# PKU-MARL/HARL

Measured on AMD Instinct MI355X. Metric: transitions/sec through HAPPO update (MPE spread, 3 agents), higher is better.
Workload: dtype f32

## Files before the change

### harl_amd/_lib.py

```python
from __future__ import annotations

import ctypes as C
import os
from typing import Dict, Optional

import torch

from .traffic import algorithmic_bytes, algorithmic_flops

_HERE = os.path.dirname(os.path.abspath(__file__))
LIB_PATH = os.path.join(_HERE, "lib", "libharl_%s.so" % (os.environ.get("HARL_LIB") or "hip"))

PS_STRIDE = 48
DHEAD_LD = 32
SLAB = 32

_vp, _i, _l, _f, _d = C.c_void_p, C.c_int, C.c_long, C.c_float, C.c_double

SIGNATURES = {
    "harl_gae_returns": [_vp] * 8 + [_i, _i, _f, _f, _i, _i, _i, _vp],
    "harl_masked_moments": [_vp, _vp, _l, _vp, _vp, _vp],
    "harl_dist_rows": [_vp, _l, _i, _i, _vp, _f, _f, _vp, _vp, _vp, _i, _i, _vp, _vp, _vp, _vp, _vp, _vp],
    "harl_moments_mean": [_vp, _vp, _vp],
    "harl_clock_probe": [_vp, _l, _vp],
    "harl_build_seq": [_vp, _i, _i, _i, _l, _vp, _vp, _i, _vp, _vp, _vp, _vp, _vp],
    "harl_adv_normalize": [_vp, _vp, _vp, _l, _vp],
    "harl_factor_update": [_vp, _vp, _vp, _l, _i, _i, _vp],
    "harl_sum_sumsq": [_vp, _vp, _l, _vp, _vp],
    "harl_valuenorm_apply": [_vp, _vp, _d, _d, _vp],
    "harl_gradnorm_clip_adam": [_vp, _vp, _vp, _vp, _l, _vp, _i, _f, _d, _d, _d, _f, _f, _d, _d, _vp, _vp],
    "harl_fold_linear": [_vp] * 6 + [_i, _i, _vp],
    "harl_unfold_linear_grads": [_vp, _vp, _i, _vp, _vp, _vp, _vp, _vp, _vp, _vp, _i, _i, _i, _vp],
    "harl_mlp_fwd_input": [_vp, _l, _vp, _l, _i, _vp, _vp, _i, _i, _vp, _vp, _vp, _vp, _vp, _vp, _vp],
    "harl_mlp_x0n_wide": [_vp, _l, _vp, _l, _i, _i, _vp, _vp, _vp, _vp],
    "harl_mlp_fwd_wide": [_vp, _l, _i, _vp, _i, _vp, _i, _vp, _vp, _vp, _vp, _vp],
    "harl_mlp_linear_wide": [_vp, _l, _i, _vp, _i, _vp, _i, _vp, _vp, _vp],
    "harl_act_ln_fwd": [_vp, _l, _i, _i, _vp, _vp, _vp, _vp],
    "harl_act_bwd": [_vp, _vp, _vp, _vp, _l, _i, _i, _vp],
    "harl_act_ln_tangent": [_vp, _vp, _vp, _vp, _vp, _l, _i, _i, _vp, _vp],
    "harl_mlp_tangent_wide": [_vp, _l, _i, _vp, _i, _vp, _i, _vp, _vp, _vp, _vp, _vp, _vp],
    "harl_mlp_fwd_fused2x": [_vp, _l, _vp, _i, _vp, _vp, _vp, _i, _i, _vp, _vp, _vp, _vp, _vp, _vp, _vp],
    "harl_mlp_fwd_fused2": [_vp, _l, _vp, _l, _i, _vp, _vp, _i, _vp, _vp, _i, _i, _vp, _vp, _vp, _vp, _vp, _vp, _vp, _vp,
                            _vp, _vp],
    "harl_mlp_fwd_hidden": [_vp, _l, _i, _i, _vp, _vp, _vp, _vp, _vp, _vp],
    "harl_mlp_bwd_dx": [_vp, _vp, _vp, _vp, _l, _i, _i, _vp, _vp, _vp, _i, _vp, _i, _vp],
    "harl_mlp_bwd_dx_dw": [_vp, _vp, _vp, _vp, _l, _i, _i, _vp, _vp, _vp, _i, _vp, _vp, _i, _i, _vp],
    "harl_mlp_dw_partials": [_vp, _i, _i, _i, _vp, _i, _l, _vp, _vp, _vp, _i, _l, _vp, _i, _vp],
    "harl_mlp_dw_partials_multi": [_i, _vp, _vp, _vp, _i, _i, _l, _i, _vp],
    "harl_mlp_dw_partials_multi_v": [_i, _vp, _vp, _vp, _i, _vp, _vp, _vp, _l, _i, _vp],
    "harl_gru_dw6": [_vp, _vp, _vp, _vp, _vp, _vp, _vp, _l, _i, _vp],
    "harl_mlp_fwd_trunk": [_vp, _l, _i, _vp, _i, _vp, _i, _vp, _i, _vp, _vp, _vp, _vp, _vp, _vp, _vp, _vp, _vp, _vp],
    "harl_mlp_bwd_trunk": [_l, _i, _i, _vp, _vp, _vp, _vp, _vp, _vp, _vp, _vp, _vp, _vp, _vp],
    "harl_reduce_partials": [_vp, _i, _l, _vp, _vp],
    "harl_reduce_partials_multi": [_vp, _vp, _i, _i, _l, _vp, _vp],
    "harl_adam_fold": [_vp, _vp, _vp, _vp, _l, _vp, _vp, _i, _vp, _vp, _vp, _i, _vp, _i, _f, _i, _i, _vp, _i, _f, _d, _d,
                       _d, _f, _f, _d, _d, _vp, _vp],
    "harl_pack_scalars_hilo": [_vp, _vp, _vp],
    "harl_reduce_pack_scalars": [_vp, _i, _vp, _vp, _vp],
    "harl_randperm_replay": [_vp, _l, _l, _vp, _vp, _vp],
    "harl_rng_advance": [_vp, _l, _l, _vp],
    "harl_rng_jump": [_vp, _l, _l, _vp],
    "harl_actor_head_logp": [_vp, _l, _i, _vp, _vp, _vp, _f, _f, _i, _i, _vp, _vp, _vp, _vp, _vp, _i, _vp, _l, _l, _vp],
    "harl_actor_head_loss": [_vp, _vp, _vp, _l, _i, _vp, _vp, _vp, _f, _f, _i, _i, _vp, _vp, _vp, _vp, _vp, _vp,
                             _vp, _vp, _d, _f, _i, _i, _l, _l, _vp, _vp, _vp, _vp, _vp, _i, _vp],
    "harl_critic_head_values": [_vp, _l, _i, _vp, _vp, _vp, _vp],
    "harl_critic_head_loss": [_vp, _vp, _vp, _l, _i, _vp, _vp, _vp, _vp, _vp, _vp, _f, _i, _i, _f, _l, _l, _vp, _vp, _vp,
                              _vp, _i, _vp],
    "harl_gru_fwd": [_vp] * 7 + [_i, _i, _l] + [_vp] * 8 + [_i, _vp, _vp],
    "harl_gru_bwd": [_vp] * 9 + [_i, _i, _l] + [_vp] * 8 + [_vp],
    "harl_fold_linear_tangent": [_vp] * 9 + [_i, _i, _vp],
    "harl_fold_table": [_vp, _vp, _vp, _i, _i, _vp],
    "harl_unfold_table": [_vp, _vp, _vp, _vp, _i, _i, _vp],
    "harl_fold_tangent_table": [_vp, _vp, _vp, _vp, _i, _i, _vp],
    "harl_mlp_tangent_input": [_vp, _l, _vp, _l, _i, _vp, _vp, _i, _i, _vp, _vp, _vp, _vp, _vp],
    "harl_gru_gates": [_vp, _vp, _i, _l, _vp, _vp, _vp, _i, _vp],
    "harl_gru_tangent": [_vp] * 15 + [_i, _i, _l, _vp, _vp],
    "harl_mlp_tangent_hidden": [_vp, _vp, _l, _i, _i, _vp, _vp, _vp, _vp, _vp, _vp, _vp, _vp],
    "harl_mlp_tangent_hidden2": [_vp, _vp, _l, _i, _i, _vp, _vp, _vp, _vp, _vp, _vp, _vp, _vp, _vp],
    "harl_actor_head_fvp": [_vp, _vp, _vp, _vp, _l, _i, _vp, _vp, _vp, _vp, _vp, _f, _f, _i, _i, _vp, _l, _l, _vp, _vp, _vp],
    "harl_trpo_kl_sum": [_vp, _vp, _vp, _vp, _f, _f, _l, _i, _i, _vp, _vp],
    "harl_update_supported": [_i, _i, _i, _i],
    "harl_update_fwd_actor": [_vp, _l, _i, _i] + [_vp] * 7 + [_f, _f, _i, _i] + [_vp] * 7 + [_d, _f, _i, _i] + [_vp] * 4 + [_i] + [_vp] * 4,
    "harl_update_logp": [_vp, _l, _i, _i] + [_vp] * 7 + [_f, _f, _i, _i] + [_vp] * 5 + [_i, _vp, _vp],
    "harl_update_last_actor": [_vp, _l, _i] + [_vp] * 5 + [_f, _f, _i, _i] + [_vp] * 8 + [_d, _f, _i, _i] + [_vp] * 4 + [_i, _vp],
    "harl_update_last_critic": [_vp, _l, _i] + [_vp] * 8 + [_f, _i, _i, _f] + [_vp] * 3 + [_i, _vp],
    "harl_update_fwd_critic": [_vp, _l, _i, _i] + [_vp] * 9 + [_f, _i, _i, _f] + [_vp] * 3 + [_i] + [_vp] * 4,
    "harl_update_values": [_vp, _l, _i, _i] + [_vp] * 7 + [_vp],
    "harl_update_bwd": [_vp, _vp, _l, _i, _i] + [_vp] * 5 + [_i, _vp],
    "harl_head_blocks": [_l],
    "harl_trpo_fvp_finish": [_vp, _vp, _vp, _vp, _l, _f, _f, _l, _i, _f, _f, _vp],
    "harl_trpo_cg_step": [_vp, _vp, _vp, _vp, _l, _vp, _vp, _vp],
    "harl_mlp_panel_fwd": [_vp, _l, _i, _vp, _i, _vp, _i, _vp, _vp, _vp, _vp],
    "harl_mlp_panel_bwd": [_vp, _vp, _vp, _vp, _l, _i, _i, _vp, _vp, _vp],
    "harl_head_dw_rows256": [_vp, _l, _i, _vp, _vp, _i, _vp],
    "harl_mlp_panel_tangent": [_vp, _vp, _l, _i, _vp, _vp, _i, _vp, _vp, _vp, _vp, _vp, _vp],
    "harl_reduce_scalars": [_vp, _i, _vp, _vp],
    "harl_mlp_linear": [_vp, _l, _i, _i, _vp, _vp, _vp, _vp],
    "harl_mlp_linear3": [_vp, _vp, _vp, _l, _i, _i, _vp, _vp, _vp, _vp, _vp, _vp, _vp, _vp, _vp, _vp],
    "harl_gru_cell_init": [_vp, _vp, _i, _l, _vp, _vp],
    "harl_gru_cell_fwd": [_vp] * 8 + [_i, _l] + [_vp] * 7 + [_vp],
    "harl_gru_cell_bwd": [_vp] * 10 + [_i, _l] + [_vp] * 5 + [_vp],
    "harl_rownorm": [_vp, _l, _i, _vp, _vp, _vp],
    "harl_gru_cell_tangent": [_vp] * 19 + [_i, _l] + [_vp] * 3,
    "harl_md_head_logp": [_vp, _i, _vp, _i, _vp, _vp, _l, _vp, _vp, _vp, _i, _vp, _i, _vp, _l, _l, _vp],
    "harl_md_head_loss": [_vp, _vp, _i, _vp, _i, _vp, _vp, _l, _vp, _vp, _vp, _i, _vp, _vp, _vp, _vp, _vp, _d, _f, _i, _i,
                          _l, _l, _vp, _vp, _i, _vp],
    "harl_trpo_begin": [_vp, _vp, _l, _i, _vp, _vp, _vp, _vp, _l, _vp, _vp, _vp, _vp],
    "harl_trpo_step": [_vp, _vp, _vp, _vp, _vp, _vp, _l, _f, _vp, _vp, _vp],
    "harl_trpo_ls_candidate": [_vp, _vp, _vp, _vp, _l, _vp],
    "harl_trpo_ls_test": [_vp, _vp, _d, _d, _d, _d, _vp, _vp],
    "harl_reduce_scalars_set": [_vp, _i, _vp, _vp],
    "harl_zero_bytes": [_vp, _l, _vp],
    "harl_comm_create": [_i, _i, _l, _i, _vp, _vp],
    "harl_comm_connect": [_vp, _vp],
    "harl_comm_allreduce": [_vp, _vp, _l, _i, _vp],
    "harl_comm_set_timeout": [_vp, _d],
    "harl_comm_status": [_vp],
    "harl_comm_destroy": [_vp],
    "harl_version": [],
}


class HipLibraryMissing(RuntimeError):
    pass


_lib: Optional[C.CDLL] = None


def load() -> C.CDLL:
    global _lib
    if _lib is not None:
        return _lib
    if not os.path.exists(LIB_PATH):
        raise HipLibraryMissing(
# ... 109 lines not shown
```

### harl_amd/csrc/heads_common.h

```cpp
#pragma once
#include "common.h"

using namespace harl;

namespace {
constexpr float LOG_SQRT_2PI = 0.918938533204672741780329736406f;
constexpr float HALF_LOG_2PI_PLUS_HALF = 1.418938533204672741780329736406f;

struct ActorArgs {
  const float *xL;
  const uint32_t *relu_mask;
  const float *rstd;
  long M;
  const float *Whp, *bhp, *log_std;
  float std_x_coef, std_y_coef;
  int act_dim;
  const int64_t *idx;
  const float *actions, *avail, *old_logp, *adv;
  const double *adv_moments;
  const float *factor_in, *active;
  float clip_lo, clip_hi, entropy_coef;
  int agg_mean;
  float *dzL, *dhead, *part_scalars;
  float *dw_part;
  float *logp_out, *factor_out;
  float *head_out;
  long m_valid, m_pad;
  int trpo;
  long n_slabs;
};

template <int H, int DAP>
__device__ __forceinline__ void stage_head(float *whl, float *cst, const float *__restrict__ Whp,
                                           const float *__restrict__ bhp, int act_dim) {
  for (int e = threadIdx.x; e < 2 * (H / 2) * DAP; e += WG_THREADS) {
    const int d = e % DAP, R = (e / DAP) % (H / 2), hh = e / (DAP * (H / 2));
    const int f = feat_base(R) + 4 * hh;
    whl[e] = d < act_dim ? Whp[d * H + f] : 0.f;
  }
  for (int e = threadIdx.x; e < DAP; e += WG_THREADS) {
    cst[e] = e < act_dim ? bhp[e] : 0.f;
    float rs = 0.f;
    if (e < act_dim)
      for (int f = 0; f < H; ++f) rs += Whp[e * H + f];
    cst[4 * DAP + e] = rs;
  }
}

template <int H, int DAP>
__device__ __forceinline__ void head_fwd_stream(const float *__restrict__ xL, long slab, int lane,
                                                const float *whl_h, const float *cst, float (&z)[DAP]) {
#pragma unroll
  for (int d = 0; d < DAP; ++d) z[d] = 0.f;
  const f32x4 *xp = reinterpret_cast<const f32x4 *>(xL + slab * (long)(H * SLAB)) + lane;
// ... 78 lines not shown
      }
    }
    __builtin_amdgcn_sched_barrier(0);
  }
#pragma unroll
  for (int d = 0; d < DA; ++d) z[d] = wave_sum32(z[d]) + cst[d];
}

constexpr int HEAD_T_PAD = 16;
__host__ __device__ constexpr int head_t_rows(int da) { return 2 * ((da + 1) / 2); }
__host__ __device__ constexpr int head_t_block(int H, int da) { return head_t_rows(da) * (H / 2) + HEAD_T_PAD; }

template <int H, int DAP, int DA>
__device__ __forceinline__ void head_fwd_regs_t(const f32x4 (&xs)[H / 8], const float *whlT_h, const float *cst,
                                                float (&z)[DAP]) {
#pragma unroll
  for (int d = 0; d < DAP; ++d) z[d] = 0.f;
  f32x4 w[2][DA];
#pragma unroll
  for (int d = 0; d < DA; ++d) w[0][d] = *reinterpret_cast<const f32x4 *>(whlT_h + d * (H / 2));
#pragma unroll
  for (int q = 0; q < H / 8; ++q) {
    if (q + 1 < H / 8) {
#pragma unroll
      for (int d = 0; d < DA; ++d) w[(q + 1) & 1][d] = *reinterpret_cast<const f32x4 *>(whlT_h + d * (H / 2) + 4 * (q + 1));
    }
#pragma unroll
    for (int c = 0; c < 4; ++c)
#pragma unroll
      for (int d = 0; d < DA; ++d) z[d] += xs[q][c] * w[q & 1][d][c];
    __builtin_amdgcn_sched_barrier(0);
  }
#pragma unroll
  for (int d = 0; d < DA; ++d) z[d] = wave_sum32(z[d]) + cst[d];
}

template <int H, int DAP, int DA>
__device__ __forceinline__ void stage_head_t(float *whlT, float *cst, const float *__restrict__ Whp,
                                             const float *__restrict__ bhp, int n_threads) {
  constexpr int DAE = head_t_rows(DA), BLK = head_t_block(H, DA);
  for (int e = threadIdx.x; e < 2 * DAE * (H / 2); e += n_threads) {
    const int R = e % (H / 2), d = (e / (H / 2)) % DAE, hh = e / ((H / 2) * DAE);
    whlT[hh * BLK + d * (H / 2) + R] = d < DA ? Whp[d * H + feat_base(R) + 4 * hh] : 0.f;
  }
  for (int e = threadIdx.x; e < DAP; e += n_threads) {
    cst[e] = e < DA ? bhp[e] : 0.f;
    float rs = 0.f;
    if (e < DA)
      for (int f = 0; f < H; ++f) rs += Whp[e * H + f];
    cst[4 * DAP + e] = rs;
  }
}

template <int H, int DAP, int DA = DAP, bool PACKED = false, bool WT = false>
__device__ __forceinline__ void head_bwd_regs_bits(const f32x4 (&xs)[H / 8], uint32_t b0, const uint32_t b1, float rstd,
                                                   long slab, int lane, const float *whl ,
                                                   const float (&dzh)[DAP], float s1, float s2,
                                                   float *__restrict__ dz_out, const uint32_t bm1 = 0u,
                                                   const uint32_t bm2 = 0u) {
  s1 *= (1.0f / H);
  s2 *= (1.0f / H);
  const int i = lane & 31, h = lane >> 5;
  const float *wa = WT ? whl + ((i >> 2) & 1) * head_t_block(H, DA) + (i & 3) + 4 * (i >> 3) + h * (H / 2)
                       : whl + (((i >> 2) & 1) * (H / 2) + (i & 3) + 4 * (i >> 3)) * DAP + h;
  f32x16 acc[H / 32];
#pragma unroll
  for (int t = 0; t < H / 32; ++t)
#pragma unroll
    for (int r = 0; r < 16; ++r) acc[t][r] = 0.f;
#pragma unroll
  for (int st = 0; st < (DA + 1) / 2; ++st) {
    const unsigned hm = 0u - (unsigned)h;
    const float bsel = __uint_as_float((__float_as_uint(dzh[2 * st + 1]) & hm) | (__float_as_uint(dzh[2 * st]) & ~hm));
#pragma unroll
    for (int t = 0; t < H / 32; ++t)
      acc[t] = __builtin_amdgcn_mfma_f32_32x32x2f32(wa[WT ? 16 * t + 2 * st * (H / 2) : 16 * t * DAP + 2 * st], bsel, acc[t], 0, 0, 0);
  }
  f32x4 *op = reinterpret_cast<f32x4 *>(dz_out + slab * (long)(H * SLAB)) + lane;
  const float c1 = -s1 * rstd, c2 = -s2 * rstd;
  const f32x2 c1v = {c1, c1}, c2v = {c2, c2}, rv = {rstd, rstd};
#pragma unroll
  for (int q = 0; q < H / 8; ++q) {
    if (q == 8) b0 = H == 256 ? bm1 : b1;
    if (H == 256 && q == 16) b0 = bm2;
    if (H == 256 && q == 24) b0 = b1;
    f32x4 o;
    if constexpr (PACKED) {
#pragma unroll
      for (int P = 0; P < 2; ++P) {
        const int e = 4 * q + 2 * P;
        const f32x2 d = {acc[e >> 4][e & 15], acc[(e + 1) >> 4][(e + 1) & 15]}, x = {xs[q][2 * P], xs[q][2 * P + 1]};
        const f32x2 da = fma2(x, c2v, fma2(d, rv, c1v));
        o[2 * P] = mask_pop(da[0], b0);
        o[2 * P + 1] = mask_pop(da[1], b0);
      }
    } else {
#pragma unroll
      for (int c = 0; c < 4; ++c) {
        const float dx = acc[(4 * q + c) >> 4][(4 * q + c) & 15];
        const float da = rstd * (dx - s1 - xs[q][c] * s2);
        o[c] = (int)b0 < 0 ? da : 0.f;
        b0 <<= 1;
      }
    }
    op[q * WAVE] = o;
  }
}

template <int H, int DAP>
__device__ __forceinline__ void head_bwd_regs(const f32x4 (&xs)[H / 8], const uint32_t *__restrict__ mask_in,
                                              float rstd, long slab, int lane, const float *whl ,
                                              const float (&dzh)[DAP], float s1, float s2,
                                              float *__restrict__ dz_out) {
  constexpr int NW = (H / 2 + 31) / 32;
  const uint32_t b0 = mask_in[(slab * NW + 0) * WAVE + lane];
  const uint32_t b1 = NW > 1 ? mask_in[(slab * NW + (NW - 1)) * WAVE + lane] : 0u;
  const uint32_t bm1 = NW == 4 ? mask_in[(slab * NW + 1) * WAVE + lane] : 0u, bm2 = NW == 4 ? mask_in[(slab * NW + 2) * WAVE + lane] : 0u;
  head_bwd_regs_bits<H, DAP>(xs, b0, b1, rstd, slab, lane, whl, dzh, s1, s2, dz_out, bm1, bm2);
}

template <int H>
struct HeadDw {
  static constexpr int HX = 64 + 4;
  static constexpr int TD = 33;
  static constexpr int WAVE_FLOATS = SLAB * HX + SLAB * TD;
  static constexpr int OUT_FLOATS = 32 * H + 32;
};

template <int H, int DAP>
__device__ __forceinline__ void head_dw_step(const f32x4 (&xs)[H / 8], const float (&dzh)[DAP], float *tx, float *td,
                                             int lane, f32x16 (&acc)[H / 32]) {
  constexpr int HX = HeadDw<H>::HX, TD = HeadDw<H>::TD;
  const int i = lane & 31, h = lane >> 5;
  if (h == 0) {
#pragma unroll
    for (int d = 0; d < DAP; ++d) td[i * TD + d] = dzh[d];
  }
#pragma unroll
  for (int half = 0; half < H / 64; ++half) {
#pragma unroll
    for (int q = 0; q < 8; ++q)
      *reinterpret_cast<f32x4 *>(tx + i * HX + 32 * (q >> 2) + 8 * (q & 3) + 4 * h) = xs[8 * half + q];
    asm volatile("s_waitcnt lgkmcnt(0)" ::: "memory");
    __builtin_amdgcn_wave_barrier();
#pragma unroll
    for (int t = 0; t < SLAB / 2; ++t) {
      const float a = td[(2 * t + h) * TD + i];
#pragma unroll
      for (int n = 0; n < 2; ++n) {
        const float b = tx[(2 * t + h) * HX + 32 * n + i];
        acc[2 * half + n] = __builtin_amdgcn_mfma_f32_32x32x2f32(a, b, acc[2 * half + n], 0, 0, 0);
      }
    }
    asm volatile("s_waitcnt lgkmcnt(0)" ::: "memory");
    __builtin_amdgcn_wave_barrier();
  }
}

// ... 474 lines not shown
```

### harl_amd/csrc/mlp.hip

```cpp
#include "common.h"
#include "split_mfma.h"
#include "mfma_transpose.h"
#include "dw_common.h"
#include "fwd_epilogue.h"
#include "../../include/harl_hip.h"
#include <stdlib.h>
#include <type_traits>

using namespace harl;

#define MFMA(a, b, c) __builtin_amdgcn_mfma_f32_32x32x2f32((a), (b), (c), 0, 0, 0)

template <int HO>
__device__ __forceinline__ void ln_jac_store(f32x16 (&acc)[HO / 32], const float *__restrict__ xprimal,
                                             const uint32_t *__restrict__ mask_in, const float *__restrict__ rstd_in,
                                             int lane, long slab, float *__restrict__ xdot_out) {
  constexpr int NR = HO / 2, NW = (NR + 31) / 32;
  float xh[NR];
  atl_load<HO>(xprimal, slab, lane, xh);
  uint32_t bits[NW];
#pragma unroll
  for (int w = 0; w < NW; ++w) bits[w] = mask_in[(slab * NW + w) * WAVE + lane];
  const float rstd = rstd_in[slab * SLAB + (lane & 31)];
  float ad[NR];
// ... 1410 lines not shown
          constexpr int n = decltype(nc)::value, ks = n >> 2, b = n & 3;
          if constexpr (n + 1 < 8) read_frag(r & 1, (n + 1) >> 2, (n + 1) & 3, bv[(n + 1) & 1]);
          __builtin_amdgcn_sched_barrier(0);
          constexpr int AT[6] = {2, 0, 1, 1, 0, 0}, BT[6] = {0, 2, 1, 0, 1, 0};
          static_for<0, 6>([&](auto kc) {
            constexpr int k6 = decltype(kc)::value;
            acc2[b] = mfma_bf16(At[AT[k6]][ks], bv[n & 1][BT[k6]], acc2[b]);
            if constexpr (FILL) slot(std::integral_constant<int, 6 * n + k6>{});
            __builtin_amdgcn_sched_barrier(0);
          });
        });
        PHASE(6);
        b_store((r + 1) & 1);
#pragma unroll
        for (int t = 0; t < 3; ++t) {
          At[t][0] = AtN[t][0];
          At[t][1] = AtN[t][1];
        }
        PHASE(7);
      }
    });
  }

  {
    constexpr long ROW2 = (long)H * H + H;
    float *mypart = dw2_part + (long)blockIdx.x * ROW2;
#pragma unroll
    for (int b = 0; b < 4; ++b)
#pragma unroll
      for (int r = 0; r < 16; ++r) {
        const int o = 32 * wave + (r & 3) + 8 * (r >> 2) + 4 * h;
        mypart[(long)o * H + 32 * b + i] = acc2[b][r];
      }
    const float dbt = wave_sum32(db2);
    if (h == 0) mypart[(long)H * H + 32 * wave + i] = dbt;
    for (int row = blockIdx.x + gridDim.x; row < n_part_rows; row += gridDim.x) {
      float *z = dw2_part + (long)row * ROW2;
      for (int e = threadIdx.x; e < ROW2; e += WG_THREADS) z[e] = 0.f;
    }
  }
  if constexpr (KT > 0) {
    f32x16 a1x[4][1];
#pragma unroll
    for (int a = 0; a < 4; ++a) a1x[a][0] = acc1[a];
    finish_partials<4, 1>(a1x, dbs, reinterpret_cast<float *>(img), dw1_part, n_part_rows);
  }
  PHASE(11);
  PHASE_END(3);
}

#ifndef HARL_BWD_SPLIT_WAVES
#define HARL_BWD_SPLIT_WAVES 1
#endif
template <int KT, bool FILL>
__global__ __launch_bounds__(2 * WG_THREADS, 1) void k_bwd_dx_dw8(
    const float *__restrict__ dz, const float *__restrict__ xprev, const uint32_t *__restrict__ mask_prev,
    const float *__restrict__ rstd_prev, const float *__restrict__ Wp, float *__restrict__ dz_prev, long n_slabs,
    const float *__restrict__ x0n, float *__restrict__ dw1_part, float *__restrict__ dw2_part, int n_part_rows) {
  constexpr int H = 128, MT = 4, NJ = 8, NR = 64, KPF = 32, NTH = 2 * WG_THREADS;
  extern __shared__ __attribute__((aligned(16))) float lds[];
  PHASE_BEGIN();
  u32x4 *img = reinterpret_cast<u32x4 *>(lds);
  unsigned char *Bb = reinterpret_cast<unsigned char *>(img + 3 * MT * NJ * 64);
  stage_split_matrix<H, H, true, NTH>(img, Wp);
  __syncthreads();
  const int lane = threadIdx.x & 63, wave_ = wave_id();
  const int wave = wave_ & 3;
  const bool owner = wave_ < WAVES_PER_WG;
  const int i = lane & 31, h = lane >> 5;
  const u32x4 *wl = img + lane;
  const long sr_stride = (long)gridDim.x * WAVES_PER_WG;
  const long base0 = (long)blockIdx.x * WAVES_PER_WG;
  const Ident ident = make_ident(lane);

  f32x16 acc2[4];
  f32x16 acc1[KT > 0 ? 4 : 1];
  float dbs[KT > 0 ? 4 : 1];
  float db2 = 0.f;
  auto zero_acc2 = [&]() {
#pragma unroll
    for (int b = 0; b < 4; ++b)
#pragma unroll
      for (int r = 0; r < 16; ++r) acc2[b][r] = 0.f;
  };
  auto zero_acc1 = [&]() {
#pragma unroll
    for (int a = 0; a < (KT > 0 ? 4 : 1); ++a) {
      dbs[a] = 0.f;
#pragma unroll
      for (int r = 0; r < 16; ++r) acc1[a][r] = 0.f;
    }
  };

  f32x4 prA[4], prB[4];
  u32x2_t spB[4][3];
  u32x4 ya[3][2];
  f32x16 tc[3];
  u32x4 At[3][2], AtN[3][2];
  float rr0 = 0.f, rr1 = 0.f;
  auto d_load = [&](long ds) {
#pragma unroll
    for (int u = 0; u < 4; ++u) {
      prA[u] = (reinterpret_cast<const f32x4 *>(dz + ds * (long)(H * SLAB)) + lane)[(4 * wave + u) * WAVE];
      prB[u] = (reinterpret_cast<const f32x4 *>(xprev + ds * (long)(H * SLAB)) + lane)[(4 * wave + u) * WAVE];
    }
  };
  float vnext = 1.f;
  auto d_load_next = [&](long ds, long fallback) { d_load(ds < n_slabs ? ds : fallback); };
  auto a_chunk = [&](int k) {
    const int pi = k >> 1, j = pi >> 2, c = pi & 3, u = pi >> 1, e = 2 * (pi & 1);
    if ((k & 1) == 0) {
      unsigned p1;
      split_stage1(prA[u][e], prA[u][e + 1], p1, rr0, rr1);
      ya[0][j][c] = p1;
    } else {
      unsigned p2, p3;
      split_stage2(rr0, rr1, p2, p3);
      ya[1][j][c] = p2;
      ya[2][j][c] = p3;
    }
  };
  auto b_chunk = [&](int k) {
    const int u = k >> 2, c2 = (k >> 1) & 1;
    if ((k & 1) == 0) {
      unsigned p1;
      split_stage1(prB[u][2 * c2], prB[u][2 * c2 + 1], p1, rr0, rr1);
      spB[u][0][c2] = p1;
    } else {
      unsigned p2, p3;
      split_stage2(rr0, rr1, p2, p3);
      spB[u][1][c2] = p2;
      spB[u][2][c2] = p3;
    }
  };
  auto t_mfma = [&](int k) {
    const f32x16 zero = {0.f, 0.f, 0.f, 0.f, 0.f, 0.f, 0.f, 0.f, 0.f, 0.f, 0.f, 0.f, 0.f, 0.f, 0.f, 0.f};
    const int t = k % 3;
    if (k < 3) tc[t] = mfma_bf16(ya[t][0], ident.j0, zero);
    else tc[t] = mfma_bf16(ya[t][1], ident.j1, tc[t]);
  };
  auto p_chunk = [&](int k) {
    if (k < 3) {
      pack_transposed(tc[k], AtN[k][0], AtN[k][1]);
    } else {
      f32x2 a = {0.f, 0.f};
#pragma unroll
      for (int r = 0; r < 8; ++r) a += f32x2{tc[k - 3][2 * r], tc[k - 3][2 * r + 1]};
      db2 += vnext * (a[0] + a[1]);
    }
  };
  auto b_store = [&](int buf) {
#pragma unroll
    for (int u = 0; u < 4; ++u) {
      const int q = 4 * wave + u;
      unsigned char *d = Bb + buf * BDW_BUF + (i >> 2) * BDW_SQ + (2 * (q >> 2) + ((q & 3) >> 1)) * 128 + (i & 3) * 32 +
                         (8 * (q & 1) + 4 * h) * 2;
#pragma unroll
      for (int term = 0; term < 3; ++term) *reinterpret_cast<u32x2_t *>(d + term * BDW_IMG) = spB[u][term];
    }
  };
  const int p16 = lane & 15, g1b = (lane >> 4) & 1;
  const int frag_lane = g1b * 128 + (p16 >> 2) * 32 + (p16 & 3) * 8;
  auto read_frag = [&](int buf, int ks, int tile, u32x4 (&f)[3]) {
#pragma unroll
    for (int term = 0; term < 3; ++term) {
      const unsigned char *fp = Bb + buf * BDW_BUF + term * BDW_IMG + (4 * ks + h) * BDW_SQ + 2 * tile * 128 + frag_lane;
      const u32x2_t lo = tr_read(fp), hi = tr_read(fp + 2 * BDW_SQ);
      f[term] = u32x4{lo[0], lo[1], hi[0], hi[1]};
    }
  };

  float raw[NR];
  u32x4 g1[NJ], g2[NJ], g3[NJ];
  auto o_chunk = [&](int k) {
    const int pi = k >> 1, j = pi >> 2, c = pi & 3;
    if ((k & 1) == 0) {
      unsigned p1;
      split_stage1(raw[2 * pi], raw[2 * pi + 1], p1, rr0, rr1);
      g1[j][c] = p1;
    } else {
      unsigned p2, p3;
      split_stage2(rr0, rr1, p2, p3);
      g2[j][c] = p2;
      g3[j][c] = p3;
    }
  };
  if (!owner && base0 < n_slabs) {
    d_load(base0);
#pragma unroll
    for (int k = 0; k < 16; ++k) a_chunk(k);
#pragma unroll
    for (int k = 0; k < 6; ++k) t_mfma(k);
#pragma unroll
    for (int k = 0; k < 16; ++k) b_chunk(k);
#pragma unroll
    for (int k = 0; k < 6; ++k) p_chunk(k);
#pragma unroll
    for (int t = 0; t < 3; ++t) {
      At[t][0] = AtN[t][0];
      At[t][1] = AtN[t][1];
    }
    b_store(0);
  }
  PHASE(10);

  auto o_part = [&](long base) {
    const long slab = base + wave;
    const bool own = slab < n_slabs;
    constexpr int OB1 = KT > 0 ? 4 : 3, OB2 = KT > 0 ? NJ : 6, OB3 = KT > 0 ? NJ + 1 : NJ;
    auto obar = [&](int k) {
      if (base + k < n_slabs) __builtin_amdgcn_s_barrier();
    };
    if (own) {
      constexpr int RAW_LEAD = 3;
      auto raw_ks = [&](int j) {
        const f32x4 *p = reinterpret_cast<const f32x4 *>(dz + slab * (long)(H * SLAB)) + lane;
#pragma unroll
        for (int c = 0; c < 2; ++c) {
          const f32x4 v = p[(2 * j + c) * WAVE];
#pragma unroll
          for (int e = 0; e < 4; ++e) raw[8 * j + 4 * c + e] = v[e];
        }
      };
#pragma unroll
      for (int j = 0; j < RAW_LEAD; ++j) raw_ks(j);
      obar(0);
#pragma unroll
      for (int k = 0; k < 8; ++k) o_chunk(k);
      float xh[NR];
      float rstd;
      uint32_t mbits[2];
      f32x4 x0r[KT > 0 ? KPF / 8 : 1];
      auto x0_operands = [&]() {
        if constexpr (KT > 0) {
          const f32x4 *bp = reinterpret_cast<const f32x4 *>(x0n + slab * (long)(KPF * SLAB)) + lane;
#pragma unroll
          for (int q = 0; q < KPF / 8; ++q) x0r[q] = bp[q * WAVE];
        }
      };
      auto ln_operands = [&]() {
        atl_load<H>(xprev, slab, lane, xh);
        rstd = rstd_prev[slab * SLAB + i];
#pragma unroll
        for (int w = 0; w < 2; ++w) mbits[w] = mask_prev[(slab * 2 + w) * WAVE + lane];
      };
      constexpr int LN_STEP = NJ;
      f32x16 acc[MT];
#pragma unroll
      for (int t = 0; t < MT; ++t)
#pragma unroll
        for (int r = 0; r < 16; ++r) acc[t][r] = 0.f;
      PHASE(0);
      split_gemm_fill<MT, NJ>(wl, g1, g2, g3, acc, [&](int s_, int k6) {
        const int j1 = s_ / MT + 1, q = (s_ % MT) * 6 + k6;
        if (j1 < NJ && q % 3 == 0) o_chunk(8 * j1 + q / 3);
        if (s_ % MT == 0 && k6 == 0 && j1 - 1 + RAW_LEAD < NJ) raw_ks(j1 - 1 + RAW_LEAD);
        if (s_ % MT == MT - 1 && k6 == 5) {
          if (j1 == LN_STEP) ln_operands();
          if (j1 == OB1) obar(1);
          if (j1 == OB2) obar(2);
          if (j1 == OB3) obar(3);
        }
      });
      PHASE(1);
      float dx[NR];
#pragma unroll
      for (int R = 0; R < NR; ++R) dx[R] = acc[R >> 4][R & 15];
      float out[NR];
      ln_bwd_relu_mbits<H>(dx, xh, mbits, rstd, out);
      if (dz_prev) atl_store<H>(dz_prev, slab, lane, out);
      x0_operands();
      if constexpr (OB3 == NJ + 1) obar(3);
      PHASE(2);
      if constexpr (KT > 0) {
        float xr0[KPF / 2];
#pragma unroll
        for (int q = 0; q < KPF / 8; ++q) {
          xr0[4 * q + 0] = x0r[q][0];
          xr0[4 * q + 1] = x0r[q][1];
          xr0[4 * q + 2] = x0r[q][2];
          xr0[4 * q + 3] = x0r[q][3];
        }
        u32x4 a1[KPF / 16], a2[KPF / 16], a3[KPF / 16];
        split_acts<KPF / 2>(xr0, a1, a2, a3);
        u32x4 Bt[3][2];
        transpose_block<false>(a1[0], a1[1], a2[0], a2[1], a3[0], a3[1], ident, Bt);
#pragma unroll
        for (int a = 0; a < 4; ++a) {
          u32x4 A1[3][2];
          dbs[a] += split_transpose_block<true>(&out[16 * a], ident, A1);
          dw_tile(acc1[a], A1, Bt);
        }
        PHASE(3);
      }
    }
    else {
#pragma unroll
      for (int k = 0; k < 4; ++k) obar(k);
    }
  };
  auto d_part = [&](long base) {
    d_load_next(base + 1, base);
    PHASE(4);
    static_for<0, 4>([&](auto rc) {
      constexpr int r = decltype(rc)::value;
      if (base + r < n_slabs) {
        __syncthreads();
        PHASE(5);
        const long ds1 = r < 3 ? base + r + 1 : base + sr_stride;
        const long ds2 = r < 2 ? base + r + 2 : base + sr_stride;
        vnext = uniform_f(ds1 < n_slabs ? 1.f : 0.f);
        constexpr int TSLOT = r == 0 ? 31 : 15;
        auto slot = [&](auto sc) {
          constexpr int s_ = decltype(sc)::value;
          if constexpr (r == 0) {
            if constexpr (s_ >= 16 && s_ < 32) a_chunk(s_ - 16);
            else if constexpr (s_ >= 32 && s_ < 42) b_chunk(s_ - 32 + 6);
            else if constexpr (s_ >= 42) p_chunk(s_ - 42);
            if constexpr (s_ == 47) d_load_next(ds2, base);
          } else {
            if constexpr (s_ < 16) a_chunk(s_);
            else if constexpr (s_ < 26) b_chunk(s_ - 16 + 6);
            else if constexpr (s_ < 32) p_chunk(s_ - 26);
            if constexpr (s_ == 31 && r < 3) d_load_next(ds2, base);
          }
          if constexpr (s_ == TSLOT) {
            static_for<0, 6>([&](auto kc) {
              constexpr int k = decltype(kc)::value;
              __builtin_amdgcn_sched_barrier(0);
              t_mfma(k);
              b_chunk(k);
            });
          }
        };
        u32x4 bv[2][3];
        read_frag(r & 1, 0, 0, bv[0]);
        if constexpr (!FILL) static_for<0, 48>(slot);
        static_for<0, 8>([&](auto nc) {
          constexpr int n = decltype(nc)::value, ks = n >> 2, b = n & 3;
          if constexpr (n + 1 < 8) read_frag(r & 1, (n + 1) >> 2, (n + 1) & 3, bv[(n + 1) & 1]);
          __builtin_amdgcn_sched_barrier(0);
          constexpr int AT[6] = {2, 0, 1, 1, 0, 0}, BT[6] = {0, 2, 1, 0, 1, 0};
          static_for<0, 6>([&](auto kc) {
            constexpr int k6 = decltype(kc)::value;
            acc2[b] = mfma_bf16(At[AT[k6]][ks], bv[n & 1][BT[k6]], acc2[b]);
            if constexpr (FILL) slot(std::integral_constant<int, 6 * n + k6>{});
            __builtin_amdgcn_sched_barrier(0);
          });
        });
        PHASE(6);
        b_store((r + 1) & 1);
#pragma unroll
        for (int t = 0; t < 3; ++t) {
          At[t][0] = AtN[t][0];
          At[t][1] = AtN[t][1];
        }
        PHASE(7);
      }
    });
  };
  if (owner) {
    zero_acc1();
    for (long base = base0; base < n_slabs; base += sr_stride) o_part(base);
    zero_acc2();
  } else {
    zero_acc2();
    for (long base = base0; base < n_slabs; base += sr_stride) d_part(base);
    zero_acc1();
  }

  {
    constexpr long ROW2 = (long)H * H + H;
    float *mypart = dw2_part + (long)blockIdx.x * ROW2;
    if (!owner) {
#pragma unroll
      for (int b = 0; b < 4; ++b)
#pragma unroll
        for (int r = 0; r < 16; ++r) {
          const int o = 32 * wave + (r & 3) + 8 * (r >> 2) + 4 * h;
          mypart[(long)o * H + 32 * b + i] = acc2[b][r];
        }
      const float dbt = wave_sum32(db2);
      if (h == 0) mypart[(long)H * H + 32 * wave + i] = dbt;
    }
    for (int row = blockIdx.x + gridDim.x; row < n_part_rows; row += gridDim.x) {
      float *z = dw2_part + (long)row * ROW2;
      for (int e = threadIdx.x; e < ROW2; e += NTH) z[e] = 0.f;
    }
  }
  if constexpr (KT > 0) {
    f32x16 a1x[4][1];
#pragma unroll
    for (int a = 0; a < 4; ++a) a1x[a][0] = acc1[a];
    finish_partials<4, 1, NTH>(a1x, dbs, reinterpret_cast<float *>(img), dw1_part, n_part_rows);
  }
  PHASE(11);
  PHASE_END_BY(4, 0);
  PHASE_END_BY(5, 64 * WAVES_PER_WG);
}

HARL_PHASE_ACCESSOR(mlp)

static int bad(const char *m) {
  set_error(m);
  return -2;
}

extern "C" int harl_mlp_fwd_input(const float *X, long ldx, const int64_t *idx, long M, int D, const float *Wp,
                                  const float *bp, int use_ln0, int H, float *xout, uint32_t *relu_mask, float *rstd,
                                  float *mu0, float *rstd0, float *x0n, void *stream) {
  if (M <= 0) return 0;
  const long n_slabs = n_slabs_of(M);
  const int nch = (D + 31) / 32;
  const int grid = persistent_grid(n_slabs, 2);
  hipStream_t s = (hipStream_t)stream;
  if (H != 128 && H != 64) return bad("harl_mlp_fwd_input: hidden width must be 64 or 128");
  if (D <= 64) {
    const int kr = D <= 32 ? 32 : 64;
    const size_t shm = ((size_t)kr * H + H + (size_t)WAVES_PER_WG * SLAB * (kr + 1)) * sizeof(float);
#define LS(Hv, R)                                                                                                 \
  {                                                                                                               \
    allow_big_lds(k_fwd_input_staged<Hv, R>, shm);                                                                \
    hipLaunchKernelGGL((k_fwd_input_staged<Hv, R>), dim3(grid), dim3(WG_THREADS), shm, s, X, ldx, idx, M, D, Wp, bp, \
                       use_ln0, xout, relu_mask, rstd, mu0, rstd0, x0n, n_slabs);                                  \
  }
    if (H == 128) {
      if (D <= 32) LS(128, 2) else LS(128, 1)
    } else {
      if (D <= 32) LS(64, 2) else LS(64, 1)
    }
#undef LS
    return check_launch("harl_mlp_fwd_input");
  }
  const int resident = (long)nch * 32 * H * 4 <= 64 * 1024;
  const size_t shm = ((size_t)(resident ? nch * 32 : 32) * H + H) * sizeof(float);
  if (H == 128) {
    allow_big_lds(k_fwd_input<128, false>, shm);
    hipLaunchKernelGGL((k_fwd_input<128, false>), dim3(grid), dim3(WG_THREADS), shm, s, X, ldx, idx, M, D, Wp, bp,
                       use_ln0, xout, relu_mask, rstd, mu0, rstd0, n_slabs, nch, resident, nullptr, nullptr, nullptr);
  } else {
    allow_big_lds(k_fwd_input<64, false>, shm);
    hipLaunchKernelGGL((k_fwd_input<64, false>), dim3(grid), dim3(WG_THREADS), shm, s, X, ldx, idx, M, D, Wp, bp,
                       use_ln0, xout, relu_mask, rstd, mu0, rstd0, n_slabs, nch, resident, nullptr, nullptr, nullptr);
  }
  return check_launch("harl_mlp_fwd_input");
}

extern "C" int harl_mlp_tangent_input(const float *X, long ldx, const int64_t *idx, long M, int D, const float *Wdp,
                                      const float *bdp, int use_ln0, int H, const float *x1, const uint32_t *mask1,
                                      const float *rstd1, float *x1dot, void *stream) {
  if (M <= 0) return 0;
  const long n_slabs = n_slabs_of(M);
// ... 176 lines not shown
static bool lean_bwd() {
  static const bool v = [] {
    const char *e = getenv("HARL_BWD_STREAMS");
    return e && e[0] == '1';
  }();
  return v;
}

extern "C" int harl_mlp_bwd_dx(const float *dz, const float *xprev, const uint32_t *relu_mask_prev,
                               const float *rstd_prev, long M, int HO, int HI, const float *Wp, float *dz_prev,
                               const float *x0n, int kp0, float *dw_part, int n_wg, void *stream) {
  if (M <= 0) return 0;
  const long n_slabs = n_slabs_of(M);
  hipStream_t s = (hipStream_t)stream;
  if (dw_part) {
    if (!x0n || (kp0 != 32 && kp0 != 64) || n_wg <= 0)
      return bad("harl_mlp_bwd_dx: fused first-layer gradient needs x0n, kp0 in {32, 64} and n_wg > 0");
#define LFX(a, b, kt, lean)                                                                                       \
  {                                                                                                               \
    size_t shm = split_image_bytes(b, a);                                                                         \
    const size_t rowb = ((size_t)b * 32 * kt + b) * sizeof(float);                                                \
    if (shm < rowb) shm = rowb;                                                                                   \
    allow_big_lds(k_bwd_dx<a, b, kt, lean>, shm);                                                                 \
    hipLaunchKernelGGL((k_bwd_dx<a, b, kt, lean>), dim3(n_wg < 256 ? n_wg : 256), dim3(WG_THREADS), shm, s, dz,   \
                       xprev, relu_mask_prev, rstd_prev, Wp, dz_prev, n_slabs, x0n, dw_part, n_wg);               \
  }
#define LF(a, b, kt) LFX(a, b, kt, false)
    const int kt = kp0 / 32;
    if (HO == 128 && HI == 128 && kt == 1 && lean_bwd()) LFX(128, 128, 1, true)
    else if (HO == 128 && HI == 128) { if (kt == 1) LF(128, 128, 1) else LF(128, 128, 2) }
    else if (HO == 64 && HI == 64) { if (kt == 1) LF(64, 64, 1) else LF(64, 64, 2) }
    else if (HO == 128 && HI == 64) { if (kt == 1) LF(128, 64, 1) else LF(128, 64, 2) }
    else if (HO == 64 && HI == 128) { if (kt == 1) LF(64, 128, 1) else LF(64, 128, 2) }
    else return bad("harl_mlp_bwd_dx: widths must be 64 or 128");
#undef LF
#undef LFX
    return check_launch("harl_mlp_bwd_dx");
  }
  const size_t shm = split_image_bytes(HI, HO);
  const int grid = persistent_grid(n_slabs, split_one_wg(HI, HO) ? 1 : 2);
#define L(a, b)                                                                                                    \
  allow_big_lds(k_bwd_dx<a, b>, shm);                                                                              \
  hipLaunchKernelGGL((k_bwd_dx<a, b>), dim3(grid), dim3(WG_THREADS), shm, s, dz, xprev, relu_mask_prev, rstd_prev, Wp, \
                     dz_prev, n_slabs, nullptr, nullptr, 0)
  if (HO == 128 && HI == 128) { L(128, 128); }
  else if (HO == 64 && HI == 64) { L(64, 64); }
  else if (HO == 128 && HI == 64) { L(128, 64); }
  else if (HO == 64 && HI == 128) { L(64, 128); }
  else return bad("harl_mlp_bwd_dx: widths must be 64 or 128");
#undef L
  return check_launch("harl_mlp_bwd_dx");
}

extern "C" int harl_mlp_bwd_dx_dw(const float *dz, const float *xprev, const uint32_t *relu_mask_prev,
                                  const float *rstd_prev, long M, int HO, int HI, const float *Wp, float *dz_prev,
                                  const float *x0n, int kp0, float *dw1_part, float *dw2_part, int n_wg, int fill,
                                  void *stream) {
  if (M <= 0) return 0;
  if (HO != 128 || HI != 128) return bad("harl_mlp_bwd_dx_dw: 128 x 128 layers only (the layer kernels take the other widths)");
  if (!dw2_part || n_wg <= 0) return bad("harl_mlp_bwd_dx_dw: needs the partial arena of dW' and n_wg > 0");
  const bool first = dw1_part != nullptr;
  if (first && (!x0n || kp0 != 32)) return bad("harl_mlp_bwd_dx_dw: the fused first-layer gradient needs x0n with kp0 = 32");
  if (!first && !dz_prev) return bad("harl_mlp_bwd_dx_dw: dz_prev is required when no first-layer gradient is fused");
  const long n_slabs = n_slabs_of(M);
  const long wgs = (n_slabs + WAVES_PER_WG - 1) / WAVES_PER_WG;
  int grid = n_wg < 256 ? n_wg : 256;
  if (wgs < grid) grid = (int)wgs;
  const size_t shm = bdw_lds_bytes();
  hipStream_t s = (hipStream_t)stream;
#if HARL_BWD_SPLIT_WAVES
#define LB(kt, fl)                                                                                                    \
  {                                                                                                                   \
    allow_big_lds(k_bwd_dx_dw8<kt, fl>, shm);                                                                         \
    hipLaunchKernelGGL((k_bwd_dx_dw8<kt, fl>), dim3(grid), dim3(2 * WG_THREADS), shm, s, dz, xprev, relu_mask_prev,  \
                       rstd_prev, Wp, dz_prev, n_slabs, x0n, dw1_part, dw2_part, n_wg);                              \
  }
#else
#define LB(kt, fl)                                                                                                    \
  {                                                                                                                   \
    allow_big_lds(k_bwd_dx_dw<kt, fl>, shm);                                                                          \
    hipLaunchKernelGGL((k_bwd_dx_dw<kt, fl>), dim3(grid), dim3(WG_THREADS), shm, s, dz, xprev, relu_mask_prev,       \
                       rstd_prev, Wp, dz_prev, n_slabs, x0n, dw1_part, dw2_part, n_wg);                              \
  }
#endif
  if (first) { if (fill) LB(1, true) else LB(1, false) }
  else { if (fill) LB(0, true) else LB(0, false) }
#undef LB
  return check_launch("harl_mlp_bwd_dx_dw");
}

template <int MT, int NT>
static void launch_dw_tr(const float *a, const float *b, long n_slabs, float *part, int K, int tile0, int n_wg, hipStream_t s) {
  const size_t shm = (size_t)3 * 8 * ((2 * MT * 128 + 8) + (2 * NT * 128 + 8));
  allow_big_lds(k_dw_tr<MT, NT>, shm);
  hipLaunchKernelGGL((k_dw_tr<MT, NT>), dim3(n_wg), dim3(WG_THREADS), shm, s, a, b, n_slabs, part, (long)K * SLAB, tile0, K);
}

template <int A_KIND, int B_KIND, int MT, int NT>
static void launch_dw(const float *a, const float *b, long ldx, const int64_t *idx, const float *mu0,
                      const float *rstd0, int K, long M, long n_slabs, float *part, int KP, int n_wg, int ny,
                      hipStream_t s) {
  const size_t shm = ((size_t)DW_S * ((32 * MT + 4) + (32 * NT + 4)) + 2 * DW_S) * sizeof(float);
  hipLaunchKernelGGL((k_dw<A_KIND, B_KIND, MT, NT>), dim3(n_wg, ny), dim3(WG_THREADS), shm, s, a, b, ldx, idx, mu0,
                     rstd0, K, M, n_slabs, part, KP);
}

extern "C" int harl_mlp_dw_partials(const float *a, int a_kind, int lda, int HO, const float *b, int b_kind, long ldx,
                                    const int64_t *idx, const float *mu0, const float *rstd0, int K, long M,
                                    float *part, int n_wg, void *stream) {
  if (M <= 0 || n_wg <= 0) return 0;
  const long n_slabs = n_slabs_of(M);
  const int KP = ((K + 31) / 32) * 32;
  hipStream_t s = (hipStream_t)stream;
  if (a_kind == 1 && lda != DHEAD_LD) return bad("harl_mlp_dw_partials: head gradient matrix must have row stride 32");
  const int MT = a_kind == 1 ? 1 : HO / 32;
  if (a_kind == 0 && HO != 64 && HO != 128 && HO != 256) return bad("harl_mlp_dw_partials: HO must be 64, 128 or 256");
  if (a_kind == 1 && HO > 32) return bad("harl_mlp_dw_partials: head width must be <= 32");
#define DW(AK, BK, MTv, NTv, ny) launch_dw<AK, BK, MTv, NTv>(a, b, ldx, idx, mu0, rstd0, K, M, n_slabs, part, KP, n_wg, ny, s)
  if (b_kind == 0) {
    const int NT = K / 32;
    if (K % 32 != 0 || K < 32) return bad("harl_mlp_dw_partials: ATL input width must be a multiple of 32");
#define DWS(MTv, NTv) launch_dw_tr<MTv, NTv>(a, b, n_slabs, part, K, tile0, n_wg, s);
    if (K > 128 || K == 96 || MT == 8) {
      if (K % 32 != 0 || K > 512 || (MT != 8 && MT != 4 && MT != 2)) return bad("harl_mlp_dw_partials: wide ATL input must be a multiple of 32, <= 512");
      const int ntiles = K / 32;
      const int gstep = MT == 8 ? 2 : (MT == 4 && ntiles > 4 ? (ntiles + (ntiles + 5) / 6 - 1) / ((ntiles + 5) / 6) : 4);
      for (int tile0 = 0; tile0 < ntiles; tile0 += gstep) {
        const int nt = ntiles - tile0 < gstep ? ntiles - tile0 : gstep;
        if (MT == 8) {
          if (nt == 2) DWS(8, 2) else DWS(8, 1)
        } else if (MT == 4) {
          if (nt == 6) DWS(4, 6) else if (nt == 5) DWS(4, 5) else
          if (nt == 4) DWS(4, 4) else if (nt == 3) DWS(4, 3) else if (nt == 2) DWS(4, 2) else DWS(4, 1)
        } else {
          if (nt == 4) DWS(2, 4) else if (nt == 3) DWS(2, 3) else if (nt == 2) DWS(2, 2) else DWS(2, 1)
        }
      }
      return check_launch("harl_mlp_dw_partials");
    }
    const int tile0 = 0;
    if (MT == 4 && NT == 1) DW(0, 0, 4, 1, 1);
    else if (MT == 2 && NT == 1) DW(0, 0, 2, 1, 1);
// ... 92 lines not shown
```

### harl_amd/csrc/update.hip

```cpp
#include <type_traits>
#include "common.h"
#include "split_mfma.h"
#include "heads_common.h"
#include "mfma_transpose.h"
#include "../../include/harl_hip.h"

using namespace harl;

namespace {

int bad(const char *m) {
  set_error(m);
  return -2;
}

template <int H, bool MASK>
__device__ __forceinline__ void relu_ln(const f32x16 (&acc)[H / 32], float (&v)[H / 2], uint32_t (&bits)[(H / 2 + 31) / 32],
                                        float &rstd_out) {
  constexpr int NR = H / 2;
#pragma unroll
  for (int w = 0; w < (NR + 31) / 32; ++w) bits[w] = 0u;
#pragma unroll
  for (int R = 0; R < NR; ++R) {
    if constexpr (MASK) v[R] = relu_push(acc[R >> 4][R & 15], bits[R >> 5]);
// ... 208 lines not shown
#pragma unroll
        for (int r = 0; r < 16; ++r) acc[t][r] = b1l[32 * t + (r & 3) + 8 * (r >> 2) + 4 * h];
      split_gemm<MT, NJ1>(wl1, a1, a2, a3, acc, [](int) {});
      relu_ln<H, true>(acc, x1, bits1, r1);
      ln_bwd_relu_bits<H>(dx, x1, bits1, r1, dz1);
    }
    u32x4 B[KT][3][2];
#pragma unroll
    for (int n = 0; n < KT; ++n)
      transpose_block<false>(a1[2 * n], a1[2 * n + 1], a2[2 * n], a2[2 * n + 1], a3[2 * n], a3[2 * n + 1], I, B[n]);
#pragma unroll
    for (int a = 0; a < MT; ++a) {
      u32x4 A[3][2];
      dbs[a] += split_transpose_block<true>(&dz1[16 * a], I, A);
#pragma unroll
      for (int n = 0; n < KT; ++n) dw_tile(acc1[a][n], A, B[n]);
    }
  }
  finish_partials<MT, KT>(acc1, dbs, reinterpret_cast<float *>(img2), part, n_part_rows);
}

struct UpdFwdArgs {
  const float *x0n, *W1p, *b1p, *W2p, *b2p;
  int D;
  long n_slabs;
  float *dz2;
  int n_part_rows;
  float *xh1;
  uint32_t *mask1;
  float *rstd1;
};

constexpr int UF_WAVES = 8, UF_THREADS = 64 * UF_WAVES;

template <int NV>
__device__ __forceinline__ void block_reduce_store8(float (&v)[NV], float *red , float *out_row) {
  const int lane = threadIdx.x & 63, wave = wave_id();
#pragma unroll
  for (int k = 0; k < NV; ++k) {
    float t = wave_reduce_sum(v[k]);
    if (lane == 0) red[wave * PS_STRIDE + k] = t;
  }
  __syncthreads();
  if (threadIdx.x < PS_STRIDE) {
    float t = 0.f;
    if (threadIdx.x < NV) {
#pragma unroll
      for (int w = 0; w < UF_WAVES; ++w) t += red[w * PS_STRIDE + threadIdx.x];
    }
    out_row[threadIdx.x] = t;
  }
}

template <int H, int KP0, int DA, bool DISCRETE, bool TRAIN, typename ARGS>
__global__ __launch_bounds__(UF_THREADS, 2) void k_upd_fwd(UpdFwdArgs U, ARGS A) {
  constexpr bool CRITIC = std::is_same<ARGS, CriticArgs>::value;
  static_assert(DA >= 1 && DA <= 8 && (!CRITIC || DA == 1), "the LDS head-gradient tile covers 8 head outputs");
  constexpr int DAP = DA <= 4 ? 4 : 8;
  constexpr int HROWS = DA;
  constexpr bool HID = KP0 == 0;
  constexpr bool EARLY_X0N = H == 128 && KP0 == 32 && DA <= 5 && !DISCRETE;
  constexpr bool EARLY_X0N_LP = !TRAIN && !HID && (H == 64 || (DA != 4 && !(KP0 == 64 && DA >= 7 && !DISCRETE)));
  static_assert(!HID || TRAIN, "the last-layer variant exists for optimiser steps only");
  extern __shared__ __attribute__((aligned(16))) float lds[];
  PHASE_BEGIN();
  constexpr int MT = H / 32, NJ1 = KP0 / 16, NJ2 = H / 16, NR = H / 2, NW = (NR + 31) / 32;
  u32x4 *w2img = reinterpret_cast<u32x4 *>(lds);
  u32x4 *w1img = w2img + 3 * MT * NJ2 * 64;
  float *b1l = reinterpret_cast<float *>(w1img + 3 * MT * NJ1 * 64);
  float *b2l = b1l + H;
  float *whlT = b2l + H;
  float *cst = whlT + 2 * head_t_block(H, DA);
  float *red = cst + 7 * DAP;
  float *hacc = red + UF_WAVES * PS_STRIDE;
  const int lane = threadIdx.x & 63, wave = wave_id(), i = lane & 31, h = lane >> 5;
  const long slab0 = (long)wave * gridDim.x + blockIdx.x, slab_stride = (long)gridDim.x * UF_WAVES;
  constexpr int NXR = HID ? NR : KP0 / 2;
  float xr[NXR];
  atl_load<2 * NXR>(U.x0n, slab0 < U.n_slabs ? slab0 : 0, lane, xr);
  constexpr bool ROWS = !CRITIC || TRAIN;
  long rawn = 0;
  if constexpr (ROWS) rawn = row_index_request(A.idx, A.Whp, slab0, lane, A.M);
  stage_split_matrix<H, H, false, UF_THREADS>(w2img, U.W2p);
  if constexpr (!HID) stage_w1_images<H, KP0, UF_THREADS>(w1img, U.W1p, U.D);
  for (int e = threadIdx.x; e < H; e += UF_THREADS) {
    if constexpr (!HID) b1l[e] = U.b1p[e];
    b2l[e] = U.b2p[e];
  }
  if (TRAIN)
    for (int e = threadIdx.x; e < UF_WAVES * HROWS * H; e += UF_THREADS) hacc[e] = 0.f;
  if (threadIdx.x < WG_THREADS) {
    stage_head_t<H, DAP, DA>(whlT, cst, A.Whp, A.bhp, WG_THREADS);
    if constexpr (!CRITIC) {
      if (!DISCRETE) {
        for (int e = threadIdx.x; e < DAP; e += WG_THREADS) {
          float sg = 0.5f, sig = 1.f, lsig = 0.f, dsd = 0.f;
          if (e < A.act_dim) {
            sg = 1.0f / (1.0f + expf(-A.log_std[e] / A.std_x_coef));
            sig = sg * A.std_y_coef;
            lsig = logf(sig);
            dsd = A.std_y_coef * sg * (1.f - sg) / A.std_x_coef;
          }
          cst[DAP + e] = sig;
          cst[2 * DAP + e] = lsig;
          cst[3 * DAP + e] = dsd;
          cst[5 * DAP + e] = 1.0f / sig;
          cst[6 * DAP + e] = 1.0f / (sig * sig);
        }
// ... 113 lines not shown
      s2 = dv * (z[0] - cst[0]);
    } else {
      if (!actor_sample<DAP, DISCRETE, TRAIN, DA>(A, cst, z, slab, lane, adv_mean, adv_den, sc, dzh, s1, s2, rcur)) continue;
    }
    PHASE(6);
    if constexpr (TRAIN) {
      if constexpr (EARLY_X0N) atl_load<2 * NXR>(U.x0n, sn, lane, xr);
      int lane_o = lane;
      asm volatile("" : "+v"(lane_o));
      const Ident I = make_ident(lane_o);
      const u32x4 I16 = make_ident16(lane_o);
      u32x4 Ah[3][2];
      {
        float e8[8];
#pragma unroll
        for (int c = 0; c < 8; ++c) e8[c] = (c < DAP && h == 0) ? dzh[c < DAP ? c : 0] : 0.f;
        u32x4 t1, t2, t3;
#pragma unroll
        for (int c = 0; c < 4; ++c) {
          unsigned a, b, d;
          split3(e8[2 * c], e8[2 * c + 1], a, b, d);
          t1[c] = a;
          t2[c] = b;
          t3[c] = d;
        }
        const f32x16 zero = {0.f, 0.f, 0.f, 0.f, 0.f, 0.f, 0.f, 0.f, 0.f, 0.f, 0.f, 0.f, 0.f, 0.f, 0.f, 0.f};
        const f32x16 c1 = mfma_bf16(t1, I16, zero), c2 = mfma_bf16(t2, I16, zero), c3 = mfma_bf16(t3, I16, zero);
        pack_transposed(c1, Ah[0][0], Ah[0][1]);
        pack_transposed(c2, Ah[1][0], Ah[1][1]);
        pack_transposed(c3, Ah[2][0], Ah[2][1]);
      }
#pragma unroll
      for (int n = 0; n < MT; ++n) {
        u32x4 B[3][2];
        split_transpose_block<false>(&v[16 * n], I, B);
        f32x16 tile = {0.f, 0.f, 0.f, 0.f, 0.f, 0.f, 0.f, 0.f, 0.f, 0.f, 0.f, 0.f, 0.f, 0.f, 0.f, 0.f};
        dw_tile(tile, Ah, B);
#pragma unroll
        for (int r = 0; r < 4; ++r) {
          if (r < HROWS && h == 0) hw[r * H + 32 * n + i] += tile[r];
          if (4 + r < HROWS && h == 1) hw[(4 + r) * H + 32 * n + i] += tile[r];
        }
      }
      if constexpr (CRITIC) {
        if (h == 0) dbacc[0] += dzh[0];
      } else {
        if (h == 1) {
#pragma unroll
          for (int d = 0; d < DAP; ++d) sc[8 + d] += dzh[d];
        }
      }
      PHASE(7);
      if constexpr (!EARLY_X0N) atl_load<2 * NXR>(U.x0n, sn, lane, xr);
      head_bwd_regs_bits<H, DAP, DA, true, true>(xs, bits2[0], bits2[NW - 1], r2, slab, lane, whlT, dzh, s1, s2, U.dz2);
      PHASE(8);
    }
  }
  if constexpr (TRAIN) {
    float dbv[DAP];
#pragma unroll
    for (int d = 0; d < DAP; ++d) {
      if constexpr (CRITIC) {
        dbv[d] = dbacc[d];
      } else {
        dbv[d] = h == 1 ? sc[8 + d] : 0.f;
        sc[8 + d] = h == 0 ? sc[8 + d] : 0.f;
      }
    }
    block_reduce_store8<NSC>(sc, red, A.part_scalars + (long)blockIdx.x * PS_STRIDE);
    for (int row = blockIdx.x + gridDim.x; row < U.n_part_rows; row += gridDim.x)
      if (threadIdx.x < PS_STRIDE) A.part_scalars[(long)row * PS_STRIDE + threadIdx.x] = 0.f;
    float dbs[DAP];
#pragma unroll
    for (int d = 0; d < DAP; ++d) dbs[d] = wave_reduce_sum(dbv[d]);
    float *dbl = red;
    __syncthreads();
    if (lane == 0) {
#pragma unroll
      for (int d = 0; d < DAP; ++d) dbl[wave * PS_STRIDE + d] = dbs[d];
    }
    __syncthreads();
    float *out = A.dw_part + (long)blockIdx.x * HeadDw<H>::OUT_FLOATS;
    for (int e = threadIdx.x; e < HeadDw<H>::OUT_FLOATS; e += UF_THREADS) {
      float t = 0.f;
      if (e < 32 * H) {
        const int row = e / H;
        if (row < HROWS) {
#pragma unroll
          for (int w = 0; w < UF_WAVES; ++w) t += hacc[(w * HROWS + row) * H + (e - row * H)];
        }
      } else {
        const int d = e - 32 * H;
        if (d < DAP) {
#pragma unroll
          for (int w = 0; w < UF_WAVES; ++w) t += dbl[w * PS_STRIDE + d];
        }
      }
      out[e] = t;
    }
    for (int row = blockIdx.x + gridDim.x; row < U.n_part_rows; row += gridDim.x) {
      float *zr = A.dw_part + (long)row * HeadDw<H>::OUT_FLOATS;
      for (int e = threadIdx.x; e < HeadDw<H>::OUT_FLOATS; e += UF_THREADS) zr[e] = 0.f;
    }
  }
  PHASE(11);
  PHASE_END((TRAIN ? 0 : 2) + (CRITIC ? 1 : 0));
}

int fwd_grid(long n_slabs) {
  const long wgs = (n_slabs + UF_WAVES - 1) / UF_WAVES;
  return (int)(wgs < 256 ? (wgs < 1 ? 1 : wgs) : 256);
}

int upd_grid(long n_slabs) {
  const long wgs = (n_slabs + WAVES_PER_WG - 1) / WAVES_PER_WG;
  return (int)(wgs < 256 ? (wgs < 1 ? 1 : wgs) : 256);
}

size_t fwd_lds_bytes(int H, int kp0, int dap, int hrows, int da) {
  return split_image_bytes(H, H) + split_image_bytes(H, kp0) +
         ((size_t)2 * H + (size_t)2 * head_t_block(H, da) + 7 * dap + UF_WAVES * PS_STRIDE + (size_t)UF_WAVES * hrows * H) *
             sizeof(float);
}

constexpr size_t LDS_PER_WG_MAX = 160 * 1024;

template <int H, int KP0, int DA, bool DISC, bool TRAIN, typename ARGS>
int launch_fwd(const UpdFwdArgs &U, const ARGS &A, hipStream_t s) {
  const size_t shm = fwd_lds_bytes(H, KP0, DA <= 4 ? 4 : 8, TRAIN ? DA : 0, DA);
  if (shm > LDS_PER_WG_MAX) {
    return bad("harl_update_*: this (D, H, act_dim) does not fit the LDS of one workgroup");
  }
  allow_big_lds(k_upd_fwd<H, KP0, DA, DISC, TRAIN, ARGS>, shm);
  hipLaunchKernelGGL((k_upd_fwd<H, KP0, DA, DISC, TRAIN, ARGS>), dim3(fwd_grid(U.n_slabs)), dim3(UF_THREADS), shm, s, U, A);
  return 0;
}

template <int H, int KP0, bool TRAIN, int DA = 8>
int launch_actor_width(const UpdFwdArgs &U, const ActorArgs &A, int discrete, hipStream_t s) {
  if (A.act_dim == DA)
    return discrete ? launch_fwd<H, KP0, DA, true, TRAIN, ActorArgs>(U, A, s) : launch_fwd<H, KP0, DA, false, TRAIN, ActorArgs>(U, A, s);
  if constexpr (DA > 1) return launch_actor_width<H, KP0, TRAIN, DA - 1>(U, A, discrete, s);
  return bad("harl_update_*: act_dim must be in [1, 8]");
}

template <bool TRAIN>
int dispatch_fwd_actor(const UpdFwdArgs &U, const ActorArgs &A, int H, int discrete, hipStream_t s) {
  const int D = A.act_dim;
  if (D < 1 || D > 8) return bad("harl_update_fwd: act_dim must be in [1, 8]");
  const int kp0 = U.D <= 32 ? 32 : 64;
#define CASE(Hv, Kv)                                                                \
  if (H == Hv && kp0 == Kv) {                                                       \
    const int rc = launch_actor_width<Hv, Kv, TRAIN>(U, A, discrete, s);             \
    return rc ? rc : check_launch("harl_update_fwd");                               \
  }
  CASE(128, 32) CASE(128, 64) CASE(64, 32) CASE(64, 64)
#undef CASE
  return bad("harl_update_fwd: hidden width must be 64 or 128");
}

int dispatch_last_actor(const UpdFwdArgs &U, const ActorArgs &A, int H, int discrete, hipStream_t s) {
  const int D = A.act_dim;
  if (D < 1 || D > 8) return bad("harl_update_last_actor: act_dim must be in [1, 8]");
  int rc;
  if (H == 128) rc = launch_actor_width<128, 0, true>(U, A, discrete, s);
  else if (H == 64) rc = launch_actor_width<64, 0, true>(U, A, discrete, s);
  else return bad("harl_update_last_actor: hidden width must be 64 or 128");
  return rc ? rc : check_launch("harl_update_last_actor");
}

int dispatch_last_critic(const UpdFwdArgs &U, const CriticArgs &A, int H, hipStream_t s) {
  int rc;
  if (H == 128) rc = launch_fwd<128, 0, 1, false, true, CriticArgs>(U, A, s);
  else if (H == 64) rc = launch_fwd<64, 0, 1, false, true, CriticArgs>(U, A, s);
  else return bad("harl_update_last_critic: hidden width must be 64 or 128");
  return rc ? rc : check_launch("harl_update_last_critic");
}

template <bool TRAIN>
int dispatch_fwd_critic(const UpdFwdArgs &U, const CriticArgs &A, int H, hipStream_t s) {
  const int kp0 = U.D <= 32 ? 32 : 64;
#define CASE(Hv, Kv)                                                     \
  if (H == Hv && kp0 == Kv) {                                            \
    const int rc = launch_fwd<Hv, Kv, 1, false, TRAIN, CriticArgs>(U, A, s); \
    return rc ? rc : check_launch("harl_update_fwd");                        \
  }
  CASE(128, 32) CASE(128, 64) CASE(64, 32) CASE(64, 64)
#undef CASE
  return bad("harl_update_fwd: hidden width must be 64 or 128");
}

}

HARL_PHASE_ACCESSOR(update)

extern "C" int harl_update_supported(int D, int H, int act_dim, int kind) {
  if (!(D >= 0 && D <= 64 && (H == 64 || H == 128) && act_dim >= 1 && act_dim <= 8)) return 0;
  const int dap = act_dim <= 4 ? 4 : 8;
  const int hrows = kind == 0 ? 0 : (kind == 2 ? 1 : act_dim);
  return fwd_lds_bytes(H, D == 0 ? 0 : (D <= 32 ? 32 : 64), dap, hrows, kind == 2 ? 1 : act_dim) <= LDS_PER_WG_MAX ? 1 : 0;
}

extern "C" int harl_update_fwd_actor(const float *x0n, long M, int D, int H, const float *W1p, const float *b1p,
                                     const float *W2p, const float *b2p, const float *Whp, const float *bhp,
                                     const float *log_std, float std_x_coef, float std_y_coef, int discrete, int act_dim,
                                     const float *actions, const float *avail, const float *old_logp, const float *adv,
                                     const double *adv_moments, const float *factor, const float *active,
                                     double clip_param, float entropy_coef, int agg_mean, int trpo, float *logp_out,
                                     float *dz2, float *part_scalars, float *dw_part_head, int n_part_rows, float *xh1,
                                     uint32_t *rmask1, float *rstd1, void *stream) {
  if (M <= 0) return 0;
  if (D < 1 || D > 64) return bad("harl_update_fwd_actor: input width must be <= 64");
  if (!dz2 || !part_scalars || !dw_part_head || n_part_rows <= 0) return bad("harl_update_fwd_actor: missing outputs");
  if (xh1 && (!rmask1 || !rstd1)) return bad("harl_update_fwd_actor: xh1 needs rmask1 and rstd1");
  UpdFwdArgs U{x0n, W1p, b1p, W2p, b2p, D, n_slabs_of(M), dz2, n_part_rows, xh1, rmask1, rstd1};
  if (fwd_grid(U.n_slabs) > n_part_rows) return bad("harl_update_fwd_actor: n_part_rows smaller than the launch grid");
  ActorArgs A{};
  A.trpo = trpo;
  A.logp_out = logp_out;
  A.dw_part = dw_part_head;
  A.M = M; A.Whp = Whp; A.bhp = bhp; A.log_std = log_std;
  A.std_x_coef = std_x_coef; A.std_y_coef = std_y_coef; A.act_dim = act_dim;
  A.actions = actions; A.avail = avail; A.old_logp = old_logp; A.adv = adv; A.adv_moments = adv_moments;
  A.factor_in = factor; A.active = active; A.entropy_coef = entropy_coef;
  A.clip_lo = (float)(1.0 - clip_param); A.clip_hi = (float)(1.0 + clip_param);
  A.agg_mean = agg_mean; A.part_scalars = part_scalars; A.n_slabs = U.n_slabs;
  return dispatch_fwd_actor<true>(U, A, H, discrete, (hipStream_t)stream);
}

extern "C" int harl_update_logp(const float *x0n, long M, int D, int H, const float *W1p, const float *b1p,
                                const float *W2p, const float *b2p, const float *Whp, const float *bhp,
                                const float *log_std, float std_x_coef, float std_y_coef, int discrete, int act_dim,
                                const float *actions, const float *avail, float *logp_out, const float *old_logp,
                                float *factor, int agg_mean, float *head_out, void *stream) {
  if (M <= 0) return 0;
  if (D < 1 || D > 64) return bad("harl_update_logp: input width must be <= 64");
  if (factor && !old_logp) return bad("harl_update_logp: factor update needs old_logp");
  UpdFwdArgs U{x0n, W1p, b1p, W2p, b2p, D, n_slabs_of(M), nullptr, 0, nullptr, nullptr, nullptr};
  ActorArgs A{};
  A.head_out = head_out;
  A.M = M; A.Whp = Whp; A.bhp = bhp; A.log_std = log_std;
  A.std_x_coef = std_x_coef; A.std_y_coef = std_y_coef; A.act_dim = act_dim;
  A.actions = actions; A.avail = avail; A.old_logp = old_logp; A.agg_mean = agg_mean;
  A.logp_out = logp_out; A.factor_out = factor; A.n_slabs = U.n_slabs;
  return dispatch_fwd_actor<false>(U, A, H, discrete, (hipStream_t)stream);
}

extern "C" int harl_update_fwd_critic(const float *x0n, long M, int D, int H, const float *W1p, const float *b1p,
                                      const float *W2p, const float *b2p, const float *Whp, const float *bhp,
                                      const float *value_preds, const float *returns, const float *vn_stats,
                                      float clip_param, int use_clipped, int use_huber, float huber_delta, float *dz2,
                                      float *part_scalars, float *dw_part_head, int n_part_rows, float *xh1,
                                      uint32_t *rmask1, float *rstd1, void *stream) {
  if (M <= 0) return 0;
  if (D < 1 || D > 64) return bad("harl_update_fwd_critic: input width must be <= 64");
  if (!dz2 || !part_scalars || !dw_part_head || n_part_rows <= 0) return bad("harl_update_fwd_critic: missing outputs");
  if (xh1 && (!rmask1 || !rstd1)) return bad("harl_update_fwd_critic: xh1 needs rmask1 and rstd1");
  UpdFwdArgs U{x0n, W1p, b1p, W2p, b2p, D, n_slabs_of(M), dz2, n_part_rows, xh1, rmask1, rstd1};
  if (fwd_grid(U.n_slabs) > n_part_rows) return bad("harl_update_fwd_critic: n_part_rows smaller than the launch grid");
  CriticArgs A{};
  A.M = M; A.Whp = Whp; A.bhp = bhp;
  A.value_preds = value_preds; A.returns = returns; A.vn_stats = vn_stats; A.clip_param = clip_param;
  A.huber_delta = huber_delta; A.use_clipped = use_clipped; A.use_huber = use_huber;
  A.part_scalars = part_scalars; A.n_slabs = U.n_slabs;
  A.dw_part = dw_part_head;
  return dispatch_fwd_critic<true>(U, A, H, (hipStream_t)stream);
}

extern "C" int harl_update_last_actor(const float *xin, long M, int H, const float *Wp, const float *bp, const float *Whp,
                                      const float *bhp, const float *log_std, float std_x_coef, float std_y_coef,
                                      int discrete, int act_dim, const int64_t *idx, const float *actions,
                                      const float *avail, const float *old_logp, const float *adv,
                                      const double *adv_moments, const float *factor, const float *active,
                                      double clip_param, float entropy_coef, int agg_mean, int trpo, float *logp_out,
                                      float *dz, float *part_scalars, float *dw_part_head, int n_part_rows, void *stream) {
  if (M <= 0) return 0;
  if (!xin || !dz || !part_scalars || !dw_part_head || n_part_rows <= 0) return bad("harl_update_last_actor: missing arguments");
  UpdFwdArgs U{xin, nullptr, nullptr, Wp, bp, 0, n_slabs_of(M), dz, n_part_rows, nullptr, nullptr, nullptr};
  if (fwd_grid(U.n_slabs) > n_part_rows) return bad("harl_update_last_actor: n_part_rows smaller than the launch grid");
  ActorArgs A{};
  A.trpo = trpo;
  A.logp_out = logp_out;
  A.dw_part = dw_part_head;
  A.M = M; A.Whp = Whp; A.bhp = bhp; A.log_std = log_std;
  A.std_x_coef = std_x_coef; A.std_y_coef = std_y_coef; A.act_dim = act_dim; A.idx = idx;
  A.actions = actions; A.avail = avail; A.old_logp = old_logp; A.adv = adv; A.adv_moments = adv_moments;
  A.factor_in = factor; A.active = active; A.entropy_coef = entropy_coef;
  A.clip_lo = (float)(1.0 - clip_param); A.clip_hi = (float)(1.0 + clip_param);
  A.agg_mean = agg_mean; A.part_scalars = part_scalars; A.n_slabs = U.n_slabs;
  return dispatch_last_actor(U, A, H, discrete, (hipStream_t)stream);
}

extern "C" int harl_update_last_critic(const float *xin, long M, int H, const float *Wp, const float *bp, const float *Whp,
                                       const float *bhp, const int64_t *idx, const float *value_preds, const float *returns,
                                       const float *vn_stats, float clip_param, int use_clipped, int use_huber,
                                       float huber_delta, float *dz, float *part_scalars, float *dw_part_head,
                                       int n_part_rows, void *stream) {
  if (M <= 0) return 0;
  if (!xin || !dz || !part_scalars || !dw_part_head || n_part_rows <= 0) return bad("harl_update_last_critic: missing arguments");
  UpdFwdArgs U{xin, nullptr, nullptr, Wp, bp, 0, n_slabs_of(M), dz, n_part_rows, nullptr, nullptr, nullptr};
  if (fwd_grid(U.n_slabs) > n_part_rows) return bad("harl_update_last_critic: n_part_rows smaller than the launch grid");
  CriticArgs A{};
  A.M = M; A.Whp = Whp; A.bhp = bhp; A.idx = idx;
  A.value_preds = value_preds; A.returns = returns; A.vn_stats = vn_stats; A.clip_param = clip_param;
  A.huber_delta = huber_delta; A.use_clipped = use_clipped; A.use_huber = use_huber;
  A.part_scalars = part_scalars; A.n_slabs = U.n_slabs;
  A.dw_part = dw_part_head;
  return dispatch_last_critic(U, A, H, (hipStream_t)stream);
}

extern "C" int harl_update_values(const float *x0n, long M, int D, int H, const float *W1p, const float *b1p,
                                  const float *W2p, const float *b2p, const float *Whp, const float *bhp, float *values,
                                  void *stream) {
  if (M <= 0) return 0;
  if (D < 1 || D > 64) return bad("harl_update_values: input width must be <= 64");
  UpdFwdArgs U{x0n, W1p, b1p, W2p, b2p, D, n_slabs_of(M), nullptr, 0, nullptr, nullptr, nullptr};
  CriticArgs A{};
  A.M = M; A.Whp = Whp; A.bhp = bhp; A.values_out = values; A.n_slabs = U.n_slabs;
  return dispatch_fwd_critic<false>(U, A, H, (hipStream_t)stream);
// ... 33 lines not shown
```

### harl_amd/happo.py

```python
from __future__ import annotations

import os
from typing import Optional

import numpy as np
import torch

from . import _lib
from ._lib import PS_STRIDE, call, ptr, stream
from .buffers import OnPolicyActorBuffer, consume_randperm, minibatch_indices, rng_sync
from .dist import Comm, local_minibatch_rows
from .nets import FusedAdam, StochasticPolicy, build_seq, seq_compact
from .valuenorm import _as_dev


class OnPolicyBase:

    def __init__(self, args, obs_space, act_space, device=torch.device("cuda:0")):
        self.args = args
        self.device = torch.device(device)
        _lib.require_gpu(self.device)
        self.tpdv = dict(dtype=torch.float32, device=self.device)
        self.data_chunk_length = args["data_chunk_length"]
        self.use_recurrent_policy = args["use_recurrent_policy"]
# ... 142 lines not shown
                else:
                    actions.copy_(torch.multinomial(probs, 1))
                self._dist_rows(head, M, actions=actions, logp=logp)
        else:
            noise = None if deterministic else torch.randn_like(head)
            actions = torch.empty_like(head)
            logp = torch.empty_like(head)
            self._dist_rows(head, M, noise=noise, actions=actions, logp=logp)
        return actions, logp, rnn_out

    @torch.no_grad()
    def act(self, obs, rnn_states_actor, masks, available_actions=None, deterministic=False):
        actions, _, rnn = self.get_actions(obs, rnn_states_actor, masks, available_actions, deterministic)
        return actions, rnn

    def prep_training(self):
        self.actor.train()
        self.actor.invalidate_caches()

    def prep_rollout(self):
        self.actor.eval()
        self.actor.invalidate_caches()


class HAPPO(OnPolicyBase):
    def __init__(self, args, obs_space, act_space, device=torch.device("cuda:0")):
        super().__init__(args, obs_space, act_space, device)
        self.clip_param = args["clip_param"]
        self.ppo_epoch = args["ppo_epoch"]
        self.actor_num_mini_batch = args["actor_num_mini_batch"]
        self.entropy_coef = args["entropy_coef"]
        self.use_max_grad_norm = args["use_max_grad_norm"]
        self.max_grad_norm = args["max_grad_norm"]
        self._surrogate_mode = 0
        self._info = torch.zeros(4, dtype=torch.float64, device=self.device)
        self._grad_tap = None
        self._trace = None
        self._state_tap = None
        self._factor_ready = None

    def _await_factor(self) -> None:
        ev = self._factor_ready
        if ev is not None:
            self._factor_ready = None
            torch.cuda.current_stream(self.device).wait_event(ev)

    def _forward_backward(self, obs, idx, m, actions, avail, old_logp, adv, adv_moments, factor, active, seq=None,
                          logp_out=None):
        net = self.actor
        s = stream()
        if net.fused_update_ok(idx, seq):
            fa = net.fused_args(obs, m)
            self._await_factor()
            call("harl_update_fwd_actor", *fa, ptr(net.log_std()), net.std_x_coef, net.std_y_coef, int(net.discrete),
                 net.act_dim, ptr(actions), ptr(avail), ptr(old_logp), ptr(adv), ptr(adv_moments), ptr(factor),
                 ptr(active), float(self.clip_param), float(self.entropy_coef), int(self.action_aggregation == "mean"),
                 self._surrogate_mode, ptr(logp_out), ptr(net.dz[0]), ptr(net.part_scalars),
                 ptr(net.part[net._part_offs[-1]:]), net.n_wg, *net.hybrid_outputs(), s, tag="update_fwd")
            net.backward_after_fused(obs, m)
            return net.n_wg
        if net.fused_last_ok(idx, seq):
            L = len(net.hidden_sizes)
            net.forward_trunk(obs, idx, m, upto=L - 1)
            (Wl, bl), (Wh, bh) = net._packs[L - 1], net._packs[-1]
            self._await_factor()
            call("harl_update_last_actor", ptr(net.xh[L - 2]), m, net.hidden_sizes[-1], ptr(Wl), ptr(bl), ptr(Wh), ptr(bh),
                 ptr(net.log_std()), net.std_x_coef, net.std_y_coef, int(net.discrete), net.act_dim, ptr(idx), ptr(actions),
                 ptr(avail), ptr(old_logp), ptr(adv), ptr(adv_moments), ptr(factor), ptr(active), float(self.clip_param),
                 float(self.entropy_coef), int(self.action_aggregation == "mean"), self._surrogate_mode, ptr(logp_out),
                 ptr(net.dz[0]), ptr(net.part_scalars), ptr(net.part[net._part_offs[-1]:]), net.n_wg, s, tag="update_last")
            net.backward_trunk(obs, idx, m, head_dw_done=True)
            return net.n_wg
        net.forward_trunk(obs, idx, m, seq=seq)
        Wp, bp = net._packs[-1]
        fx, fmask, frstd, fh = net.feat()
        mv, mp = (seq["m"], seq["m_pad"]) if seq is not None else (0, 0)
        self._await_factor()
        if net.md:
            net.md_logits(m)
            nblk = _lib.load().harl_head_blocks(m)
            lay = net.md_layout()
            call("harl_md_head_loss", lay[0], *lay, m, ptr(idx), ptr(actions), ptr(old_logp), old_logp.shape[1], ptr(adv),
                 ptr(adv_moments), ptr(factor), ptr(active), ptr(self._md_ent_scale(idx, m, active, seq)),
                 float(self.clip_param), float(self.entropy_coef), int(self.action_aggregation == "mean"),
                 self._surrogate_mode, mv, mp, ptr(logp_out), ptr(net.part_scalars), nblk, s, tag="md_head_loss")
            net.backward_trunk(obs, idx, m, seq=seq)
            return nblk
        call("harl_actor_head_loss", ptr(fx), ptr(fmask), ptr(frstd), m, fh,
             ptr(Wp), ptr(bp), ptr(net.log_std()), net.std_x_coef, net.std_y_coef, int(net.discrete), net.act_dim,
             ptr(idx), ptr(actions), ptr(avail), ptr(old_logp), ptr(adv), ptr(adv_moments), ptr(factor), ptr(active),
             float(self.clip_param), float(self.entropy_coef), int(self.action_aggregation == "mean"), self._surrogate_mode,
             mv, mp, ptr(logp_out), ptr(net.dz[0]), ptr(net.dhead), ptr(net.part_scalars),
             None if net.wide_head else ptr(net.part[net._part_offs[-1]:]), net.n_wg, s,
             tag="actor_head_loss")
        net.backward_trunk(obs, idx, m, seq=seq, head_dw_done=not net.wide_head)
        return net.n_wg if not net.wide_head else _lib.load().harl_head_blocks(m)

    def _md_ent_scale(self, idx, m, active, seq) -> Optional[torch.Tensor]:
        if active is None:
            return None
        if getattr(self, "_md_ent_override", None) is not None:
            return self._md_ent_override
        if seq is not None:
            j = torch.arange(m, device=self.device)
            live = (j % seq["m_pad"]) < seq["m"]
            rows = idx[live] if idx is not None else j[live]
            st = torch.stack([active[rows].sum(), torch.tensor(float(rows.numel()), device=self.device)])
        else:
            a = active if idx is None else active[idx]
            st = torch.stack([a.sum(), torch.tensor(float(m), device=self.device)])
        self.comm.all_reduce_sum(st)
        return (st[0] / st[1]).reshape(1).contiguous()
# ... 160 lines not shown
```

### harl_amd/nets.py

```python
from __future__ import annotations

import math
import os
from typing import Dict, List, Optional, Sequence, Tuple

import torch
import torch.nn as nn

from . import _lib
from ._lib import DHEAD_LD, PS_STRIDE, SLAB, call, ptr, stream

SUPPORTED_WIDTHS = (64, 128, 256)
ACT_IDS = {"relu": 0, "leaky_relu": 1, "tanh": 2, "sigmoid": 3, "selu": 4}


_FUSED_UPDATE_MODES = ("hybrid", "logp", "1", "actor", "0")


def _fused_update_mode() -> str:
    mode = os.environ.get("HARL_FUSED_UPDATE", "hybrid")
    if mode not in _FUSED_UPDATE_MODES:
        raise ValueError(f"HARL_FUSED_UPDATE={mode!r}: expected one of {_FUSED_UPDATE_MODES}")
    return mode


BWD_FUSED_MIN_ROWS = 400_000


def _bwd_fused_mode(M: int = 0) -> str:
    m = os.environ.get("HARL_BWD_FUSED", "auto")
    if m not in ("0", "1", "nofill", "auto"):
        raise ValueError(f"HARL_BWD_FUSED={m!r}: expected auto, 0, 1 or nofill")
    if m == "auto":
        return "1" if M >= BWD_FUSED_MIN_ROWS else "0"
    return m


def _bwd_streams() -> bool:
    return os.environ.get("HARL_BWD_STREAMS", "0") == "1"


def _space_shape(space) -> Tuple[int, ...]:
    name = space.__class__.__name__
    if name == "Box":
        return tuple(space.shape)
    if name == "list":
        return tuple(space)
    raise NotImplementedError(f"observation space {name}")


class _Node(nn.Module):
    """Empty container used to reproduce the reference's dotted parameter names."""


def _register(root: nn.Module, dotted: str, p: nn.Parameter) -> None:
    parts = dotted.split(".")
    mod = root
    for name in parts[:-1]:
        if name not in mod._modules:
            mod.add_module(name, _Node())
        mod = mod._modules[name]
    mod.register_parameter(parts[-1], p)


class _FlatNet(nn.Module):

    def __init__(self, args: dict, in_dim: int, device: torch.device):
        super().__init__()
        _lib.require_gpu(device)
        self.device_ = device
        self.hidden_sizes = list(args["hidden_sizes"])
        self.use_feature_normalization = bool(args["use_feature_normalization"])
        self.activation_func = args.get("activation_func", "relu")
        if self.activation_func not in ACT_IDS:
            raise NotImplementedError(f"activation_func {self.activation_func!r}: supported are {sorted(ACT_IDS)} (the functions "
                                      "torch.nn.init.calculate_gain knows, as in the reference's MLPLayer)")
        self.act_id = ACT_IDS[self.activation_func]
        self.recurrent = bool(args.get("use_recurrent_policy", False) or args.get("use_naive_recurrent_policy", False))
        self.recurrent_n = int(args.get("recurrent_n", 1))
        hl = self.hidden_sizes[-1]
        self.gru_wide = self.recurrent and ((hl == 128 and os.environ.get("HARL_GRU128", "1") != "0")
                                            or (hl in (64, 128) and self.recurrent_n > 1))
        if self.recurrent and hl == 64 and os.environ.get("HARL_GRU_COMPOSED") == "1":
            self.gru_wide = True
        if self.recurrent and self.recurrent_n < 1:
# ... 175 lines not shown
                b0 = self._gru_pack_base + 2 * l * (n + 3 * H)
                self.gru_packs.append(dict(Wih=self.pack_arena[b0:b0 + n], bih=self.pack_arena[b0 + n:b0 + n + 3 * H],
                                           Whh=self.pack_arena[b0 + n + 3 * H:b0 + 2 * n + 3 * H],
                                           bhh=self.pack_arena[b0 + 2 * n + 3 * H:b0 + 2 * n + 6 * H]))
            self.gru_pack = self.gru_packs[0]
        covered = sum(o * k + o for (_, _, _, _, o, k) in ents)
        covered += sum(k for go, k in {(go, k) for (_, _, go, _, _, k) in ents if go >= 0}) * 2
        if isinstance(self, StochasticPolicy) and not self.discrete:
            covered += self.act_dim
        assert covered == self.n_params, f"layer table covers {covered} of {self.n_params} parameters"
        self.table = None

    def fold(self) -> None:
        if not self._packs:
            self._build_tables()
        ver = self.flat_param._version
        if getattr(self, "_fold_version", None) == ver and os.environ.get("HARL_ALWAYS_FOLD", "0") != "1":
            return
        s = stream()
        fp, pa = self.flat_param, self.pack_arena
        if self.table is not None and os.environ.get("HARL_FOLD_TABLE", "1") != "0":
            call("harl_fold_table", ptr(fp), ptr(pa), ptr(self.table), self.n_entries, sum(r[4] for r in self._table_rows), s)
            self._fold_version = ver
            return
        for (wo, bo, go, beo, o, k), (pw, pb, _, _) in zip(self._entries(), self._pack_slots):
            call("harl_fold_linear", ptr(fp[wo:]), ptr(fp[bo:]), ptr(fp[go:]) if go >= 0 else None,
                 ptr(fp[beo:]) if beo >= 0 else None, ptr(pa[pw:]), ptr(pa[pb:]), o, k, s)
        self._fold_version = ver

    def _ensure_ws(self, M: int) -> None:
        if M <= self._max_rows:
            return
        dev = self.device_
        n_slabs = (M + SLAB - 1) // SLAB
        mp = n_slabs * SLAB
        f32, u32 = torch.float32, torch.int32
        self.xh = [torch.empty(mp * h, dtype=f32, device=dev) for h in self.hidden_sizes]
        self.rmask = [torch.empty(n_slabs * max(h // 64, 1) * 64, dtype=u32, device=dev) for h in self.hidden_sizes]
        self.rstd = [torch.empty(mp, dtype=f32, device=dev) for _ in self.hidden_sizes]
        self.mu0 = torch.empty(mp, dtype=f32, device=dev)
        self.rstd0 = torch.empty(mp, dtype=f32, device=dev)
        self.kp0 = ((self.in_dim + 31) // 32) * 32
        self.wide = 32 < self.in_dim <= 512
        self._x0n_key = None
        self.x0n = torch.empty(mp * self.kp0, dtype=f32, device=dev) if (self.in_dim <= 64 or self.wide) else None
        self.w1img = (torch.empty(3 * self.hidden_sizes[0] * self.kp0 // 2, dtype=f32, device=dev)
                      if (self.wide or self.act_id) else None)
        hmax = max(self.hidden_sizes)
        if self.act_id:
            self.zraw = torch.empty(mp * hmax, dtype=f32, device=dev)
            self.amean = [torch.empty(mp, dtype=f32, device=dev) for _ in self.hidden_sizes]
            self.ones_mask = torch.full((n_slabs * 64 * 2,), -1, dtype=u32, device=dev)
        self.dz = [torch.empty(mp * hmax, dtype=f32, device=dev) for _ in range(3 if len(self.hidden_sizes) == 3 and self.trunk_fused() else 2)]
        self._trunk_cache = {}
        self.wide_head = (not self.md) and self._layers()[-1][4] > 32
        self.dhead = torch.zeros(mp * (64 if self.wide_head else DHEAD_LD), dtype=f32, device=dev)
        self.md_z = [torch.zeros(mp * sp, dtype=f32, device=dev) for sp in self._md_sp]
        n_iter = (n_slabs + 1) // 2
        nwg_env = os.environ.get("HARL_NWG")
        nwg_cap = int(nwg_env) if nwg_env else max(256, min(512, n_slabs // 10))
        if (not nwg_env and _bwd_fused_mode(M) == "1" and len(self.hidden_sizes) >= 2 and all(h == 128 for h in self.hidden_sizes)
                and ((self.in_dim + 31) // 32) * 32 == 32 and not (self.recurrent or self.md or self.act_id or self.panel)):
            nwg_cap = 256
        self.n_wg = max(1, min(nwg_cap, n_iter))
        part_off, rows = 0, [list(r) for r in self._table_rows]
        self._part_offs = []
        for r, elems in zip(rows, self._elems):
            r[11] = part_off
            self._part_offs.append(part_off)
            part_off += self.n_wg * elems
        self.part = torch.empty(part_off, dtype=f32, device=dev)
        self.table = torch.tensor(rows, dtype=torch.int32, device=dev).reshape(-1).contiguous()
        if self.recurrent:
            H = self.hidden_sizes[-1]
            a = lambda: torch.empty(mp * H, dtype=f32, device=dev)
            self.rnn_y, self.rnn_rstd = a(), torch.empty(mp, dtype=f32, device=dev)
            self.rnn_saved_l = [[a() for _ in range(5)] for _ in range(self.recurrent_n)]
            self.rnn_dgate_l = [[a() for _ in range(4)] for _ in range(self.recurrent_n)]
            self.rnn_saved, self.rnn_dgate = self.rnn_saved_l[0], self.rnn_dgate_l[0]
            self.rnn_ones = torch.full((n_slabs * 64 * ((H // 2 + 31) // 32),), -1, dtype=u32, device=dev)
            self.rnn_gi = torch.empty(3 * mp * H, dtype=f32, device=dev)
            if self.gru_wide:
                from . import gru_wide
                gru_wide.ensure_ws(self, mp)
        self.n_head_blocks = max(_lib.load().harl_head_blocks(M), self.n_wg)
        self.part_scalars = torch.zeros(self.n_head_blocks * PS_STRIDE, dtype=f32, device=dev)
        self.scalars = torch.zeros(PS_STRIDE, dtype=torch.float64, device=dev)
        self._max_rows = M

    def feat(self):
        if self.recurrent:
            return self.rnn_y, self.rnn_ones, self.rnn_rstd, self.hidden_sizes[-1]
        if self.act_id:
            return self.xh[-1], self.ones_mask, self.rstd[-1], self.hidden_sizes[-1]
        return self.xh[-1], self.rmask[-1], self.rstd[-1], self.hidden_sizes[-1]

    def forward_rnn(self, seq: dict, save: bool, gates_done: bool = False) -> None:
        if self.gru_wide:
            from . import gru_wide
            return gru_wide.forward(self, seq, save)
        gp = self.gru_pack
        sv = self.rnn_saved
        call("harl_gru_fwd", ptr(self.xh[-1]), ptr(seq["mask_rows"]), ptr(seq["h0"]), ptr(gp["Wih"]), ptr(gp["bih"]),
             ptr(gp["Whh"]), ptr(gp["bhh"]), self.hidden_sizes[-1], seq["L"], seq["m_pad"], ptr(self.rnn_y),
             ptr(self.rnn_rstd), ptr(sv[0]), ptr(sv[1]), ptr(sv[2]), ptr(sv[3]), ptr(sv[4]), ptr(seq.get("h_last")),
             int(save) | (2 if gates_done else 0), ptr(self.rnn_gi), stream(), tag="gru_fwd")
# ... 82 lines not shown
            first_hidden = 2
        elif len(hs) >= 2 and hs[0] == hs[1] and self.in_dim <= 32:
            (W1, b1), (W2, b2) = self._packs[0], self._packs[1]
            self._x0n_key = None
            call("harl_mlp_fwd_fused2", ptr(X), X.shape[1], ptr(idx), M, self.in_dim, ptr(W1), ptr(b1),
                 int(self.use_feature_normalization), ptr(W2), ptr(b2), hs[0], int(for_backward), ptr(self.xh[0]),
                 ptr(self.rmask[0]), ptr(self.rstd[0]), ptr(self.mu0), ptr(self.rstd0), ptr(self.xh[1]),
                 ptr(self.rmask[1]), ptr(self.rstd[1]), ptr(self.x0n) if for_backward else None, s, tag="fwd_fused2")
            first_hidden = 2
        elif self.wide:
            Wp, bp = self._packs[0]
            self._x0n_image(X, M, s, idx)
            call("harl_mlp_fwd_wide", ptr(self.x0n), M, self.kp0, ptr(Wp), self.in_dim, ptr(bp), hs[0], ptr(self.w1img),
                 ptr(self.xh[0]), ptr(self.rmask[0]), ptr(self.rstd[0]), s, tag="fwd_wide")
        else:
            Wp, bp = self._packs[0]
            self._x0n_key = None
            call("harl_mlp_fwd_input", ptr(X), X.shape[1], ptr(idx), M, self.in_dim, ptr(Wp), ptr(bp),
                 int(self.use_feature_normalization), hs[0], ptr(self.xh[0]), ptr(self.rmask[0]), ptr(self.rstd[0]),
                 ptr(self.mu0), ptr(self.rstd0), ptr(self.x0n) if for_backward else None, s, tag="fwd_input")
        assert upto is None or upto >= first_hidden
        for l in range(first_hidden, len(hs) if upto is None else upto):
            Wp, bp = self._packs[l]
            call("harl_mlp_fwd_hidden", ptr(self.xh[l - 1]), M, hs[l - 1], hs[l],
                 ptr(Wp), ptr(bp), ptr(self.xh[l]), ptr(self.rmask[l]), ptr(self.rstd[l]), s, tag="fwd_hidden")
        if self.recurrent:
            self.forward_rnn(seq, save=rnn_save)

    def fused_update_ok(self, idx: Optional[torch.Tensor], seq: Optional[dict] = None, train: bool = True) -> bool:
        hs = self.hidden_sizes
        mode = _fused_update_mode()
        if self.act_id:
            return False
        if mode == "0" or (train and mode == "logp") or (train and mode == "actor" and isinstance(self, VNet)):
            return False
        if not (not self.recurrent and not self.md and idx is None and seq is None
                and len(hs) == 2 and hs[0] == hs[1] and hs[0] in (64, 128) and self.in_dim <= 64 and self._layers()[-1][4] <= 8):
            return False
        kind = 0 if not train else (2 if isinstance(self, VNet) else 1)
        return bool(_lib.load().harl_update_supported(self.in_dim, hs[0], self._layers()[-1][4], kind))

    def fused_last_ok(self, idx: Optional[torch.Tensor], seq: Optional[dict] = None) -> bool:
        hs = self.hidden_sizes
        if _fused_update_mode() != "hybrid" or self.act_id or self.recurrent or self.md or self.panel:
            return False
        if seq is not None or len(hs) < 2 or hs[-1] != hs[-2] or hs[-1] not in (64, 128) or self._layers()[-1][4] > 8:
            return False
        two_fused = hs[0] == hs[1] and ((self.in_dim <= 64 and idx is None) or self.in_dim <= 32)
        return len(hs) >= (3 if two_fused else 2) and bool(_lib.load().harl_update_supported(0, hs[-1], self._layers()[-1][4], 2 if isinstance(self, VNet) else 1))

    def fused_hybrid(self) -> bool:
        return _fused_update_mode() == "hybrid"

    def hybrid_outputs(self):
        if not self.fused_hybrid():
            return (None, None, None)
        return (ptr(self.xh[0]), ptr(self.rmask[0]), ptr(self.rstd[0]))

    def backward_after_fused(self, X: torch.Tensor, M: int) -> None:
        if self.fused_hybrid():
            self.backward_trunk(X, None, M, head_dw_done=True)
        else:
            self.backward_fused(M)

    def fused_args(self, X: torch.Tensor, M: int):
        self._ensure_ws(M)
        self._x0n_image(X, M, stream())
        (W1, b1), (W2, b2), (Wh, bh) = self._packs[0], self._packs[1], self._packs[-1]
        return (ptr(self.x0n), M, self.in_dim, self.hidden_sizes[0], ptr(W1), ptr(b1), ptr(W2), ptr(b2), ptr(Wh), ptr(bh))

    def _bwd_side(self):
        if getattr(self, "_bwd_side_stream", None) is None:
            self._bwd_side_stream = torch.cuda.Stream(device=self.device_)
            self._bwd_ev = [torch.cuda.Event(), torch.cuda.Event()]
        return self._bwd_side_stream

    def _combine_partials(self, s) -> None:
        call("harl_reduce_partials_multi", ptr(self.part), ptr(self.table), self.n_entries, self.n_wg, self.total_dwp,
             ptr(self.dwp), s, tag="reduce_partials")

    def backward_fused(self, M: int) -> None:
        s = stream()
        (W1, b1), (W2, _) = self._packs[0], self._packs[1]
        po = self._part_offs
        call("harl_update_bwd", ptr(self.x0n), ptr(self.dz[0]), M, self.in_dim, self.hidden_sizes[0], ptr(W1), ptr(b1),
             ptr(W2), ptr(self.part[po[0]:]), ptr(self.part[po[1]:]), self.n_wg, s, tag="update_bwd")
        self._combine_partials(s)

    def backward_trunk(self, X: torch.Tensor, idx: Optional[torch.Tensor], M: int, seq: Optional[dict] = None,
                       head_dw_done: bool = False) -> None:
        s = stream()
        L = len(self.hidden_sizes)
        nwg = self.n_wg
        po = self._part_offs
        hdim = self._layers()[-1][4]
        fx, _, _, fh = self.feat()
        if self.md:
            self.md_backward(M)
        elif not head_dw_done:
            if self.wide_head:
                call("harl_mlp_dw_partials", ptr(self.dhead), 0, 0, 64, ptr(fx), 0, 0, None, None, None, fh, M,
                     ptr(self.part[po[-1]:]), nwg, s, tag="dw_head")
            elif self.panel:
                call("harl_head_dw_rows256", ptr(self.dhead), M, hdim, ptr(fx), ptr(self.part[po[-1]:]), nwg, s, tag="dw_head")
            else:
                call("harl_mlp_dw_partials", ptr(self.dhead), 1, DHEAD_LD, hdim, ptr(fx), 0, 0, None, None, None, fh, M,
                     ptr(self.part[po[-1]:]), nwg, s, tag="dw_head")
        if self.trunk_fused() and not self.gru_wide:
            return self._backward_trunk_fused(M, seq, s)
        cur = 0
        if self.recurrent:
            gp, sv, dg = self.gru_pack, self.rnn_saved, self.rnn_dgate
            H = self.hidden_sizes[-1]
            if self.gru_wide:
                from . import gru_wide
                gru_wide.backward(self, seq)
            else:
                call("harl_gru_bwd", ptr(self.dz[0]), ptr(seq["mask_rows"]), ptr(gp["Wih"]), ptr(gp["Whh"]), ptr(sv[0]),
                     ptr(sv[1]), ptr(sv[2]), ptr(sv[3]), ptr(sv[4]), H, seq["L"], seq["m_pad"], ptr(self.xh[-1]),
                     ptr(self.rmask[-1]), ptr(self.rstd[-1]), ptr(dg[0]), ptr(dg[1]), ptr(dg[2]), ptr(dg[3]), ptr(self.dz[1]), s,
                     tag="gru_bwd")
            import ctypes as C
            for gl in range(self.recurrent_n):
                dg_, sv_ = self.rnn_dgate_l[gl], self.rnn_saved_l[gl]
                xin = self.xh[-1] if gl == 0 else self.rnn_hraw_l[gl - 1]
                a6 = (C.c_void_p * 6)(*[ptr(t) for t in (dg_[0], dg_[1], dg_[2], dg_[0], dg_[1], dg_[3])])
                b6 = (C.c_void_p * 6)(*([ptr(xin)] * 3 + [ptr(sv_[0])] * 3))
                p6 = (C.c_void_p * 6)(*[ptr(self.part[po[L + 6 * gl + k]:]) for k in range(6)])
                call("harl_mlp_dw_partials_multi", 6, a6, b6, p6, H, H, M, nwg, s, tag="dw_gru")
            cur = 1
        if self.panel:
            for l in range(L - 1, -1, -1):
                b_in, k_in = (self.x0n, self.kp0) if l == 0 else (self.xh[l - 1], 256)
                call("harl_mlp_dw_partials", ptr(self.dz[cur]), 0, 0, 256, ptr(b_in), 0, 0, None, None, None, k_in, M,
                     ptr(self.part[po[l]:]), nwg, s, tag="dw_hidden" if l else "dw_input")
                if l > 0:
                    Wp, _ = self._packs[l]
                    call("harl_mlp_panel_bwd", ptr(self.dz[cur]), ptr(self.xh[l - 1]), ptr(self.rmask[l - 1]),
                         ptr(self.rstd[l - 1]), M, 256, 256, ptr(Wp), ptr(self.dz[1 - cur]), s, tag="bwd_panel")
                    cur = 1 - cur
            self._combine_partials(s)
            return
        if self.act_id:
            hs = self.hidden_sizes
            call("harl_act_bwd", ptr(self.dz[cur]), ptr(self.xh[L - 1]), ptr(self.amean[L - 1]), ptr(self.rstd[L - 1]), M, hs[L - 1],
                 self.act_id, s, tag="act_bwd")
            for l in range(L - 1, 0, -1):
                ho, hi = hs[l], hs[l - 1]
                call("harl_mlp_dw_partials", ptr(self.dz[cur]), 0, 0, ho, ptr(self.xh[l - 1]), 0, 0, None, None, None, hi, M,
                     ptr(self.part[po[l]:]), nwg, s, tag="dw_hidden")
                Wp, _ = self._packs[l]
                call("harl_mlp_bwd_dx", ptr(self.dz[cur]), ptr(self.xh[l - 1]), ptr(self.ones_mask), ptr(self.rstd[l - 1]), M, ho,
                     hi, ptr(Wp), ptr(self.dz[1 - cur]), None, 0, None, 0, s, tag="bwd_dx")
                cur = 1 - cur
                call("harl_act_bwd", ptr(self.dz[cur]), ptr(self.xh[l - 1]), ptr(self.amean[l - 1]), ptr(self.rstd[l - 1]), M, hi,
                     self.act_id, s, tag="act_bwd")
            call("harl_mlp_dw_partials", ptr(self.dz[cur]), 0, 0, hs[0], ptr(self.x0n), 0, 0, None, None, None, self.kp0, M,
                 ptr(self.part[po[0]:]), nwg, s, tag="dw_input")
            self._combine_partials(s)
            return
        fuse_dw1 = L >= 2 and self.x0n is not None and self.in_dim < self.kp0 and self.kp0 <= 64
        bwd_mode = _bwd_fused_mode(M)
        side_pending = False
        if (bwd_mode != "0" and fuse_dw1 and self.kp0 == 64 and L >= 2 and self.hidden_sizes[0] == 128 and self.hidden_sizes[1] == 128
                and os.environ.get("HARL_BWD_K64", "0") == "1"):
            fuse_dw1 = False
        for l in range(L - 1, 0, -1):
            ho, hi = self.hidden_sizes[l], self.hidden_sizes[l - 1]
            Wp, _ = self._packs[l]
            dw1_here = l == 1 and fuse_dw1
            if bwd_mode != "0" and ho == 128 and hi == 128 and (not dw1_here or self.kp0 == 32):
                call("harl_mlp_bwd_dx_dw", ptr(self.dz[cur]), ptr(self.xh[l - 1]), ptr(self.rmask[l - 1]), ptr(self.rstd[l - 1]), M,
                     ho, hi, ptr(Wp), None if dw1_here else ptr(self.dz[1 - cur]), ptr(self.x0n) if dw1_here else None,
                     self.kp0 if dw1_here else 0, ptr(self.part[po[0]:]) if dw1_here else None, ptr(self.part[po[l]:]), nwg,
                     int(bwd_mode != "nofill"), s, tag="bwd_full_dw1" if dw1_here else "bwd_full")
                cur = 1 - cur
                continue
            two = (_bwd_streams() and ho == 128 and hi == 128 and self.device_.type == "cuda"
                   and (not (l == 1 and fuse_dw1) or self.kp0 == 32))
            if side_pending and not (l == 1 and fuse_dw1):
                torch.cuda.current_stream(self.device_).wait_event(self._bwd_ev[1])
            if two:
                main_s, side_s, e0 = torch.cuda.current_stream(self.device_), self._bwd_side(), self._bwd_ev[0]
                e0.record(main_s)
            else:
                call("harl_mlp_dw_partials", ptr(self.dz[cur]), 0, 0, ho, ptr(self.xh[l - 1]), 0, 0, None, None, None, hi, M,
                     ptr(self.part[po[l]:]), nwg, s, tag="dw_hidden")
            if l == 1 and fuse_dw1:
                call("harl_mlp_bwd_dx", ptr(self.dz[cur]), ptr(self.xh[0]), ptr(self.rmask[0]), ptr(self.rstd[0]), M, ho, hi,
                     ptr(Wp), None, ptr(self.x0n), self.kp0, ptr(self.part[po[0]:]), nwg, s, tag="bwd_dx_dw1")
            else:
                call("harl_mlp_bwd_dx", ptr(self.dz[cur]), ptr(self.xh[l - 1]), ptr(self.rmask[l - 1]),
                     ptr(self.rstd[l - 1]), M, ho, hi, ptr(Wp), ptr(self.dz[1 - cur]), None, 0, None, 0, s, tag="bwd_dx")
            if two:
                side_s.wait_event(e0)
                with torch.cuda.stream(side_s):
                    call("harl_mlp_dw_partials", ptr(self.dz[cur]), 0, 0, ho, ptr(self.xh[l - 1]), 0, 0, None, None, None, hi, M,
                         ptr(self.part[po[l]:]), nwg, side_s.cuda_stream, tag="dw_hidden")
                self._bwd_ev[1].record(side_s)
                side_pending = True
            cur = 1 - cur
        h0 = self.hidden_sizes[0]
        use_ln = self.use_feature_normalization
        if fuse_dw1:
            pass
        elif self.x0n is not None:
            call("harl_mlp_dw_partials", ptr(self.dz[cur]), 0, 0, h0, ptr(self.x0n), 0, 0, None, None, None, self.kp0, M,
                 ptr(self.part[po[0]:]), nwg, s, tag="dw_input")
        else:
            call("harl_mlp_dw_partials", ptr(self.dz[cur]), 0, 0, h0, ptr(X), 1, X.shape[1], ptr(idx),
                 ptr(self.mu0) if use_ln else None, ptr(self.rstd0) if use_ln else None, self.in_dim, M,
                 ptr(self.part[po[0]:]), nwg, s, tag="dw_input")
        if side_pending:
            e1 = self._bwd_ev[1]
            e1.record(self._bwd_side())
            torch.cuda.current_stream(self.device_).wait_event(e1)
        self._combine_partials(s)

    def _backward_trunk_fused(self, M: int, seq: Optional[dict], s) -> None:
        import ctypes as C
        L, po, nwg = len(self.hidden_sizes), self._part_offs, self.n_wg
        spare = [self.dz[2]] if L == 3 else []
        if self.recurrent:
            gp, sv, dg = self.gru_pack, self.rnn_saved, self.rnn_dgate
            call("harl_gru_bwd", ptr(self.dz[0]), ptr(seq["mask_rows"]), ptr(gp["Wih"]), ptr(gp["Whh"]), ptr(sv[0]),
                 ptr(sv[1]), ptr(sv[2]), ptr(sv[3]), ptr(sv[4]), 64, seq["L"], seq["m_pad"], ptr(self.xh[-1]),
                 ptr(self.rmask[-1]), ptr(self.rstd[-1]), ptr(dg[0]), ptr(dg[1]), ptr(dg[2]), ptr(dg[3]), None, s, tag="gru_bwd")
            dzs = [self.dz[1], self.dz[0]] + spare
        else:
            dzs = [self.dz[0], self.dz[1]] + spare
        args = self._trunk_cache.get("bwd")
        if args is None:
            vp = lambda ts: (C.c_void_p * len(ts))(*[ptr(t) for t in ts])
            top_down = range(L - 1, -1, -1)
            a, b, part, K, t0, nt = [], [], [], [], [], []

            def add(aa, bb, l, k, t, n):
                a.append(aa), b.append(bb), part.append(self.part[po[l]:]), K.append(k), t0.append(t), nt.append(n)
            if self.recurrent:
                for k, (aa, bb) in enumerate(zip((dg[0], dg[1], dg[2], dg[0], dg[1], dg[3]), [self.xh[-1]] * 3 + [sv[0]] * 3)):
# ... 347 lines not shown
```

### harl_amd/traffic.py

```python
from __future__ import annotations

from typing import Callable, Dict, Optional, Sequence


def _act(H: int) -> float:
    return 4.0 * H + H / 8.0 + 4.0


def _kp(D: int) -> int:
    return 32 * ((int(D) + 31) // 32)


def _fwd_fused2x(a: Sequence) -> float:
    M, D, H, store1 = a[1], a[3], a[7], a[8]
    return M * (4.0 * _kp(D) + (_act(H) if store1 else 0.0) + _act(H))


def _fwd_fused2(a: Sequence) -> float:
    M, D, H, store1, x0n = a[3], a[4], a[10], a[11], a[20]
    return M * (4.0 * D + (8.0 if a[2] else 0.0) + (_act(H) if store1 else 0.0) + _act(H) + 8.0 + (4.0 * _kp(D) if x0n else 0.0))


def _fwd_hidden(a: Sequence) -> float:
    return a[1] * (4.0 * a[2] + _act(a[3]))


def _fwd_wide(a: Sequence) -> float:
    return a[1] * (4.0 * a[2] + _act(a[6]))


def _fwd_input(a: Sequence) -> float:
    return a[3] * (4.0 * a[4] + (8.0 if a[2] else 0.0) + _act(a[8]) + 8.0 + (4.0 * _kp(a[4]) if a[14] else 0.0))


def _x0n_wide(a: Sequence) -> float:
    return a[3] * (4.0 * a[4] + (8.0 if a[2] else 0.0) + 4.0 * _kp(a[4]) + 8.0)


def _tangent_wide(a: Sequence) -> float:
    return a[1] * (4.0 * a[2] + _act(a[6]) + 4.0 * a[6])


def _bwd_dx(a: Sequence) -> float:
    M, HO, HI = a[4], a[5], a[6]
    return M * (4.0 * HO + _act(HI) + (4.0 * HI if a[8] else 0.0) + (4.0 * a[10] if a[9] else 0.0))


def _bwd_dx_dw(a: Sequence) -> float:
    M, HO, HI = a[4], a[5], a[6]
    return M * (4.0 * HO + _act(HI) + (4.0 * HI if a[8] else 0.0) + (4.0 * a[10] if a[9] else 0.0))


def _dw_partials(a: Sequence) -> float:
    lda, HO, K, M = a[2], a[3], a[10], a[11]
    return M * (4.0 * (lda if a[1] else HO) + 4.0 * K)


def _dw_partials_multi(a: Sequence) -> float:
    n, HO, K, M = a[0], a[4], a[5], a[6]
    return n * M * (4.0 * HO + 4.0 * K)


def _gru_fwd(a: Sequence) -> float:
    H, L, m_pad, save = a[7], a[8], a[9], a[18]
    xin = 3 * 4.0 * H if (save & 2) else 4.0 * H
    return L * m_pad * (xin + 4.0 + 4.0 * H + 4.0 + (5 * 4.0 * H if (save & 1) else 0.0))


def _gru_bwd(a: Sequence) -> float:
    H, L, m_pad = a[9], a[10], a[11]
    if not a[19]:
        return L * m_pad * (6 * 4.0 * H + 4.0 + 4 * 4.0 * H)
    return L * m_pad * (6 * 4.0 * H + 4.0 + _act(H) + 4 * 4.0 * H + 4.0 * H)


def _nonnull(arr) -> int:
    return sum(1 for p in arr if p)


def _fwd_trunk(a: Sequence) -> float:
    M, KP, H = a[1], a[2], a[6]
    return M * (4.0 * KP + _nonnull(a[11]) * _act(H) + (3 * 4.0 * H if a[17] else 0.0))


def _bwd_trunk(a: Sequence) -> float:
    M, H, nh = a[0], a[1], a[2]
    top = (3 * 4.0 * H + _act(H) + 4.0 * H) if a[3] else 4.0 * H
    return M * (top + nh * (_act(H) + 4.0 * H))


def _dw_partials_multi_v(a: Sequence) -> float:
    n, HO, M = a[0], a[4], a[8]
    return M * sum(4.0 * HO + 4.0 * 32 * a[7][k] for k in range(n))


def _head_rows(discrete: int, act_dim: int, avail) -> float:
    w = 1 if discrete else act_dim
    return 4.0 * w + 4.0 * w + (4.0 * act_dim if avail else 0.0)


def _actor_head_loss(a: Sequence) -> float:
    M, H, disc, ad = a[3], a[4], a[10], a[11]
    w = 1 if disc else ad
    return M * (_act(H) + _head_rows(disc, ad, a[14]) + 4.0 + (4.0 if a[18] else 0.0) + (4.0 if a[19] else 0.0)
                + (4.0 * w if a[26] else 0.0) + 4.0 * H + (4.0 * 32 if (a[28] and not a[30]) else 0.0))


def _actor_head_logp(a: Sequence) -> float:
    M, H, disc, ad = a[1], a[2], a[8], a[9]
    w = 1 if disc else ad
    return M * (4.0 * H + 4.0 * w + (4.0 * ad if a[11] else 0.0) + (4.0 * w if a[12] else 0.0) + (4.0 * w if a[13] else 0.0)
                + (8.0 if a[14] else 0.0) + (4.0 * ad if a[16] else 0.0))


def _critic_head_loss(a: Sequence) -> float:
    return a[3] * (_act(a[4]) + 8.0 + 4.0 * a[4])


def _update_fwd_actor(a: Sequence) -> float:
    M, D, H, disc, ad = a[1], a[2], a[3], a[13], a[14]
    w = 1 if disc else ad
    return M * (4.0 * _kp(D) + _head_rows(disc, ad, a[16]) + 4.0 + (4.0 if a[20] else 0.0) + (4.0 if a[21] else 0.0)
                + (4.0 * w if a[26] else 0.0) + 4.0 * H + (_act(H) if a[31] else 0.0))


def _update_logp(a: Sequence) -> float:
    M, D, disc, ad = a[1], a[2], a[13], a[14]
    w = 1 if disc else ad
    return M * (4.0 * _kp(D) + 4.0 * w + (4.0 * ad if a[16] else 0.0) + (4.0 * w if a[17] else 0.0) + (4.0 * w if a[18] else 0.0)
                + (8.0 if a[19] else 0.0) + (4.0 * ad if a[21] else 0.0))


def _update_fwd_critic(a: Sequence) -> float:
    return a[1] * (4.0 * _kp(a[2]) + 8.0 + 4.0 * a[3] + (_act(a[3]) if a[21] else 0.0))


def _update_last_actor(a: Sequence) -> float:
    M, H, disc, ad = a[1], a[2], a[10], a[11]
    w = 1 if disc else ad
    return M * (4.0 * H + _head_rows(disc, ad, a[14]) + 4.0 + (4.0 if a[18] else 0.0) + (4.0 if a[19] else 0.0)
                + (4.0 * w if a[24] else 0.0) + 4.0 * H)


def _update_last_critic(a: Sequence) -> float:
    return a[1] * (4.0 * a[2] + 8.0 + 4.0 * a[2])


def _update_values(a: Sequence) -> float:
    return a[1] * (4.0 * _kp(a[2]) + 4.0)


def _update_bwd(a: Sequence) -> float:
    return a[2] * (4.0 * _kp(a[3]) + 4.0 * a[4])


def _panel_fwd(a: Sequence) -> float:
    return a[1] * (4.0 * a[2] + _act(a[6]))


def _panel_bwd(a: Sequence) -> float:
    return a[4] * (4.0 * a[5] + _act(a[6]) + 4.0 * a[6])


def _tangent_hidden(a: Sequence) -> float:
    return a[2] * (2 * 4.0 * a[3] + _act(a[4]) + 4.0 * a[4])


def _gae(a: Sequence) -> float:
    T, n = a[8], a[9]
    return 4.0 * n * (T + 3 * (T + 1) + (T + 1) + T)


ALGORITHMIC_BYTES: Dict[str, Callable[[Sequence], float]] = {
    "harl_mlp_fwd_fused2x": _fwd_fused2x,
    "harl_mlp_fwd_fused2": _fwd_fused2,
    "harl_mlp_fwd_hidden": _fwd_hidden,
    "harl_mlp_fwd_wide": _fwd_wide,
    "harl_mlp_fwd_input": _fwd_input,
    "harl_mlp_x0n_wide": _x0n_wide,
    "harl_mlp_tangent_wide": _tangent_wide,
    "harl_mlp_bwd_dx": _bwd_dx,
    "harl_mlp_bwd_dx_dw": _bwd_dx_dw,
    "harl_mlp_dw_partials": _dw_partials,
    "harl_mlp_dw_partials_multi": _dw_partials_multi,
    "harl_mlp_dw_partials_multi_v": _dw_partials_multi_v,
    "harl_gru_dw6": lambda a: a[7] * 6 * 4.0 * 64,
    "harl_mlp_fwd_trunk": _fwd_trunk,
    "harl_mlp_bwd_trunk": _bwd_trunk,
    "harl_gru_fwd": _gru_fwd,
    "harl_gru_bwd": _gru_bwd,
    "harl_actor_head_loss": _actor_head_loss,
    "harl_actor_head_logp": _actor_head_logp,
    "harl_critic_head_loss": _critic_head_loss,
    "harl_update_fwd_actor": _update_fwd_actor,
    "harl_update_logp": _update_logp,
    "harl_update_fwd_critic": _update_fwd_critic,
    "harl_update_values": _update_values,
    "harl_update_last_actor": _update_last_actor,
    "harl_update_last_critic": _update_last_critic,
    "harl_update_bwd": _update_bwd,
    "harl_gae_returns": _gae,
    "harl_mlp_panel_fwd": _panel_fwd,
    "harl_mlp_panel_bwd": _panel_bwd,
    "harl_mlp_tangent_hidden": _tangent_hidden,
    "harl_mlp_tangent_hidden2": _tangent_hidden,
}


def algorithmic_bytes(name: str, args: Sequence) -> Optional[float]:
    f = ALGORITHMIC_BYTES.get(name)
    return None if f is None else float(f(args))


def _f_fused2x(a):
    return 2.0 * a[1] * (a[3] * a[7] + a[7] * a[7])


def _f_fused2(a):
    return 2.0 * a[3] * (a[4] * a[10] + a[10] * a[10])


def _f_update_fwd_actor(a):
    M, D, H, ad = a[1], a[2], a[3], a[14]
    return 2.0 * M * (D * H + H * H + 3 * ad * H)


def _f_update_logp(a):
    M, D, H, ad = a[1], a[2], a[3], a[14]
    return 2.0 * M * (D * H + H * H + ad * H)


def _f_update_fwd_critic(a):
    M, D, H = a[1], a[2], a[3]
    return 2.0 * M * (D * H + H * H + 3 * H)


def _f_update_values(a):
    M, D, H = a[1], a[2], a[3]
    return 2.0 * M * (D * H + H * H + H)


def _f_update_last_actor(a):
    return 2.0 * a[1] * (a[2] * a[2] + 3 * a[11] * a[2])


def _f_update_last_critic(a):
    return 2.0 * a[1] * (a[2] * a[2] + 3 * a[2])


# ... 8 lines not shown


def _f_bwd_dx_dw(a):
    M, HO, HI = a[4], a[5], a[6]
    return 2.0 * M * (2 * HO * HI + (HI * a[10] if a[9] else 0))


def _f_dw(a):
    return 2.0 * a[11] * a[3] * a[10]


def _f_dw_multi(a):
    return 2.0 * a[0] * a[6] * a[4] * a[5]


def _f_gru_fwd(a):
    H, L, m_pad = a[7], a[8], a[9]
    return 2.0 * L * m_pad * (3 if (a[18] & 2) else 6) * H * H


def _f_gru_bwd(a):
    H, L, m_pad = a[9], a[10], a[11]
    return 2.0 * L * m_pad * (6 if a[19] else 3) * H * H


def _f_fwd_trunk(a):
    M, D, H, nh = a[1], a[4], a[6], a[8]
    return 2.0 * M * (D * H + nh * H * H + (3 * H * H if a[17] else 0))


def _f_bwd_trunk(a):
    M, H, nh = a[0], a[1], a[2]
    return 2.0 * M * ((3 * H * H if a[3] else 0) + nh * H * H)


def _f_head(a_M, a_H, ad, train):
    return 2.0 * a_M * ad * a_H * (3 if train else 1)


ALGORITHMIC_FLOPS: Dict[str, Callable[[Sequence], float]] = {
    "harl_mlp_fwd_fused2x": _f_fused2x,
    "harl_mlp_fwd_fused2": _f_fused2,
    "harl_mlp_fwd_hidden": lambda a: 2.0 * a[1] * a[2] * a[3],
    "harl_mlp_linear": lambda a: 2.0 * a[1] * a[2] * a[3],
    "harl_mlp_linear3": lambda a: 3 * 2.0 * a[3] * a[4] * a[5],
    "harl_mlp_fwd_wide": lambda a: 2.0 * a[1] * a[4] * a[6],
    "harl_mlp_linear_wide": lambda a: 2.0 * a[1] * a[4] * a[6],
    "harl_mlp_fwd_input": lambda a: 2.0 * a[3] * a[4] * a[8],
    "harl_mlp_tangent_wide": lambda a: 2.0 * a[1] * a[4] * a[6],
    "harl_mlp_tangent_hidden": lambda a: 2.0 * 2 * a[2] * a[3] * a[4],
    "harl_mlp_tangent_hidden2": lambda a: 2.0 * 2 * a[2] * a[3] * a[4],
    "harl_mlp_bwd_dx": _f_bwd_dx,
    "harl_mlp_bwd_dx_dw": _f_bwd_dx_dw,
    "harl_mlp_dw_partials": _f_dw,
    "harl_mlp_dw_partials_multi": _f_dw_multi,
    "harl_mlp_dw_partials_multi_v": lambda a: 2.0 * a[8] * a[4] * 32 * sum(a[7][k] for k in range(a[0])),
    "harl_gru_dw6": lambda a: 2.0 * a[7] * 6 * 64 * 64,
    "harl_mlp_fwd_trunk": _f_fwd_trunk,
    "harl_mlp_bwd_trunk": _f_bwd_trunk,
    "harl_mlp_panel_fwd": lambda a: 2.0 * a[1] * a[4] * a[6],
    "harl_mlp_panel_bwd": lambda a: 2.0 * a[4] * a[5] * a[6],
    "harl_gru_fwd": _f_gru_fwd,
    "harl_gru_bwd": _f_gru_bwd,
    "harl_actor_head_loss": lambda a: _f_head(a[3], a[4], a[11], True) - (2.0 * a[3] * a[11] * a[4] if not a[30] else 0.0),
    "harl_actor_head_logp": lambda a: _f_head(a[1], a[2], a[9], False),
    "harl_actor_head_fvp": lambda a: 0.0,
    "harl_critic_head_loss": lambda a: _f_head(a[3], a[4], 1, True),
    "harl_update_fwd_actor": _f_update_fwd_actor,
    "harl_update_logp": _f_update_logp,
    "harl_update_fwd_critic": _f_update_fwd_critic,
    "harl_update_values": _f_update_values,
    "harl_update_last_actor": _f_update_last_actor,
    "harl_update_last_critic": _f_update_last_critic,
    "harl_update_bwd": _f_update_bwd,
}


def algorithmic_flops(name: str, args: Sequence) -> Optional[float]:
    f = ALGORITHMIC_FLOPS.get(name)
    if f is None:
        return None
    try:
        return float(f(args))
    except (TypeError, IndexError):
        return None
```

### harl_amd/v_critic.py

```python
from __future__ import annotations

import os
from typing import Optional

import torch

from . import _lib
from ._lib import PS_STRIDE, call, ptr, stream
from .buffers import OnPolicyCriticBufferEP, consume_randperm, minibatch_indices, rng_sync
from .dist import Comm, local_minibatch_rows
from .nets import FusedAdam, VNet, build_seq
from .valuenorm import ValueNorm, _as_dev


class VCritic:
    def __init__(self, args, cent_obs_space, device=torch.device("cuda:0")):
        self.args = args
        self.device = torch.device(device)
        _lib.require_gpu(self.device)
        self.tpdv = dict(dtype=torch.float32, device=self.device)
        self.clip_param = args["clip_param"]
        self.critic_epoch = args["critic_epoch"]
        self.critic_num_mini_batch = args["critic_num_mini_batch"]
        self.data_chunk_length = args["data_chunk_length"]
# ... 35 lines not shown
        if net.fused_update_ok(None, train=False):
            call("harl_update_values", *net.fused_args(x, M), ptr(out), stream(), tag="update_values")
            return out, (None if rnn_states_critic is None else _as_dev(rnn_states_critic, self.device))
        if not net.recurrent:
            net.forward_trunk(x, None, M, for_backward=False)
            call("harl_critic_head_values", ptr(net.xh[-1]), M, net.hidden_sizes[-1], ptr(Wp), ptr(bp), ptr(out), stream())
            return out, (None if rnn_states_critic is None else _as_dev(rnn_states_critic, self.device))
        H = net.hidden_sizes[-1]
        h0 = _as_dev(rnn_states_critic, self.device)
        m = h0.shape[0]
        HS = H * net.recurrent_n
        seq = build_seq(self.device, M // m, m, HS, h0=h0.reshape(m, HS), masks_src=_as_dev(masks, self.device),
                        want_h_last=True)
        Mp = seq["L"] * seq["m_pad"]
        net.forward_trunk(x, seq["idx"], Mp, for_backward=False, seq=seq)
        fx, _, _, fh = net.feat()
        outp = out if seq["idx"] is None else torch.empty(Mp, 1, **self.tpdv)
        call("harl_critic_head_values", ptr(fx), Mp, fh, ptr(Wp), ptr(bp), ptr(outp), stream())
        if seq["idx"] is not None:
            out.copy_(outp.reshape(seq["L"], seq["m_pad"], 1)[:, :m].reshape(M, 1))
        return out, seq["h_last"][:m].reshape(m, net.recurrent_n, H).clone()

    def _update_core(self, share_obs, idx, m, m_global, value_preds, returns, vn: Optional[ValueNorm], seq=None):
        net = self.critic
        s = stream()
        if vn is not None:
            vidx = seq["valid_idx"] if seq is not None else idx
            vn.update(returns, vidx, count=m_global, reduce_fn=self.comm.all_reduce_sum if self.comm.enabled else None,
                      local_count=(seq["L"] * seq["m"] if seq is not None else m))
        net._ensure_ws(max(m, 1))
        sc = net.scalars
        self._forward_backward(net, share_obs, idx, m, value_preds, returns, vn, seq, s)
        nblk = net.n_wg if m > 0 else 0
        ps_kw = dict(part_scalars=net.part_scalars, n_scalar_blocks=nblk)
        if self.comm.enabled:
            if m <= 0:
                net.dwp.zero_()
            hilo = net.dwp_msg[net.total_dwp:]
            call("harl_reduce_pack_scalars", ptr(net.part_scalars), nblk, ptr(sc), ptr(hilo), s)
            self.comm.all_reduce_message(net.dwp_msg)
            ps_kw = dict(scalars_hilo=hilo)
        scale = float(self.value_loss_coef) / float(m_global)
        if self._state_tap is not None:
            o = self.critic_optimizer
            self._state_tap.append((net.flat_param.clone(), o.exp_avg.clone(), o.exp_avg_sq.clone(), o.step_count))
        self.critic_optimizer.step(1, scale, self.use_max_grad_norm, self.max_grad_norm, self._info, **ps_kw)
        if self._trace is not None:
            self._trace.append(self._info.clone())
        if self._grad_tap is not None:
            self._grad_tap(net.flat_grad * scale, sc.clone())

    def _forward_backward(self, net, share_obs, idx, m, value_preds, returns, vn, seq, s) -> None:
        if m > 0 and net.fused_update_ok(idx, seq):
            call("harl_update_fwd_critic", *net.fused_args(share_obs, m), ptr(value_preds), ptr(returns),
                 ptr(vn.stats) if vn is not None else None, float(self.clip_param), int(self.use_clipped_value_loss),
                 int(self.use_huber_loss), float(self.huber_delta), ptr(net.dz[0]), ptr(net.part_scalars),
                 ptr(net.part[net._part_offs[-1]:]), net.n_wg, *net.hybrid_outputs(), s, tag="update_fwd_critic")
            net.backward_after_fused(share_obs, m)
        elif m > 0 and net.fused_last_ok(idx, seq):
            L = len(net.hidden_sizes)
            net.forward_trunk(share_obs, idx, m, upto=L - 1)
            (Wl, bl), (Wh, bh) = net._packs[L - 1], net._packs[-1]
            call("harl_update_last_critic", ptr(net.xh[L - 2]), m, net.hidden_sizes[-1], ptr(Wl), ptr(bl), ptr(Wh), ptr(bh),
                 ptr(idx), ptr(value_preds), ptr(returns), ptr(vn.stats) if vn is not None else None, float(self.clip_param),
                 int(self.use_clipped_value_loss), int(self.use_huber_loss), float(self.huber_delta), ptr(net.dz[0]),
                 ptr(net.part_scalars), ptr(net.part[net._part_offs[-1]:]), net.n_wg, s, tag="update_last_critic")
            net.backward_trunk(share_obs, idx, m, head_dw_done=True)
        elif m > 0:
            net.forward_trunk(share_obs, idx, m, seq=seq)
            Wp, bp = net._packs[-1]
            fx, fmask, frstd, fh = net.feat()
            mv, mp = (seq["m"], seq["m_pad"]) if seq is not None else (0, 0)
            call("harl_critic_head_loss", ptr(fx), ptr(fmask), ptr(frstd), m, fh,
                 ptr(Wp), ptr(bp), ptr(idx), ptr(value_preds), ptr(returns), ptr(vn.stats) if vn is not None else None,
                 float(self.clip_param), int(self.use_clipped_value_loss), int(self.use_huber_loss), float(self.huber_delta),
                 mv, mp, ptr(net.dz[0]), ptr(net.dhead), ptr(net.part_scalars), ptr(net.part[net._part_offs[-1]:]),
                 net.n_wg, s, tag="critic_head_loss")
            net.backward_trunk(share_obs, idx, m, seq=seq, head_dw_done=True)

    def update(self, sample, value_normalizer=None):
        share_obs, _rnn, value_preds, returns, _masks = sample
        dev = self.device
        x = _as_dev(share_obs, dev)
        m = x.shape[0]
        before = self._info.clone()
        self.critic.fold()
        if self.critic.recurrent:
            HS = self.critic.hidden_sizes[-1] * self.critic.recurrent_n
            h0 = _as_dev(_rnn, dev)
            seq = build_seq(dev, m // h0.shape[0], h0.shape[0], HS, h0=h0.reshape(-1, HS), masks_src=_as_dev(_masks, dev))
            self._update_core(x.reshape(m, -1), seq["idx"], seq["L"] * seq["m_pad"], m, _as_dev(value_preds, dev).reshape(m),
                              _as_dev(returns, dev).reshape(m), value_normalizer, seq=seq)
            d = self._info - before
            return d[0], d[1]
        self._update_core(x.reshape(m, -1), None, m, m, _as_dev(value_preds, dev).reshape(m),
                          _as_dev(returns, dev).reshape(m), value_normalizer)
        d = self._info - before
        return d[0], d[1]

    def train(self, critic_buffer: OnPolicyCriticBufferEP, value_normalizer: Optional[ValueNorm] = None, _defer=False):
        for _ in self._train_epochs(critic_buffer, value_normalizer):
            pass
        return self._train_result(_defer)

    def _train_result(self, _defer: bool):
        n_upd = self.critic_epoch * self.critic_num_mini_batch
        if _defer:
            return self._info / n_upd
        rng_sync()
        vals = (self._info / n_upd).cpu().tolist()
        return {"value_loss": vals[0], "critic_grad_norm": vals[1]}
# ... 48 lines not shown
```

### include/harl_hip.h

```cpp
#ifndef HARL_HIP_H
#define HARL_HIP_H

#include <stdint.h>

#ifdef __cplusplus
extern "C" {
#endif

#define HARL_PS_STRIDE 48
#define HARL_DHEAD_LD 32
#define HARL_MD_MAX_HEADS 8
#define HARL_MD_MAX_GROUPS 4
#define HARL_MM_SCRATCH_BYTES 24640
#define HARL_CG_SCRATCH_BYTES 1088

int harl_version(void);
const char *harl_last_error(void);

int harl_gae_returns(const float *rewards, float *value_preds, const float *masks, const float *bad_masks,
                     const float *next_value, const float *vn_stats, float *returns, float *advantages,
                     int T, int ncols, float gamma, float gamma_lambda, int use_gae,
                     int use_proper_time_limits, int fp_order, void *stream);

int harl_masked_moments(const float *x, const float *active, long n, double *out3, void *scratch, void *stream);
// ... 4 lines not shown
int harl_moments_mean(const double *moments3, float *mean_out, void *stream);
int harl_build_seq(const int64_t *first, int m, int m_pad, int L, long stride, const float *masks_src, const float *h0_src,
                   int H, int64_t *idx, int64_t *valid_idx, float *mask_rows, float *h0, void *stream);
int harl_clock_probe(long long *cycles_ticks, long ticks, void *stream);
int harl_adv_normalize(const float *adv, const double *moments3, float *adv_out, long n, void *stream);

int harl_factor_update(float *factor, const float *new_logp, const float *old_logp, long n, int act_dim,
                       int agg_mean, void *stream);

int harl_sum_sumsq(const float *x, const int64_t *idx, long m, double *sums2, void *stream);
int harl_valuenorm_apply(float *vn_stats, const double *sums2, double count, double beta, void *stream);

int harl_gradnorm_clip_adam(float *param, float *grad, float *exp_avg, float *exp_avg_sq, long n,
                            const float *grad_scale, int use_clip, float max_norm, double lr, double beta1,
                            double beta2, float eps, float weight_decay, double bias_correction1,
                            double bias_correction2, double *info_out, void *stream);

int harl_fold_linear(const float *W, const float *b, const float *gamma, const float *beta, float *Wp,
                     float *bp, int out_dim, int in_dim, void *stream);
int harl_unfold_linear_grads(const float *dWp, const float *dbp, int ldp, const float *W, const float *gamma,
                             const float *beta, float *dW, float *db, float *dgamma, float *dbeta,
                             int out_dim, int in_dim, int accumulate, void *stream);

int harl_mlp_fwd_input(const float *X, long ldx, const int64_t *idx, long M, int D, const float *Wp,
                       const float *bp, int use_ln0, int H, float *xout, uint32_t *relu_mask, float *rstd,
                       float *mu0, float *rstd0, float *x0n, void *stream);
int harl_mlp_x0n_wide(const float *X, long ldx, const int64_t *idx, long M, int D, int use_ln0, float *x0n, float *mu0,
                      float *rstd0, void *stream);
int harl_mlp_fwd_wide(const float *x0n, long M, int KP, const float *Wp, int D, const float *bp, int H, void *w_img,
                      float *xout, uint32_t *relu_mask, float *rstd, void *stream);
int harl_mlp_panel_fwd(const float *xin, long M, int KP, const float *Wp, int D, const float *bp, int HO, float *xout,
                       uint32_t *relu_mask, float *rstd, void *stream);
int harl_head_dw_rows256(const float *dhead, long M, int act_dim, const float *xhat, float *part, int n_wg, void *stream);
int harl_mlp_panel_tangent(const float *xin_dot, const float *xin, long M, int KP, const float *Wp, const float *Wdp, int D,
                           const float *bdp, const float *xprimal, const uint32_t *mask_in, const float *rstd_in,
                           float *xout_dot, void *stream);
int harl_mlp_panel_bwd(const float *dz, const float *xprev, const uint32_t *relu_mask_prev, const float *rstd_prev, long M,
                       int HO, int HI, const float *Wp, float *dz_prev, void *stream);
int harl_mlp_fwd_fused2x(const float *x0n, long M, const float *W1p, int D, const float *b1p, const float *W2p,
                         const float *b2p, int H, int store1, float *x1out, uint32_t *mask1, float *rstd1, float *x2out,
                         uint32_t *mask2, float *rstd2, void *stream);
int harl_mlp_fwd_fused2(const float *X, long ldx, const int64_t *idx, long M, int D, const float *W1p,
                        const float *b1p, int use_ln0, const float *W2p, const float *b2p, int H, int store1,
                        float *x1out, uint32_t *mask1, float *rstd1, float *mu0, float *rstd0, float *x2out,
                        uint32_t *mask2, float *rstd2, float *x0n, void *stream);
int harl_mlp_fwd_hidden(const float *xin, long M, int HI, int HO, const float *Wp, const float *bp,
                        float *xout, uint32_t *relu_mask, float *rstd, void *stream);
int harl_mlp_bwd_dx(const float *dz, const float *xprev, const uint32_t *relu_mask_prev, const float *rstd_prev,
                    long M, int HO, int HI, const float *Wp, float *dz_prev, const float *x0n, int kp0, float *dw_part,
                    int n_wg, void *stream);
int harl_mlp_bwd_dx_dw(const float *dz, const float *xprev, const uint32_t *relu_mask_prev, const float *rstd_prev,
                       long M, int HO, int HI, const float *Wp, float *dz_prev, const float *x0n, int kp0, float *dw1_part,
                       float *dw2_part, int n_wg, int fill, void *stream);
int harl_mlp_dw_partials(const float *a, int a_kind, int lda, int HO, const float *b, int b_kind, long ldx,
                         const int64_t *idx, const float *mu0, const float *rstd0, int K, long M, float *part,
                         int n_wg, void *stream);
int harl_mlp_dw_partials_multi(int n, const float *const *a, const float *const *b, float *const *part, int HO, int K,
                               long M, int n_wg, void *stream);
int harl_mlp_dw_partials_multi_v(int n, const float *const *a, const float *const *b, float *const *part, int HO, const int *K,
                                 const int *tile0, const int *nt, long M, int n_wg, void *stream);
int harl_gru_dw6(const float *dr, const float *dz, const float *dn, const float *dhn, const float *xhat, const float *hpm,
                 float *const *part, long M, int n_wg, void *stream);
int harl_mlp_fwd_trunk(const float *x0n, long M, int KP, const float *W1p, int D, const float *b1p, int H, void *w_img,
                       int n_hidden, const float *const *Wp, const float *const *bp, float *const *xout,
                       uint32_t *const *relu_mask, float *const *rstd, const float *Wih, const float *bih, const float *bhh,
                       float *gi_ws, void *stream);
int harl_mlp_bwd_trunk(long M, int H, int n_hidden, const float *Wih, const float *dr, const float *dzg, const float *dn,
                       const float *dz_in, const float *const *Wp, const float *const *xh, const uint32_t *const *relu_mask,
                       const float *const *rstd, float *const *dz_out, void *stream);
int harl_reduce_partials(const float *part, int n_wg, long elems, float *out, void *stream);

#define HARL_TABLE_STRIDE 12
int harl_reduce_partials_multi(const float *part, const int *table, int n_layers, int n_wg, long total_elems,
                               float *dwp, void *stream);
int harl_fold_table(const float *param, float *packs, const int *table, int n_layers, int total_rows, void *stream);
int harl_unfold_table(const float *param, float *grad, const float *dwp, const int *table, int n_layers, int total_cols,
                      void *stream);
int harl_fold_tangent_table(const float *param, const float *vec, float *pack_d, const int *table, int n_layers,
                            int total_rows, void *stream);
int harl_pack_scalars_hilo(const double *scalars, float *hilo, void *stream);
int harl_reduce_pack_scalars(const float *part_scalars, int n_blocks, double *scalars, float *hilo, void *stream);
int harl_adam_fold(float *param, float *grad, float *exp_avg, float *exp_avg_sq, long n, const float *dwp,
                   const int *table, int n_layers, float *packs, double *scalars, const float *part_scalars,
                   int n_scalar_blocks, const float *scalars_hilo, int mode, float const_scale, int logstd_off,
                   int act_dim, double *info,
                   int use_clip, float max_norm, double lr, double beta1, double beta2, float eps, float weight_decay,
                   double bias_correction1, double bias_correction2, void *ws, void *stream);

int harl_actor_head_logp(const float *xL, long M, int H, const float *Whp, const float *bhp,
                         const float *log_std, float std_x_coef, float std_y_coef, int discrete, int act_dim,
                         const float *actions, const float *avail, float *logp_out, const float *old_logp,
                         float *factor, int agg_mean, float *head_out, long m_valid, long m_pad, void *stream);
int harl_actor_head_loss(const float *xL, const uint32_t *relu_mask, const float *rstd, long M, int H,
                         const float *Whp, const float *bhp, const float *log_std, float std_x_coef,
                         float std_y_coef, int discrete, int act_dim, const int64_t *idx, const float *actions,
                         const float *avail, const float *old_logp, const float *adv, const double *adv_moments,
                         const float *factor, const float *active, double clip_param, float entropy_coef,
                         int agg_mean, int trpo, long m_valid, long m_pad, float *logp_out, float *dzL, float *dhead,
                         float *part_scalars, float *dw_part, int n_wg, void *stream);
int harl_critic_head_values(const float *xL, long M, int H, const float *Whp, const float *bhp, float *values,
                            void *stream);
int harl_critic_head_loss(const float *xL, const uint32_t *relu_mask, const float *rstd, long M, int H,
                          const float *Whp, const float *bhp, const int64_t *idx, const float *value_preds,
                          const float *returns, const float *vn_stats, float clip_param, int use_clipped,
                          int use_huber, float huber_delta, long m_valid, long m_pad, float *dzL, float *dhead,
                          float *part_scalars, float *dw_part, int n_wg, void *stream);
// ... 24 lines not shown
                             const float *Wdp, const float *bdp, void *w_img, const float *xprimal,
                             const uint32_t *mask_in, const float *rstd_in, float *xout_dot, void *stream);
int harl_actor_head_fvp(const float *xL, const float *xLdot, const uint32_t *relu_mask, const float *rstd, long M, int H,
                        const float *Whp, const float *bhp, const float *Whdp, const float *bhdp, const float *log_std,
                        float std_x_coef, float std_y_coef, int discrete, int act_dim, const float *avail, long m_valid,
                        long m_pad, float *dzL, float *dhead, void *stream);
int harl_trpo_fvp_finish(const float *grad, const float *vec, const float *log_std, float *out, long n, float m_global,
                         float damping, long logstd_off, int act_dim, float std_x_coef, float std_y_coef, void *stream);
int harl_trpo_cg_step(float *x, float *r, float *p, const float *avp, long n, float *state, void *scratch, void *stream);
#define HARL_TRPO_STATE 16
int harl_trpo_begin(const float *grad_sum, const double *scalars, long logstd_off, int act_dim, float *g, float *x, float *r,
                    float *p, long n, float *cg_state, double *st, void *scratch, void *stream);
int harl_trpo_step(const float *x, const float *fx, const float *g, const float *theta, float *theta_save, float *full_step,
                   long n, float kl_threshold, double *st, void *scratch, void *stream);
int harl_trpo_ls_candidate(const float *theta_save, const float *full_step, const double *st, float *theta, long n, void *stream);
int harl_trpo_ls_test(const double *scalars, double *kl_sum, double m_global, double kl_threshold, double accept_ratio,
                      double backtrack_coeff, double *st, void *stream);
int harl_reduce_scalars_set(const float *part_scalars, int n_blocks, double *scalars, void *stream);
int harl_zero_bytes(void *p, long bytes, void *stream);
int harl_trpo_kl_sum(const float *head_old, const float *head_new, const float *log_std_old, const float *log_std_new,
                     float std_x_coef, float std_y_coef, long M, int act_dim, int discrete, double *out_sum,
                     void *stream);

int harl_mlp_linear(const float *xin, long M, int HI, int HO, const float *Wp, const float *bp, float *xout, void *stream);
int harl_mlp_linear3(const float *x0, const float *x1, const float *x2, long M, int HI, int HO, const float *W0, const float *W1,
                     const float *W2, const float *b0, const float *b1, const float *b2, float *o0, float *o1, float *o2,
                     void *stream);
int harl_md_head_logp(const float *const *z, int n_groups, const int *sp, int n_heads, const int *nvec,
                      const int *head_group, long M, const float *actions, float *logp_out, const float *old_logp,
                      int old_w, float *factor, int agg_mean, float *head_out, long m_valid, long m_pad, void *stream);
int harl_md_head_loss(const float *const *z, float *const *dz, int n_groups, const int *sp, int n_heads, const int *nvec,
                      const int *head_group, long M, const int64_t *idx, const float *actions, const float *old_logp,
                      int old_w, const float *adv, const double *adv_moments, const float *factor, const float *active,
                      const float *ent_scale, double clip_param, float entropy_coef, int agg_mean, int mode, long m_valid,
                      long m_pad, float *logp_out, float *part_scalars, int n_blocks, void *stream);

int harl_update_supported(int D, int H, int act_dim, int kind);
int harl_update_fwd_actor(const float *x0n, long M, int D, int H, const float *W1p, const float *b1p, const float *W2p,
                          const float *b2p, const float *Whp, const float *bhp, const float *log_std, float std_x_coef,
                          float std_y_coef, int discrete, int act_dim, const float *actions, const float *avail,
                          const float *old_logp, const float *adv, const double *adv_moments, const float *factor,
                          const float *active, double clip_param, float entropy_coef, int agg_mean, int trpo,
                          float *logp_out, float *dz2, float *part_scalars, float *dw_part_head, int n_part_rows,
                          float *xh1, uint32_t *rmask1, float *rstd1, void *stream);
int harl_update_logp(const float *x0n, long M, int D, int H, const float *W1p, const float *b1p, const float *W2p,
                     const float *b2p, const float *Whp, const float *bhp, const float *log_std, float std_x_coef,
                     float std_y_coef, int discrete, int act_dim, const float *actions, const float *avail,
                     float *logp_out, const float *old_logp, float *factor, int agg_mean, float *head_out, void *stream);
int harl_update_fwd_critic(const float *x0n, long M, int D, int H, const float *W1p, const float *b1p, const float *W2p,
                           const float *b2p, const float *Whp, const float *bhp, const float *value_preds,
                           const float *returns, const float *vn_stats, float clip_param, int use_clipped, int use_huber,
                           float huber_delta, float *dz2, float *part_scalars, float *dw_part_head, int n_part_rows,
                           float *xh1, uint32_t *rmask1, float *rstd1, void *stream);
int harl_update_last_actor(const float *xin, long M, int H, const float *Wp, const float *bp, const float *Whp,
                           const float *bhp, const float *log_std, float std_x_coef, float std_y_coef, int discrete,
                           int act_dim, const int64_t *idx, const float *actions, const float *avail,
                           const float *old_logp, const float *adv, const double *adv_moments, const float *factor,
                           const float *active, double clip_param, float entropy_coef, int agg_mean, int trpo,
                           float *logp_out, float *dz, float *part_scalars, float *dw_part_head, int n_part_rows,
                           void *stream);
int harl_update_last_critic(const float *xin, long M, int H, const float *Wp, const float *bp, const float *Whp,
                            const float *bhp, const int64_t *idx, const float *value_preds, const float *returns,
                            const float *vn_stats, float clip_param, int use_clipped, int use_huber, float huber_delta,
                            float *dz, float *part_scalars, float *dw_part_head, int n_part_rows, void *stream);
int harl_update_values(const float *x0n, long M, int D, int H, const float *W1p, const float *b1p, const float *W2p,
                       const float *b2p, const float *Whp, const float *bhp, float *values, void *stream);
int harl_update_bwd(const float *x0n, const float *dz2, long M, int D, int H, const float *W1p, const float *b1p,
                    const float *W2p, float *dw_part1, float *dw_part2, int n_part_rows, void *stream);

int harl_gru_fwd(const float *xin, const float *mask_rows, const float *h0, const float *Wih, const float *bih,
                 const float *Whh, const float *bhh, int H, int L, long m_pad, float *y, float *rstd_y, float *hpm, float *r,
                 float *z, float *n, float *hn, float *h_last, int save, float *gi_ws, void *stream);
int harl_gru_cell_init(const float *h0, const float *mask_rows, int H, long m_pad, float *hpm0, void *stream);
int harl_gru_cell_fwd(const float *gi_r, const float *gi_z, const float *gi_n, const float *gh_r, const float *gh_z,
                      const float *gh_n, const float *hpm, const float *mask_next, int H, long m_pad, float *r, float *z,
                      float *n, float *hn, float *h, float *hpm_next, float *h_last, void *stream);
int harl_gru_cell_bwd(const float *dh_out, const float *t_r, const float *t_z, const float *t_n, const float *mask_next,
                      const float *r, const float *z, const float *n, const float *hn, const float *hpm, int H, long m_pad,
                      float *gz, float *dr, float *dz, float *dn, float *dhn, void *stream);
int harl_rownorm(const float *x, long M, int H, float *y, float *rstd, void *stream);
int harl_gru_cell_tangent(const float *gia_r, const float *gia_z, const float *gia_n, const float *gib_r, const float *gib_z,
                          const float *gib_n, const float *gha_r, const float *gha_z, const float *gha_n, const float *ghb_r,
                          const float *ghb_z, const float *ghb_n, const float *r, const float *z, const float *n,
                          const float *hn, const float *hpm, const float *hpm_dot, const float *mask_next, int H, long m_pad,
                          float *h_dot, float *hpm_dot_next, void *stream);
int harl_gru_bwd(const float *dhout, const float *mask_rows, const float *Wih, const float *Whh, const float *hpm,
                 const float *r, const float *z, const float *n, const float *hn, int H, int L, long m_pad,
                 const float *xmlp, const uint32_t *mask_mlp, const float *rstd_mlp, float *dr, float *dz, float *dn,
                 float *dhn, float *dz_mlp, void *stream);

int harl_head_blocks(long M);
int harl_reduce_scalars(const float *part_scalars, int n_blocks, double *scalars, void *stream);

int harl_randperm_replay(const uint8_t *state_in, long state_bytes, long n, int32_t *out, uint32_t *scratch,
                         uint8_t *state_out);
int harl_rng_advance(const uint8_t *state_in, long state_bytes, long n_draws, uint8_t *state_out);
int harl_rng_jump(const uint8_t *state_in, long state_bytes, long n_draws, uint8_t *state_out);

int harl_comm_create(int world, int rank, long cap_bytes, int n_blocks, void *handle_out, void *ctx_out);
int harl_comm_connect(void *ctx, const void *all_handles);
int harl_comm_allreduce(void *ctx, void *msg, long n, int is_f64, void *stream);
int harl_comm_set_timeout(void *ctx, double seconds);
int harl_comm_status(void *ctx);
int harl_comm_destroy(void *ctx);

#ifdef __cplusplus
// ... 4 lines not shown
```

Before: 52.67 million.

## Emit dz as pre-split three-part MFMA image from fused forward for backward kernel

```diff
diff --git a/harl_amd/_lib.py b/harl_amd/_lib.py
--- a/harl_amd/_lib.py
+++ b/harl_amd/_lib.py
@@ -45,6 +45,8 @@
     "harl_mlp_fwd_hidden": [_vp, _l, _i, _i, _vp, _vp, _vp, _vp, _vp, _vp],
     "harl_mlp_bwd_dx": [_vp, _vp, _vp, _vp, _l, _i, _i, _vp, _vp, _vp, _i, _vp, _i, _vp],
     "harl_mlp_bwd_dx_dw": [_vp, _vp, _vp, _vp, _l, _i, _i, _vp, _vp, _vp, _i, _vp, _vp, _i, _i, _vp],
+    "harl_mlp_bwd_dx_dw_split": [_vp, _vp, _vp, _vp, _l, _i, _i, _vp, _vp, _vp, _i, _vp, _vp, _i, _i, _vp],
+    "harl_dz_presplit_supported": [],
     "harl_mlp_dw_partials": [_vp, _i, _i, _i, _vp, _i, _l, _vp, _vp, _vp, _i, _l, _vp, _i, _vp],
     "harl_mlp_dw_partials_multi": [_i, _vp, _vp, _vp, _i, _i, _l, _i, _vp],
     "harl_mlp_dw_partials_multi_v": [_i, _vp, _vp, _vp, _i, _vp, _vp, _vp, _l, _i, _vp],
@@ -81,6 +83,8 @@
     "harl_trpo_kl_sum": [_vp, _vp, _vp, _vp, _f, _f, _l, _i, _i, _vp, _vp],
     "harl_update_supported": [_i, _i, _i, _i],
     "harl_update_fwd_actor": [_vp, _l, _i, _i] + [_vp] * 7 + [_f, _f, _i, _i] + [_vp] * 7 + [_d, _f, _i, _i] + [_vp] * 4 + [_i] + [_vp] * 4,
+    "harl_update_fwd_actor_split": [_vp, _l, _i, _i] + [_vp] * 7 + [_f, _f, _i, _i] + [_vp] * 7 + [_d, _f, _i, _i] + [_vp] * 4 + [_i] + [_vp] * 4,
+    "harl_update_fwd_critic_split": [_vp, _l, _i, _i] + [_vp] * 9 + [_f, _i, _i, _f] + [_vp] * 3 + [_i] + [_vp] * 4,
     "harl_update_logp": [_vp, _l, _i, _i] + [_vp] * 7 + [_f, _f, _i, _i] + [_vp] * 5 + [_i, _vp, _vp],
     "harl_update_last_actor": [_vp, _l, _i] + [_vp] * 5 + [_f, _f, _i, _i] + [_vp] * 8 + [_d, _f, _i, _i] + [_vp] * 4 + [_i, _vp],
     "harl_update_last_critic": [_vp, _l, _i] + [_vp] * 8 + [_f, _i, _i, _f] + [_vp] * 3 + [_i, _vp],
diff --git a/harl_amd/csrc/heads_common.h b/harl_amd/csrc/heads_common.h
--- a/harl_amd/csrc/heads_common.h
+++ b/harl_amd/csrc/heads_common.h
@@ -1,5 +1,6 @@
 #pragma once
 #include "common.h"
+#include "split_mfma.h"
 
 using namespace harl;
 
@@ -184,7 +185,7 @@
   }
 }
 
-template <int H, int DAP, int DA = DAP, bool PACKED = false, bool WT = false>
+template <int H, int DAP, int DA = DAP, bool PACKED = false, bool WT = false, bool SPLIT_IMG = false>
 __device__ __forceinline__ void head_bwd_regs_bits(const f32x4 (&xs)[H / 8], uint32_t b0, const uint32_t b1, float rstd,
                                                    long slab, int lane, const float *whl ,
                                                    const float (&dzh)[DAP], float s1, float s2,
@@ -208,7 +209,10 @@
     for (int t = 0; t < H / 32; ++t)
       acc[t] = __builtin_amdgcn_mfma_f32_32x32x2f32(wa[WT ? 16 * t + 2 * st * (H / 2) : 16 * t * DAP + 2 * st], bsel, acc[t], 0, 0, 0);
   }
+  static_assert(!SPLIT_IMG || (PACKED && H == 128), "the split image exists for the fused kernel's 128-wide layers");
   f32x4 *op = reinterpret_cast<f32x4 *>(dz_out + slab * (long)(H * SLAB)) + lane;
+  u32x4 *ip = reinterpret_cast<u32x4 *>(dz_out) + slab * (long)(3 * (H / 16) * WAVE) + lane;
+  u32x4 t1, t2, t3;
   const float c1 = -s1 * rstd, c2 = -s2 * rstd;
   const f32x2 c1v = {c1, c1}, c2v = {c2, c2}, rv = {rstd, rstd};
 #pragma unroll
@@ -235,7 +239,23 @@
         b0 <<= 1;
       }
     }
-    op[q * WAVE] = o;
+    if constexpr (SPLIT_IMG) {
+#pragma unroll
+      for (int P = 0; P < 2; ++P) {
+        unsigned a, b, d;
+        split3<false>(o[2 * P], o[2 * P + 1], a, b, d);
+        t1[2 * (q & 1) + P] = a;
+        t2[2 * (q & 1) + P] = b;
+        t3[2 * (q & 1) + P] = d;
+      }
+      if (q & 1) {
+        ip[(q >> 1) * WAVE] = t1;
+        ip[(H / 16 + (q >> 1)) * WAVE] = t2;
+        ip[(2 * (H / 16) + (q >> 1)) * WAVE] = t3;
+      }
+    } else {
+      op[q * WAVE] = o;
+    }
   }
 }
 
diff --git a/harl_amd/csrc/mlp.hip b/harl_amd/csrc/mlp.hip
--- a/harl_amd/csrc/mlp.hip
+++ b/harl_amd/csrc/mlp.hip
@@ -1486,13 +1486,18 @@
 #ifndef HARL_BWD_SPLIT_WAVES
 #define HARL_BWD_SPLIT_WAVES 1
 #endif
-template <int KT, bool FILL>
-__global__ __launch_bounds__(2 * WG_THREADS, 1) void k_bwd_dx_dw8(
+#ifndef HARL_DZ_PRESPLIT
+#define HARL_DZ_PRESPLIT 1
+#endif
+constexpr long DZ_IMG_SLAB = 3 * 8 * WAVE;
+template <int KT, bool FILL, bool IMG>
+__device__ __forceinline__ void bwd_dx_dw8_body(
     const float *__restrict__ dz, const float *__restrict__ xprev, const uint32_t *__restrict__ mask_prev,
     const float *__restrict__ rstd_prev, const float *__restrict__ Wp, float *__restrict__ dz_prev, long n_slabs,
     const float *__restrict__ x0n, float *__restrict__ dw1_part, float *__restrict__ dw2_part, int n_part_rows) {
   constexpr int H = 128, MT = 4, NJ = 8, NR = 64, KPF = 32, NTH = 2 * WG_THREADS;
   extern __shared__ __attribute__((aligned(16))) float lds[];
+  const u32x4 *__restrict__ dzi = reinterpret_cast<const u32x4 *>(dz);
   PHASE_BEGIN();
   u32x4 *img = reinterpret_cast<u32x4 *>(lds);
   unsigned char *Bb = reinterpret_cast<unsigned char *>(img + 3 * MT * NJ * 64);
@@ -1533,25 +1538,33 @@
   u32x4 At[3][2], AtN[3][2];
   float rr0 = 0.f, rr1 = 0.f;
   auto d_load = [&](long ds) {
+    if constexpr (IMG) {
+#pragma unroll
+      for (int t = 0; t < 3; ++t)
+#pragma unroll
+        for (int c = 0; c < 2; ++c) ya[t][c] = (dzi + ds * DZ_IMG_SLAB + lane)[(t * NJ + 2 * wave + c) * WAVE];
+    }
 #pragma unroll
     for (int u = 0; u < 4; ++u) {
-      prA[u] = (reinterpret_cast<const f32x4 *>(dz + ds * (long)(H * SLAB)) + lane)[(4 * wave + u) * WAVE];
+      if constexpr (!IMG) prA[u] = (reinterpret_cast<const f32x4 *>(dz + ds * (long)(H * SLAB)) + lane)[(4 * wave + u) * WAVE];
       prB[u] = (reinterpret_cast<const f32x4 *>(xprev + ds * (long)(H * SLAB)) + lane)[(4 * wave + u) * WAVE];
     }
   };
   float vnext = 1.f;
   auto d_load_next = [&](long ds, long fallback) { d_load(ds < n_slabs ? ds : fallback); };
   auto a_chunk = [&](int k) {
-    const int pi = k >> 1, j = pi >> 2, c = pi & 3, u = pi >> 1, e = 2 * (pi & 1);
-    if ((k & 1) == 0) {
-      unsigned p1;
-      split_stage1(prA[u][e], prA[u][e + 1], p1, rr0, rr1);
-      ya[0][j][c] = p1;
-    } else {
-      unsigned p2, p3;
-      split_stage2(rr0, rr1, p2, p3);
-      ya[1][j][c] = p2;
-      ya[2][j][c] = p3;
+    if constexpr (!IMG) {
+      const int pi = k >> 1, j = pi >> 2, c = pi & 3, u = pi >> 1, e = 2 * (pi & 1);
+      if ((k & 1) == 0) {
+        unsigned p1;
+        split_stage1(prA[u][e], prA[u][e + 1], p1, rr0, rr1);
+        ya[0][j][c] = p1;
+      } else {
+        unsigned p2, p3;
+        split_stage2(rr0, rr1, p2, p3);
+        ya[1][j][c] = p2;
+        ya[2][j][c] = p3;
+      }
     }
   };
   auto b_chunk = [&](int k) {
@@ -1607,16 +1620,18 @@
   float raw[NR];
   u32x4 g1[NJ], g2[NJ], g3[NJ];
   auto o_chunk = [&](int k) {
-    const int pi = k >> 1, j = pi >> 2, c = pi & 3;
-    if ((k & 1) == 0) {
-      unsigned p1;
-      split_stage1(raw[2 * pi], raw[2 * pi + 1], p1, rr0, rr1);
-      g1[j][c] = p1;
-    } else {
-      unsigned p2, p3;
-      split_stage2(rr0, rr1, p2, p3);
-      g2[j][c] = p2;
-      g3[j][c] = p3;
+    if constexpr (!IMG) {
+      const int pi = k >> 1, j = pi >> 2, c = pi & 3;
+      if ((k & 1) == 0) {
+        unsigned p1;
+        split_stage1(raw[2 * pi], raw[2 * pi + 1], p1, rr0, rr1);
+        g1[j][c] = p1;
+      } else {
+        unsigned p2, p3;
+        split_stage2(rr0, rr1, p2, p3);
+        g2[j][c] = p2;
+        g3[j][c] = p3;
+      }
     }
   };
   if (!owner && base0 < n_slabs) {
@@ -1646,14 +1661,21 @@
       if (base + k < n_slabs) __builtin_amdgcn_s_barrier();
     };
     if (own) {
-      constexpr int RAW_LEAD = 3;
+      constexpr int RAW_LEAD = IMG && KT > 0 ? 2 : 3;
       auto raw_ks = [&](int j) {
-        const f32x4 *p = reinterpret_cast<const f32x4 *>(dz + slab * (long)(H * SLAB)) + lane;
-#pragma unroll
-        for (int c = 0; c < 2; ++c) {
-          const f32x4 v = p[(2 * j + c) * WAVE];
-#pragma unroll
-          for (int e = 0; e < 4; ++e) raw[8 * j + 4 * c + e] = v[e];
+        if constexpr (IMG) {
+          const u32x4 *p = dzi + slab * DZ_IMG_SLAB + lane;
+          g1[j] = p[j * WAVE];
+          g2[j] = p[(NJ + j) * WAVE];
+          g3[j] = p[(2 * NJ + j) * WAVE];
+        } else {
+          const f32x4 *p = reinterpret_cast<const f32x4 *>(dz + slab * (long)(H * SLAB)) + lane;
+#pragma unroll
+          for (int c = 0; c < 2; ++c) {
+            const f32x4 v = p[(2 * j + c) * WAVE];
+#pragma unroll
+            for (int e = 0; e < 4; ++e) raw[8 * j + 4 * c + e] = v[e];
+          }
         }
       };
 #pragma unroll
@@ -1751,8 +1773,10 @@
             if constexpr (s_ >= 16 && s_ < 32) a_chunk(s_ - 16);
             else if constexpr (s_ >= 32 && s_ < 42) b_chunk(s_ - 32 + 6);
             else if constexpr (s_ >= 42) p_chunk(s_ - 42);
+            if constexpr (IMG && s_ == 42) b_store((r + 1) & 1);
             if constexpr (s_ == 47) d_load_next(ds2, base);
           } else {
+            if constexpr (IMG && s_ == 26) b_store((r + 1) & 1);
             if constexpr (s_ < 16) a_chunk(s_);
             else if constexpr (s_ < 26) b_chunk(s_ - 16 + 6);
             else if constexpr (s_ < 32) p_chunk(s_ - 26);
@@ -1783,7 +1807,7 @@
           });
         });
         PHASE(6);
-        b_store((r + 1) & 1);
+        if constexpr (!IMG) b_store((r + 1) & 1);
 #pragma unroll
         for (int t = 0; t < 3; ++t) {
           At[t][0] = AtN[t][0];
@@ -1832,6 +1856,23 @@
   PHASE_END_BY(4, 0);
   PHASE_END_BY(5, 64 * WAVES_PER_WG);
 }
+
+template <int KT, bool FILL>
+__global__ __launch_bounds__(2 * WG_THREADS, 1) void k_bwd_dx_dw8(
+    const float *__restrict__ dz, const float *__restrict__ xprev, const uint32_t *__restrict__ mask_prev,
+    const float *__restrict__ rstd_prev, const float *__restrict__ Wp, float *__restrict__ dz_prev, long n_slabs,
+    const float *__restrict__ x0n, float *__restrict__ dw1_part, float *__restrict__ dw2_part, int n_part_rows) {
+  bwd_dx_dw8_body<KT, FILL, false>(dz, xprev, mask_prev, rstd_prev, Wp, dz_prev, n_slabs, x0n, dw1_part, dw2_part, n_part_rows);
+}
+#if HARL_DZ_PRESPLIT
+template <int KT, bool FILL>
+__global__ __launch_bounds__(2 * WG_THREADS, 1) void k_bwd_dx_dw8s(
+    const float *__restrict__ dz, const float *__restrict__ xprev, const uint32_t *__restrict__ mask_prev,
+    const float *__restrict__ rstd_prev, const float *__restrict__ Wp, float *__restrict__ dz_prev, long n_slabs,
+    const float *__restrict__ x0n, float *__restrict__ dw1_part, float *__restrict__ dw2_part, int n_part_rows) {
+  bwd_dx_dw8_body<KT, FILL, true>(dz, xprev, mask_prev, rstd_prev, Wp, dz_prev, n_slabs, x0n, dw1_part, dw2_part, n_part_rows);
+}
+#endif
 
 HARL_PHASE_ACCESSOR(mlp)
 
@@ -2114,10 +2155,10 @@
   return check_launch("harl_mlp_bwd_dx");
 }
 
-extern "C" int harl_mlp_bwd_dx_dw(const float *dz, const float *xprev, const uint32_t *relu_mask_prev,
-                                  const float *rstd_prev, long M, int HO, int HI, const float *Wp, float *dz_prev,
-                                  const float *x0n, int kp0, float *dw1_part, float *dw2_part, int n_wg, int fill,
-                                  void *stream) {
+static int bwd_dx_dw_launch(const float *dz, bool dz_split, const float *xprev, const uint32_t *relu_mask_prev,
+                            const float *rstd_prev, long M, int HO, int HI, const float *Wp, float *dz_prev,
+                            const float *x0n, int kp0, float *dw1_part, float *dw2_part, int n_wg, int fill,
+                            void *stream) {
   if (M <= 0) return 0;
   if (HO != 128 || HI != 128) return bad("harl_mlp_bwd_dx_dw: 128 x 128 layers only (the layer kernels take the other widths)");
   if (!dw2_part || n_wg <= 0) return bad("harl_mlp_bwd_dx_dw: needs the partial arena of dW' and n_wg > 0");
@@ -2145,11 +2186,46 @@
                        rstd_prev, Wp, dz_prev, n_slabs, x0n, dw1_part, dw2_part, n_wg);                              \
   }
 #endif
+#if HARL_BWD_SPLIT_WAVES && HARL_DZ_PRESPLIT
+#define LS(kt, fl)                                                                                                    \
+  {                                                                                                                   \
+    allow_big_lds(k_bwd_dx_dw8s<kt, fl>, shm);                                                                        \
+    hipLaunchKernelGGL((k_bwd_dx_dw8s<kt, fl>), dim3(grid), dim3(2 * WG_THREADS), shm, s, dz, xprev, relu_mask_prev, \
+                       rstd_prev, Wp, dz_prev, n_slabs, x0n, dw1_part, dw2_part, n_wg);                              \
+  }
+  if (dz_split) {
+    if (first) { if (fill) LS(1, true) else LS(1, false) }
+    else { if (fill) LS(0, true) else LS(0, false) }
+    return check_launch("harl_mlp_bwd_dx_dw_split");
+  }
+#undef LS
+#else
+  if (dz_split) return bad("harl_mlp_bwd_dx_dw_split: this build has no split-image backward (HARL_DZ_PRESPLIT=0)");
+#endif
   if (first) { if (fill) LB(1, true) else LB(1, false) }
   else { if (fill) LB(0, true) else LB(0, false) }
 #undef LB
   return check_launch("harl_mlp_bwd_dx_dw");
 }
+
+extern "C" int harl_mlp_bwd_dx_dw(const float *dz, const float *xprev, const uint32_t *relu_mask_prev,
+                                  const float *rstd_prev, long M, int HO, int HI, const float *Wp, float *dz_prev,
+                                  const float *x0n, int kp0, float *dw1_part, float *dw2_part, int n_wg, int fill,
+                                  void *stream) {
+  return bwd_dx_dw_launch(dz, false, xprev, relu_mask_prev, rstd_prev, M, HO, HI, Wp, dz_prev, x0n, kp0, dw1_part, dw2_part, n_wg,
+                          fill, stream);
+}
+
+extern "C" int harl_mlp_bwd_dx_dw_split(const void *dz_img, const float *xprev, const uint32_t *relu_mask_prev,
+                                        const float *rstd_prev, long M, int HO, int HI, const float *Wp, float *dz_prev,
+                                        const float *x0n, int kp0, float *dw1_part, float *dw2_part, int n_wg, int fill,
+                                        void *stream) {
+  if (!dz_img) return bad("harl_mlp_bwd_dx_dw_split: missing image");
+  return bwd_dx_dw_launch(static_cast<const float *>(dz_img), true, xprev, relu_mask_prev, rstd_prev, M, HO, HI, Wp, dz_prev, x0n,
+                          kp0, dw1_part, dw2_part, n_wg, fill, stream);
+}
+
+extern "C" int harl_dz_presplit_supported() { return HARL_BWD_SPLIT_WAVES && HARL_DZ_PRESPLIT ? 1 : 0; }
 
 template <int MT, int NT>
 static void launch_dw_tr(const float *a, const float *b, long n_slabs, float *part, int K, int tile0, int n_wg, hipStream_t s) {
diff --git a/harl_amd/csrc/update.hip b/harl_amd/csrc/update.hip
--- a/harl_amd/csrc/update.hip
+++ b/harl_amd/csrc/update.hip
@@ -284,8 +284,12 @@
   }
 }
 
-template <int H, int KP0, int DA, bool DISCRETE, bool TRAIN, typename ARGS>
+#ifndef HARL_DZ_PRESPLIT
+#define HARL_DZ_PRESPLIT 1
+#endif
+template <int H, int KP0, int DA, bool DISCRETE, bool TRAIN, typename ARGS, bool DZ_IMG = false>
 __global__ __launch_bounds__(UF_THREADS, 2) void k_upd_fwd(UpdFwdArgs U, ARGS A) {
+  static_assert(!DZ_IMG || (TRAIN && H == 128), "the split image of dz_2: optimiser steps of 128-wide layers");
   constexpr bool CRITIC = std::is_same<ARGS, CriticArgs>::value;
   static_assert(DA >= 1 && DA <= 8 && (!CRITIC || DA == 1), "the LDS head-gradient tile covers 8 head outputs");
   constexpr int DAP = DA <= 4 ? 4 : 8;
@@ -505,7 +509,7 @@
       }
       PHASE(7);
       if constexpr (!EARLY_X0N) atl_load<2 * NXR>(U.x0n, sn, lane, xr);
-      head_bwd_regs_bits<H, DAP, DA, true, true>(xs, bits2[0], bits2[NW - 1], r2, slab, lane, whlT, dzh, s1, s2, U.dz2);
+      head_bwd_regs_bits<H, DAP, DA, true, true, DZ_IMG>(xs, bits2[0], bits2[NW - 1], r2, slab, lane, whlT, dzh, s1, s2, U.dz2);
       PHASE(8);
     }
   }
@@ -578,22 +582,23 @@
 
 constexpr size_t LDS_PER_WG_MAX = 160 * 1024;
 
-template <int H, int KP0, int DA, bool DISC, bool TRAIN, typename ARGS>
+template <int H, int KP0, int DA, bool DISC, bool TRAIN, typename ARGS, bool DZ_IMG = false>
 int launch_fwd(const UpdFwdArgs &U, const ARGS &A, hipStream_t s) {
   const size_t shm = fwd_lds_bytes(H, KP0, DA <= 4 ? 4 : 8, TRAIN ? DA : 0, DA);
   if (shm > LDS_PER_WG_MAX) {
     return bad("harl_update_*: this (D, H, act_dim) does not fit the LDS of one workgroup");
   }
-  allow_big_lds(k_upd_fwd<H, KP0, DA, DISC, TRAIN, ARGS>, shm);
-  hipLaunchKernelGGL((k_upd_fwd<H, KP0, DA, DISC, TRAIN, ARGS>), dim3(fwd_grid(U.n_slabs)), dim3(UF_THREADS), shm, s, U, A);
+  allow_big_lds(k_upd_fwd<H, KP0, DA, DISC, TRAIN, ARGS, DZ_IMG>, shm);
+  hipLaunchKernelGGL((k_upd_fwd<H, KP0, DA, DISC, TRAIN, ARGS, DZ_IMG>), dim3(fwd_grid(U.n_slabs)), dim3(UF_THREADS), shm, s, U, A);
   return 0;
 }
 
-template <int H, int KP0, bool TRAIN, int DA = 8>
+template <int H, int KP0, bool TRAIN, int DA = 8, bool DZ_IMG = false>
 int launch_actor_width(const UpdFwdArgs &U, const ActorArgs &A, int discrete, hipStream_t s) {
   if (A.act_dim == DA)
-    return discrete ? launch_fwd<H, KP0, DA, true, TRAIN, ActorArgs>(U, A, s) : launch_fwd<H, KP0, DA, false, TRAIN, ActorArgs>(U, A, s);
-  if constexpr (DA > 1) return launch_actor_width<H, KP0, TRAIN, DA - 1>(U, A, discrete, s);
+    return discrete ? launch_fwd<H, KP0, DA, true, TRAIN, ActorArgs, DZ_IMG>(U, A, s)
+                    : launch_fwd<H, KP0, DA, false, TRAIN, ActorArgs, DZ_IMG>(U, A, s);
+  if constexpr (DA > 1) return launch_actor_width<H, KP0, TRAIN, DA - 1, DZ_IMG>(U, A, discrete, s);
   return bad("harl_update_*: act_dim must be in [1, 8]");
 }
 
@@ -612,6 +617,27 @@
   return bad("harl_update_fwd: hidden width must be 64 or 128");
 }
 
+int dispatch_fwd_actor_split(const UpdFwdArgs &U, const ActorArgs &A, int H, int discrete, hipStream_t s) {
+#if HARL_DZ_PRESPLIT
+  if (A.act_dim < 1 || A.act_dim > 8) return bad("harl_update_fwd_actor_split: act_dim must be in [1, 8]");
+  if (H != 128 || U.D > 32) return bad("harl_update_fwd_actor_split: 128-wide layers, inputs <= 32 wide");
+  const int rc = launch_actor_width<128, 32, true, 8, true>(U, A, discrete, s);
+  return rc ? rc : check_launch("harl_update_fwd_actor_split");
+#else
+  return bad("harl_update_fwd_actor_split: this build has no split image (HARL_DZ_PRESPLIT=0)");
+#endif
+}
+
+int dispatch_fwd_critic_split(const UpdFwdArgs &U, const CriticArgs &A, int H, hipStream_t s) {
+#if HARL_DZ_PRESPLIT
+  if (H != 128 || U.D > 32) return bad("harl_update_fwd_critic_split: 128-wide layers, inputs <= 32 wide");
+  const int rc = launch_fwd<128, 32, 1, false, true, CriticArgs, true>(U, A, s);
+  return rc ? rc : check_launch("harl_update_fwd_critic_split");
+#else
+  return bad("harl_update_fwd_critic_split: this build has no split image (HARL_DZ_PRESPLIT=0)");
+#endif
+}
+
 int dispatch_last_actor(const UpdFwdArgs &U, const ActorArgs &A, int H, int discrete, hipStream_t s) {
   const int D = A.act_dim;
   if (D < 1 || D > 8) return bad("harl_update_last_actor: act_dim must be in [1, 8]");
@@ -654,14 +680,14 @@
   return fwd_lds_bytes(H, D == 0 ? 0 : (D <= 32 ? 32 : 64), dap, hrows, kind == 2 ? 1 : act_dim) <= LDS_PER_WG_MAX ? 1 : 0;
 }
 
-extern "C" int harl_update_fwd_actor(const float *x0n, long M, int D, int H, const float *W1p, const float *b1p,
-                                     const float *W2p, const float *b2p, const float *Whp, const float *bhp,
-                                     const float *log_std, float std_x_coef, float std_y_coef, int discrete, int act_dim,
-                                     const float *actions, const float *avail, const float *old_logp, const float *adv,
-                                     const double *adv_moments, const float *factor, const float *active,
-                                     double clip_param, float entropy_coef, int agg_mean, int trpo, float *logp_out,
-                                     float *dz2, float *part_scalars, float *dw_part_head, int n_part_rows, float *xh1,
-                                     uint32_t *rmask1, float *rstd1, void *stream) {
+static int update_fwd_actor(bool dz_split, const float *x0n, long M, int D, int H, const float *W1p, const float *b1p,
+                            const float *W2p, const float *b2p, const float *Whp, const float *bhp,
+                            const float *log_std, float std_x_coef, float std_y_coef, int discrete, int act_dim,
+                            const float *actions, const float *avail, const float *old_logp, const float *adv,
+                            const double *adv_moments, const float *factor, const float *active,
+                            double clip_param, float entropy_coef, int agg_mean, int trpo, float *logp_out,
+                            float *dz2, float *part_scalars, float *dw_part_head, int n_part_rows, float *xh1,
+                            uint32_t *rmask1, float *rstd1, void *stream) {
   if (M <= 0) return 0;
   if (D < 1 || D > 64) return bad("harl_update_fwd_actor: input width must be <= 64");
   if (!dz2 || !part_scalars || !dw_part_head || n_part_rows <= 0) return bad("harl_update_fwd_actor: missing outputs");
@@ -678,7 +704,36 @@
   A.factor_in = factor; A.active = active; A.entropy_coef = entropy_coef;
   A.clip_lo = (float)(1.0 - clip_param); A.clip_hi = (float)(1.0 + clip_param);
   A.agg_mean = agg_mean; A.part_scalars = part_scalars; A.n_slabs = U.n_slabs;
+  if (dz_split) return dispatch_fwd_actor_split(U, A, H, discrete, (hipStream_t)stream);
   return dispatch_fwd_actor<true>(U, A, H, discrete, (hipStream_t)stream);
+}
+
+extern "C" int harl_update_fwd_actor(const float *x0n, long M, int D, int H, const float *W1p, const float *b1p,
+                                     const float *W2p, const float *b2p, const float *Whp, const float *bhp,
+                                     const float *log_std, float std_x_coef, float std_y_coef, int discrete, int act_dim,
+                                     const float *actions, const float *avail, const float *old_logp, const float *adv,
+                                     const double *adv_moments, const float *factor, const float *active,
+                                     double clip_param, float entropy_coef, int agg_mean, int trpo, float *logp_out,
+                                     float *dz2, float *part_scalars, float *dw_part_head, int n_part_rows, float *xh1,
+                                     uint32_t *rmask1, float *rstd1, void *stream) {
+  return update_fwd_actor(false, x0n, M, D, H, W1p, b1p, W2p, b2p, Whp, bhp, log_std, std_x_coef, std_y_coef, discrete, act_dim,
+                          actions, avail, old_logp, adv, adv_moments, factor, active, clip_param, entropy_coef, agg_mean, trpo,
+                          logp_out, dz2, part_scalars, dw_part_head, n_part_rows, xh1, rmask1, rstd1, stream);
+}
+
+extern "C" int harl_update_fwd_actor_split(const float *x0n, long M, int D, int H, const float *W1p, const float *b1p,
+                                           const float *W2p, const float *b2p, const float *Whp, const float *bhp,
+                                           const float *log_std, float std_x_coef, float std_y_coef, int discrete,
+                                           int act_dim, const float *actions, const float *avail, const float *old_logp,
+                                           const float *adv, const double *adv_moments, const float *factor,
+                                           const float *active, double clip_param, float entropy_coef, int agg_mean,
+                                           int trpo, float *logp_out, void *dz2_img, float *part_scalars,
+                                           float *dw_part_head, int n_part_rows, float *xh1, uint32_t *rmask1,
+                                           float *rstd1, void *stream) {
+  return update_fwd_actor(true, x0n, M, D, H, W1p, b1p, W2p, b2p, Whp, bhp, log_std, std_x_coef, std_y_coef, discrete, act_dim,
+                          actions, avail, old_logp, adv, adv_moments, factor, active, clip_param, entropy_coef, agg_mean, trpo,
+                          logp_out, static_cast<float *>(dz2_img), part_scalars, dw_part_head, n_part_rows, xh1, rmask1, rstd1,
+                          stream);
 }
 
 extern "C" int harl_update_logp(const float *x0n, long M, int D, int H, const float *W1p, const float *b1p,
@@ -699,12 +754,12 @@
   return dispatch_fwd_actor<false>(U, A, H, discrete, (hipStream_t)stream);
 }
 
-extern "C" int harl_update_fwd_critic(const float *x0n, long M, int D, int H, const float *W1p, const float *b1p,
-                                      const float *W2p, const float *b2p, const float *Whp, const float *bhp,
-                                      const float *value_preds, const float *returns, const float *vn_stats,
-                                      float clip_param, int use_clipped, int use_huber, float huber_delta, float *dz2,
-                                      float *part_scalars, float *dw_part_head, int n_part_rows, float *xh1,
-                                      uint32_t *rmask1, float *rstd1, void *stream) {
+static int update_fwd_critic(bool dz_split, const float *x0n, long M, int D, int H, const float *W1p, const float *b1p,
+                             const float *W2p, const float *b2p, const float *Whp, const float *bhp,
+                             const float *value_preds, const float *returns, const float *vn_stats,
+                             float clip_param, int use_clipped, int use_huber, float huber_delta, float *dz2,
+                             float *part_scalars, float *dw_part_head, int n_part_rows, float *xh1,
+                             uint32_t *rmask1, float *rstd1, void *stream) {
   if (M <= 0) return 0;
   if (D < 1 || D > 64) return bad("harl_update_fwd_critic: input width must be <= 64");
   if (!dz2 || !part_scalars || !dw_part_head || n_part_rows <= 0) return bad("harl_update_fwd_critic: missing outputs");
@@ -717,7 +772,30 @@
   A.huber_delta = huber_delta; A.use_clipped = use_clipped; A.use_huber = use_huber;
   A.part_scalars = part_scalars; A.n_slabs = U.n_slabs;
   A.dw_part = dw_part_head;
+  if (dz_split) return dispatch_fwd_critic_split(U, A, H, (hipStream_t)stream);
   return dispatch_fwd_critic<true>(U, A, H, (hipStream_t)stream);
+}
+
+extern "C" int harl_update_fwd_critic(const float *x0n, long M, int D, int H, const float *W1p, const float *b1p,
+                                      const float *W2p, const float *b2p, const float *Whp, const float *bhp,
+                                      const float *value_preds, const float *returns, const float *vn_stats,
+                                      float clip_param, int use_clipped, int use_huber, float huber_delta, float *dz2,
+                                      float *part_scalars, float *dw_part_head, int n_part_rows, float *xh1,
+                                      uint32_t *rmask1, float *rstd1, void *stream) {
+  return update_fwd_critic(false, x0n, M, D, H, W1p, b1p, W2p, b2p, Whp, bhp, value_preds, returns, vn_stats, clip_param,
+                           use_clipped, use_huber, huber_delta, dz2, part_scalars, dw_part_head, n_part_rows, xh1, rmask1, rstd1,
+                           stream);
+}
+
+extern "C" int harl_update_fwd_critic_split(const float *x0n, long M, int D, int H, const float *W1p, const float *b1p,
+                                            const float *W2p, const float *b2p, const float *Whp, const float *bhp,
+                                            const float *value_preds, const float *returns, const float *vn_stats,
+                                            float clip_param, int use_clipped, int use_huber, float huber_delta,
+                                            void *dz2_img, float *part_scalars, float *dw_part_head, int n_part_rows,
+                                            float *xh1, uint32_t *rmask1, float *rstd1, void *stream) {
+  return update_fwd_critic(true, x0n, M, D, H, W1p, b1p, W2p, b2p, Whp, bhp, value_preds, returns, vn_stats, clip_param,
+                           use_clipped, use_huber, huber_delta, static_cast<float *>(dz2_img), part_scalars, dw_part_head,
+                           n_part_rows, xh1, rmask1, rstd1, stream);
 }
 
 extern "C" int harl_update_last_actor(const float *xin, long M, int H, const float *Wp, const float *bp, const float *Whp,
diff --git a/harl_amd/happo.py b/harl_amd/happo.py
--- a/harl_amd/happo.py
+++ b/harl_amd/happo.py
@@ -218,12 +218,13 @@
         if net.fused_update_ok(idx, seq):
             fa = net.fused_args(obs, m)
             self._await_factor()
-            call("harl_update_fwd_actor", *fa, ptr(net.log_std()), net.std_x_coef, net.std_y_coef, int(net.discrete),
+            split = net.dz_split_ok(m)
+            call("harl_update_fwd_actor_split" if split else "harl_update_fwd_actor", *fa, ptr(net.log_std()), net.std_x_coef, net.std_y_coef, int(net.discrete),
                  net.act_dim, ptr(actions), ptr(avail), ptr(old_logp), ptr(adv), ptr(adv_moments), ptr(factor),
                  ptr(active), float(self.clip_param), float(self.entropy_coef), int(self.action_aggregation == "mean"),
-                 self._surrogate_mode, ptr(logp_out), ptr(net.dz[0]), ptr(net.part_scalars),
+                 self._surrogate_mode, ptr(logp_out), ptr(net.dzimg if split else net.dz[0]), ptr(net.part_scalars),
                  ptr(net.part[net._part_offs[-1]:]), net.n_wg, *net.hybrid_outputs(), s, tag="update_fwd")
-            net.backward_after_fused(obs, m)
+            net.backward_after_fused(obs, m, dz_split=split)
             return net.n_wg
         if net.fused_last_ok(idx, seq):
             L = len(net.hidden_sizes)
diff --git a/harl_amd/nets.py b/harl_amd/nets.py
--- a/harl_amd/nets.py
+++ b/harl_amd/nets.py
@@ -31,6 +31,15 @@
     m = os.environ.get("HARL_BWD_FUSED", "auto")
     if m not in ("0", "1", "nofill", "auto"):
         raise ValueError(f"HARL_BWD_FUSED={m!r}: expected auto, 0, 1 or nofill")
+    if m == "auto":
+        return "1" if M >= BWD_FUSED_MIN_ROWS else "0"
+    return m
+
+
+def _dz_split_mode(M: int = 0) -> str:
+    m = os.environ.get("HARL_DZ_SPLIT", "auto")
+    if m not in ("0", "1", "auto"):
+        raise ValueError(f"HARL_DZ_SPLIT={m!r}: expected auto, 0 or 1")
     if m == "auto":
         return "1" if M >= BWD_FUSED_MIN_ROWS else "0"
     return m
@@ -312,6 +321,7 @@
             self.amean = [torch.empty(mp, dtype=f32, device=dev) for _ in self.hidden_sizes]
             self.ones_mask = torch.full((n_slabs * 64 * 2,), -1, dtype=u32, device=dev)
         self.dz = [torch.empty(mp * hmax, dtype=f32, device=dev) for _ in range(3 if len(self.hidden_sizes) == 3 and self.trunk_fused() else 2)]
+        self.dzimg = None
         self._trunk_cache = {}
         self.wide_head = (not self.md) and self._layers()[-1][4] > 32
         self.dhead = torch.zeros(mp * (64 if self.wide_head else DHEAD_LD), dtype=f32, device=dev)
@@ -500,14 +510,27 @@
     def fused_hybrid(self) -> bool:
         return _fused_update_mode() == "hybrid"
 
+    def _dz_split_shape(self) -> bool:
+        hs = self.hidden_sizes
+        return (len(hs) == 2 and hs[0] == 128 and hs[1] == 128 and self.in_dim < 32 and not self.act_id
+                and not (self.recurrent or self.md or self.panel))
+
+    def dz_split_ok(self, M: int) -> bool:
+        if not (_dz_split_mode(M) == "1" and self.fused_hybrid() and self._dz_split_shape() and _bwd_fused_mode(M) != "0"
+                and bool(_lib.load().harl_dz_presplit_supported())):
+            return False
+        if self.dzimg is None:
+            self.dzimg = torch.empty(self.rstd[0].numel() * 192, dtype=torch.float32, device=self.device_)
+        return True
+
     def hybrid_outputs(self):
         if not self.fused_hybrid():
             return (None, None, None)
         return (ptr(self.xh[0]), ptr(self.rmask[0]), ptr(self.rstd[0]))
 
-    def backward_after_fused(self, X: torch.Tensor, M: int) -> None:
+    def backward_after_fused(self, X: torch.Tensor, M: int, dz_split: bool = False) -> None:
         if self.fused_hybrid():
-            self.backward_trunk(X, None, M, head_dw_done=True)
+            self.backward_trunk(X, None, M, head_dw_done=True, dz_split=dz_split)
         else:
             self.backward_fused(M)
 
@@ -536,7 +559,7 @@
         self._combine_partials(s)
 
     def backward_trunk(self, X: torch.Tensor, idx: Optional[torch.Tensor], M: int, seq: Optional[dict] = None,
-                       head_dw_done: bool = False) -> None:
+                       head_dw_done: bool = False, dz_split: bool = False) -> None:
         s = stream()
         L = len(self.hidden_sizes)
         nwg = self.n_wg
@@ -618,7 +641,10 @@
             Wp, _ = self._packs[l]
             dw1_here = l == 1 and fuse_dw1
             if bwd_mode != "0" and ho == 128 and hi == 128 and (not dw1_here or self.kp0 == 32):
-                call("harl_mlp_bwd_dx_dw", ptr(self.dz[cur]), ptr(self.xh[l - 1]), ptr(self.rmask[l - 1]), ptr(self.rstd[l - 1]), M,
+                split_here = dz_split and l == L - 1
+                dz_split = dz_split and not split_here
+                call("harl_mlp_bwd_dx_dw_split" if split_here else "harl_mlp_bwd_dx_dw",
+                     ptr(self.dzimg if split_here else self.dz[cur]), ptr(self.xh[l - 1]), ptr(self.rmask[l - 1]), ptr(self.rstd[l - 1]), M,
                      ho, hi, ptr(Wp), None if dw1_here else ptr(self.dz[1 - cur]), ptr(self.x0n) if dw1_here else None,
                      self.kp0 if dw1_here else 0, ptr(self.part[po[0]:]) if dw1_here else None, ptr(self.part[po[l]:]), nwg,
                      int(bwd_mode != "nofill"), s, tag="bwd_full_dw1" if dw1_here else "bwd_full")
@@ -634,6 +660,8 @@
             else:
                 call("harl_mlp_dw_partials", ptr(self.dz[cur]), 0, 0, ho, ptr(self.xh[l - 1]), 0, 0, None, None, None, hi, M,
                      ptr(self.part[po[l]:]), nwg, s, tag="dw_hidden")
+            if dz_split:
+                raise RuntimeError("backward_trunk: dz_L was written as the split image but this layer's kernels read fp32")
             if l == 1 and fuse_dw1:
                 call("harl_mlp_bwd_dx", ptr(self.dz[cur]), ptr(self.xh[0]), ptr(self.rmask[0]), ptr(self.rstd[0]), M, ho, hi,
                      ptr(Wp), None, ptr(self.x0n), self.kp0, ptr(self.part[po[0]:]), nwg, s, tag="bwd_dx_dw1")
diff --git a/harl_amd/traffic.py b/harl_amd/traffic.py
--- a/harl_amd/traffic.py
+++ b/harl_amd/traffic.py
@@ -49,6 +49,10 @@
 def _bwd_dx_dw(a: Sequence) -> float:
     M, HO, HI = a[4], a[5], a[6]
     return M * (4.0 * HO + _act(HI) + (4.0 * HI if a[8] else 0.0) + (4.0 * a[10] if a[9] else 0.0))
+
+
+def _bwd_dx_dw_split(a: Sequence) -> float:
+    return _bwd_dx_dw(a) + a[4] * 2.0 * a[5]
 
 
 def _dw_partials(a: Sequence) -> float:
@@ -124,6 +128,10 @@
                 + (4.0 * w if a[26] else 0.0) + 4.0 * H + (_act(H) if a[31] else 0.0))
 
 
+def _update_fwd_actor_split(a: Sequence) -> float:
+    return _update_fwd_actor(a) + a[1] * 2.0 * a[3]
+
+
 def _update_logp(a: Sequence) -> float:
     M, D, disc, ad = a[1], a[2], a[13], a[14]
     w = 1 if disc else ad
@@ -133,6 +141,10 @@
 
 def _update_fwd_critic(a: Sequence) -> float:
     return a[1] * (4.0 * _kp(a[2]) + 8.0 + 4.0 * a[3] + (_act(a[3]) if a[21] else 0.0))
+
+
+def _update_fwd_critic_split(a: Sequence) -> float:
+    return _update_fwd_critic(a) + a[1] * 2.0 * a[3]
 
 
 def _update_last_actor(a: Sequence) -> float:
@@ -181,6 +193,7 @@
     "harl_mlp_tangent_wide": _tangent_wide,
     "harl_mlp_bwd_dx": _bwd_dx,
     "harl_mlp_bwd_dx_dw": _bwd_dx_dw,
+    "harl_mlp_bwd_dx_dw_split": _bwd_dx_dw_split,
     "harl_mlp_dw_partials": _dw_partials,
     "harl_mlp_dw_partials_multi": _dw_partials_multi,
     "harl_mlp_dw_partials_multi_v": _dw_partials_multi_v,
@@ -193,8 +206,10 @@
     "harl_actor_head_logp": _actor_head_logp,
     "harl_critic_head_loss": _critic_head_loss,
     "harl_update_fwd_actor": _update_fwd_actor,
+    "harl_update_fwd_actor_split": _update_fwd_actor_split,
     "harl_update_logp": _update_logp,
     "harl_update_fwd_critic": _update_fwd_critic,
+    "harl_update_fwd_critic_split": _update_fwd_critic_split,
     "harl_update_values": _update_values,
     "harl_update_last_actor": _update_last_actor,
     "harl_update_last_critic": _update_last_critic,
@@ -309,6 +324,7 @@
     "harl_mlp_tangent_hidden2": lambda a: 2.0 * 2 * a[2] * a[3] * a[4],
     "harl_mlp_bwd_dx": _f_bwd_dx,
     "harl_mlp_bwd_dx_dw": _f_bwd_dx_dw,
+    "harl_mlp_bwd_dx_dw_split": _f_bwd_dx_dw,
     "harl_mlp_dw_partials": _f_dw,
     "harl_mlp_dw_partials_multi": _f_dw_multi,
     "harl_mlp_dw_partials_multi_v": lambda a: 2.0 * a[8] * a[4] * 32 * sum(a[7][k] for k in range(a[0])),
@@ -324,8 +340,10 @@
     "harl_actor_head_fvp": lambda a: 0.0,
     "harl_critic_head_loss": lambda a: _f_head(a[3], a[4], 1, True),
     "harl_update_fwd_actor": _f_update_fwd_actor,
+    "harl_update_fwd_actor_split": _f_update_fwd_actor,
     "harl_update_logp": _f_update_logp,
     "harl_update_fwd_critic": _f_update_fwd_critic,
+    "harl_update_fwd_critic_split": _f_update_fwd_critic,
     "harl_update_values": _f_update_values,
     "harl_update_last_actor": _f_update_last_actor,
     "harl_update_last_critic": _f_update_last_critic,
diff --git a/harl_amd/v_critic.py b/harl_amd/v_critic.py
--- a/harl_amd/v_critic.py
+++ b/harl_amd/v_critic.py
@@ -111,11 +111,13 @@
 
     def _forward_backward(self, net, share_obs, idx, m, value_preds, returns, vn, seq, s) -> None:
         if m > 0 and net.fused_update_ok(idx, seq):
-            call("harl_update_fwd_critic", *net.fused_args(share_obs, m), ptr(value_preds), ptr(returns),
+            fa = net.fused_args(share_obs, m)
+            split = net.dz_split_ok(m)
+            call("harl_update_fwd_critic_split" if split else "harl_update_fwd_critic", *fa, ptr(value_preds), ptr(returns),
                  ptr(vn.stats) if vn is not None else None, float(self.clip_param), int(self.use_clipped_value_loss),
-                 int(self.use_huber_loss), float(self.huber_delta), ptr(net.dz[0]), ptr(net.part_scalars),
+                 int(self.use_huber_loss), float(self.huber_delta), ptr(net.dzimg if split else net.dz[0]), ptr(net.part_scalars),
                  ptr(net.part[net._part_offs[-1]:]), net.n_wg, *net.hybrid_outputs(), s, tag="update_fwd_critic")
-            net.backward_after_fused(share_obs, m)
+            net.backward_after_fused(share_obs, m, dz_split=split)
         elif m > 0 and net.fused_last_ok(idx, seq):
             L = len(net.hidden_sizes)
             net.forward_trunk(share_obs, idx, m, upto=L - 1)
diff --git a/include/harl_hip.h b/include/harl_hip.h
--- a/include/harl_hip.h
+++ b/include/harl_hip.h
@@ -80,6 +80,10 @@
 int harl_mlp_bwd_dx_dw(const float *dz, const float *xprev, const uint32_t *relu_mask_prev, const float *rstd_prev,
                        long M, int HO, int HI, const float *Wp, float *dz_prev, const float *x0n, int kp0, float *dw1_part,
                        float *dw2_part, int n_wg, int fill, void *stream);
+int harl_mlp_bwd_dx_dw_split(const void *dz_img, const float *xprev, const uint32_t *relu_mask_prev, const float *rstd_prev,
+                             long M, int HO, int HI, const float *Wp, float *dz_prev, const float *x0n, int kp0,
+                             float *dw1_part, float *dw2_part, int n_wg, int fill, void *stream);
+int harl_dz_presplit_supported(void);
 int harl_mlp_dw_partials(const float *a, int a_kind, int lda, int HO, const float *b, int b_kind, long ldx,
                          const int64_t *idx, const float *mu0, const float *rstd0, int K, long M, float *part,
                          int n_wg, void *stream);
@@ -210,6 +214,18 @@
                            const float *returns, const float *vn_stats, float clip_param, int use_clipped, int use_huber,
                            float huber_delta, float *dz2, float *part_scalars, float *dw_part_head, int n_part_rows,
                            float *xh1, uint32_t *rmask1, float *rstd1, void *stream);
+int harl_update_fwd_actor_split(const float *x0n, long M, int D, int H, const float *W1p, const float *b1p, const float *W2p,
+                                const float *b2p, const float *Whp, const float *bhp, const float *log_std, float std_x_coef,
+                                float std_y_coef, int discrete, int act_dim, const float *actions, const float *avail,
+                                const float *old_logp, const float *adv, const double *adv_moments, const float *factor,
+                                const float *active, double clip_param, float entropy_coef, int agg_mean, int trpo,
+                                float *logp_out, void *dz2_img, float *part_scalars, float *dw_part_head, int n_part_rows,
+                                float *xh1, uint32_t *rmask1, float *rstd1, void *stream);
+int harl_update_fwd_critic_split(const float *x0n, long M, int D, int H, const float *W1p, const float *b1p, const float *W2p,
+                                 const float *b2p, const float *Whp, const float *bhp, const float *value_preds,
+                                 const float *returns, const float *vn_stats, float clip_param, int use_clipped,
+                                 int use_huber, float huber_delta, void *dz2_img, float *part_scalars, float *dw_part_head,
+                                 int n_part_rows, float *xh1, uint32_t *rmask1, float *rstd1, void *stream);
 int harl_update_last_actor(const float *xin, long M, int H, const float *Wp, const float *bp, const float *Whp,
                            const float *bhp, const float *log_std, float std_x_coef, float std_y_coef, int discrete,
                            int act_dim, const int64_t *idx, const float *actions, const float *avail,
```

Measured after the change: 51.17 million. -2.9%, worse.
